# sunyzhi55/Diffusion_Models_Collection

Measured on AMD Instinct MI355X. Metric: CIFAR-10 UNet DDPM train imgs/sec (aggregate over GPUs), higher is better.
Workload: dtype bf16; 1 GPU; configs/cifar10_unet.py UNet DDPM train step at 32x32 (q_sample, fwd, MSE, bwd, clip, AdamW, EMA), dropout 0.1; model=UNet 37.06M (128ch, mult 1,2,2,2, attn 16/8), global_batch=128, per_gpu_batch=128, parallelism=dp1

## Files before the change

### diffusion_models_collection_amd/_lib.py

```python
import ctypes
import os
from pathlib import Path

import torch

_PKG = Path(__file__).resolve().parent
LIB_PATH = Path(os.environ.get("DMC_LIB", _PKG / "libdmc.so"))

DMC_F32, DMC_BF16 = 0, 1
MODE_NORMAL, MODE_UPSAMPLE, MODE_DILATE = 0, 1, 2
PRO_NONE, PRO_AFFINE_SILU, PRO_SILU, PRO_AFFINE, PRO_GN_SILU = 0, 1, 2, 3, 4
LOSS = {"l1": 0, "l2": 1, "huber": 2}
PRED = {"eps": 0, "v": 1}
OBJECTIVE_MAX_BLOCKS = 64
PACK_FWD, PACK_DGRAD, PACK_UPDGRAD = 0, 1, 2

_c_int, _c_p, _c_f, _c_u32, _c_long, _c_size = (ctypes.c_int, ctypes.c_void_p, ctypes.c_float, ctypes.c_uint32,
                                                ctypes.c_long, ctypes.c_size_t)


ACT_NONE, ACT_GELU, ACT_GELU_DROP, ACT_DGELU = 0, 1, 2, 3
FUSED_GN_STATS = 1


class ConvDesc(ctypes.Structure):
    _fields_ = [
        ("dtype", _c_int), ("N", _c_int), ("H", _c_int), ("W", _c_int),
        ("C1", _c_int), ("C2", _c_int), ("ld1", _c_int), ("ld2", _c_int), ("Kc", _c_int),
        ("OH", _c_int), ("OW", _c_int), ("Cout", _c_int), ("ntaps", _c_int), ("mode", _c_int), ("stride", _c_int),
        ("tap_dy", _c_int * 16), ("tap_dx", _c_int * 16),
        ("prologue", _c_int), ("pro_scale", _c_p), ("pro_shift", _c_p), ("ld_pro", _c_int),
        ("drop_seed", _c_u32), ("drop_thresh", _c_u32), ("drop_scale", _c_f), ("drop_ld", _c_int),
        ("drop_seed_base", _c_p),
        ("bias", _c_p), ("addvec", _c_p), ("ld_add", _c_int), ("resid", _c_p), ("ld_res", _c_int),
        ("silu_pre", _c_p), ("ld_silu", _c_int), ("Csplit", _c_int), ("ldy1", _c_int), ("ldy2", _c_int),
        ("out_f32", _c_int), ("out_nchw", _c_int), ("act", _c_int), ("y_pre", _c_p), ("ld_pre", _c_int),
        ("gn_part", _c_p), ("wg_bias", _c_p), ("pro_groups", _c_int), ("pro_eps", _c_f),
    ]


class ConvPlan(ctypes.Structure):
    _fields_ = [("family", _c_int), ("grid", ctypes.c_uint * 3), ("block", _c_int), ("splits", _c_int),
                ("gn_part", _c_int), ("fused_prologue", _c_int), ("ws_bytes", _c_size)]


CONV_FAMILIES = ("none", "nin_halo", "nout_halo", "narrow_in", "narrow_out", "img", "gemm1x1", "halo", "glds", "reg")
GN_PART_NONE, GN_PART_KERNEL, GN_PART_SPLITK, GN_PART_PASS = 0, 1, 2, 3


class WgradJob(ctypes.Structure):
    _fields_ = [("slab", ctypes.c_void_p), ("bslab", ctypes.c_void_p), ("dw", ctypes.c_void_p),
                ("dbias", ctypes.c_void_p), ("splits", ctypes.c_int), ("KK", ctypes.c_int), ("Cpad", ctypes.c_int),
                ("Cout", ctypes.c_int), ("Ctot", ctypes.c_int), ("ntaps", ctypes.c_int), ("Kc", ctypes.c_int),
                ("scale", ctypes.c_float), ("layout", ctypes.c_int)]


class WgradPlan(ctypes.Structure):
    _fields_ = [("kind", _c_int), ("grid", ctypes.c_uint * 3), ("block", _c_int), ("splits", _c_int),
                ("layout", _c_int), ("group_kind", _c_int), ("ws_bytes", _c_size)]


WGRAD_KINDS = ("", "img4", "pipe", "halo", "gemm1x1", "generic")


class WgradGroupItem(ctypes.Structure):
    _fields_ = [("d", ctypes.POINTER(ConvDesc)), ("dy", ctypes.c_void_p), ("ld_dy", ctypes.c_int),
                ("x1", ctypes.c_void_p), ("x2", ctypes.c_void_p), ("workspace", ctypes.c_void_p),
                ("dw", ctypes.c_void_p), ("scale", ctypes.c_float)]


WGRAD_GROUP_MAX = 8


class ColsumJob(ctypes.Structure):
    _fields_ = [("in_", ctypes.c_void_p), ("R", ctypes.c_int), ("C", ctypes.c_int), ("ld", ctypes.c_long),
                ("stride", ctypes.c_int), ("out0", ctypes.c_void_p), ("out1", ctypes.c_void_p),
                ("scale", ctypes.c_float)]


class PackJob(ctypes.Structure):
    _fields_ = [("w", _c_p), ("dst", _c_p), ("dtype", _c_int), ("mode", _c_int), ("Cout", _c_int), ("Cin", _c_int),
                ("kh", _c_int), ("kw", _c_int), ("Kc", _c_int), ("koff", _c_int)]


class TensorRef(ctypes.Structure):
    _fields_ = [("a", _c_p), ("b", _c_p), ("n", _c_long)]


def _load():
    if not LIB_PATH.exists():
        raise RuntimeError(
            f"libdmc.so not found at {LIB_PATH}. Build it with `python -m diffusion_models_collection_amd.build` "
            "(there is no fallback: the diffusion hot path runs only on the gfx950 HIP kernels).")
    lib = ctypes.CDLL(str(LIB_PATH))
    sig = {
        "dmc_version": (_c_int, []),
        "dmc_set_option": (_c_int, [ctypes.c_char_p, _c_long]),
        "dmc_get_option": (_c_long, [ctypes.c_char_p]),
        "dmc_reset_options": (None, [_c_int]),
        "dmc_last_error": (ctypes.c_char_p, []),
        "dmc_conv2d_workspace": (_c_size, [ctypes.POINTER(ConvDesc)]),
        "dmc_conv_halo_prologue": (_c_int, [ctypes.POINTER(ConvDesc)]),
        "dmc_conv2d_fused_epilogue": (_c_int, [ctypes.POINTER(ConvDesc), ctypes.c_size_t]),
        "dmc_conv2d_plan": (_c_int, [ctypes.POINTER(ConvDesc), ctypes.c_size_t, ctypes.POINTER(ConvPlan)]),
        "dmc_conv2d": (_c_int, [ctypes.POINTER(ConvDesc), _c_p, _c_p, _c_p, _c_p, _c_p, _c_p, _c_size, _c_p]),
        "dmc_conv2d_wgrad_workspace": (_c_size, [ctypes.POINTER(ConvDesc)]),
        "dmc_conv2d_wgrad": (_c_int, [ctypes.POINTER(ConvDesc), _c_p, _c_int, _c_p, _c_p, _c_p, _c_p, _c_f, _c_p]),
        "dmc_conv2d_wgrad_partial": (_c_int, [ctypes.POINTER(ConvDesc), _c_p, _c_int, _c_p, _c_p, _c_p, _c_p, _c_f,
                                              ctypes.POINTER(WgradJob), _c_p]),
        "dmc_wgrad_reduce_batch": (_c_int, [ctypes.POINTER(WgradJob), _c_int, _c_p]),
        "dmc_conv2d_wgrad_plan": (_c_int, [ctypes.POINTER(ConvDesc), _c_int, ctypes.POINTER(WgradPlan)]),
        "dmc_conv2d_wgrad_group_ok": (_c_int, [ctypes.POINTER(ConvDesc), _c_int]),
        "dmc_conv2d_wgrad_group_workspace": (_c_size, [ctypes.POINTER(WgradGroupItem), _c_int,
                                                       ctypes.POINTER(_c_size)]),
        "dmc_conv2d_wgrad_group": (_c_int, [ctypes.POINTER(WgradGroupItem), _c_int, ctypes.POINTER(WgradJob), _c_p]),
        "dmc_wgrad_slab_bytes": (_c_long, [_c_int]),
        "dmc_pack_weight": (_c_int, [_c_int, _c_int, _c_p, _c_int, _c_int, _c_int, _c_int, _c_int, _c_p, _c_p]),
        "dmc_pack_tiles": (_c_int, [ctypes.POINTER(PackJob), _c_int, _c_p, _c_int]),
        "dmc_pack_weights": (_c_int, [_c_p, _c_p, _c_int, _c_p]),
        "dmc_gn_workspace": (_c_size, [_c_int, _c_int, _c_int, _c_int]),
        "dmc_gn_stats": (_c_int, [_c_int, _c_p, _c_p, _c_int, _c_int, _c_int, _c_int, _c_int, _c_int, _c_int, _c_f,
                                  _c_p, _c_p, _c_p, _c_p, _c_p, _c_p, _c_p]),
        "dmc_gn_finalize": (_c_int, [_c_p, _c_int, _c_p, _c_int, _c_int, _c_int, _c_int, _c_f, _c_p, _c_p, _c_p, _c_p,
                                     _c_p, _c_p]),
        "dmc_gn_stats_apply_ok": (_c_int, [_c_int, _c_int, _c_int, _c_int, _c_int, _c_int]),
        "dmc_gn_stats_apply": (_c_int, [_c_int, _c_p, _c_p, _c_int, _c_int, _c_int, _c_int, _c_int, _c_int, _c_int,
                                        _c_f, _c_p, _c_p, _c_p, _c_p, _c_p, _c_int, _c_u32, _c_p, _c_u32, _c_f, _c_p,
                                        _c_int, _c_p]),
        "dmc_gn_apply": (_c_int, [_c_int, _c_p, _c_p, _c_int, _c_int, _c_int, _c_int, _c_int, _c_int, _c_p, _c_p,
                                  _c_int, _c_u32, _c_p, _c_u32, _c_f, _c_p, _c_int, _c_p]),
        "dmc_gn_silu_bwd": (_c_int, [_c_int, _c_p, _c_int, _c_p, _c_p, _c_int, _c_int, _c_int, _c_int, _c_int,
                                     _c_int, _c_int, _c_p, _c_p, _c_p, _c_int, _c_u32, _c_p, _c_u32, _c_f, _c_p, _c_p,
                                     _c_int, _c_int, _c_int, _c_int, _c_p, _c_p, _c_p, _c_int, _c_p, _c_p, _c_p,
                                     _c_p]),
        "dmc_gn_silu_bwd_deferred": (_c_int, [_c_int, _c_p, _c_int, _c_p, _c_p, _c_int, _c_int, _c_int, _c_int,
                                              _c_int, _c_int, _c_int, _c_p, _c_p, _c_p, _c_int, _c_u32, _c_p, _c_u32,
                                              _c_f, _c_p, _c_p, _c_int, _c_int, _c_int, _c_int, _c_p, _c_p, _c_p,
                                              _c_int, _c_p, _c_p, _c_p, _c_p, _c_p, ctypes.POINTER(ctypes.c_int),
                                              _c_p, _c_int, _c_p]),
        "dmc_colsum_batch": (_c_int, [ctypes.POINTER(ColsumJob), _c_int, _c_p]),
        "dmc_channel_sum_workspace": (_c_size, [_c_int, _c_int, _c_int]),
        "dmc_channel_sum": (_c_int, [_c_int, _c_p, _c_int, _c_int, _c_int, _c_int, _c_p, _c_int, _c_p, _c_f, _c_p,
                                     _c_p]),
        "dmc_attn_fwd": (_c_int, [_c_int, _c_p, _c_int, _c_int, _c_int, _c_int, _c_int, _c_p, _c_int, _c_p, _c_u32,
                                  _c_p, _c_u32, _c_f, _c_p]),
        "dmc_attn_workspace": (_c_size, [_c_int, _c_int, _c_int]),
        "dmc_attn_bwd": (_c_int, [_c_int, _c_p, _c_int, _c_p, _c_p, _c_int, _c_p, _c_int, _c_int, _c_int, _c_int,
                                  _c_p, _c_int, _c_p, _c_u32, _c_p, _c_u32, _c_f, _c_p]),
        "dmc_time_embed": (_c_int, [_c_p, _c_int, _c_int, _c_p, _c_p]),
        "dmc_embed_fwd": (_c_int, [_c_p, _c_int, _c_int, _c_p, _c_int, _c_p, _c_p]),
        "dmc_embed_bwd": (_c_int, [_c_p, _c_int, _c_int, _c_p, _c_int, _c_p, _c_p]),
        "dmc_pack_input": (_c_int, [_c_int, _c_p, _c_p, _c_p, _c_p, _c_p, _c_int, _c_int, _c_int, _c_int, _c_p,
                                    _c_int, _c_p]),
        "dmc_q_sample": (_c_int, [_c_p, _c_p, _c_p, _c_p, _c_p, _c_int, _c_int, _c_p, _c_p]),
        "dmc_loss_fwd": (_c_int, [_c_int, _c_p, _c_p, _c_long, _c_p, _c_p, _c_p]),
        "dmc_loss_bwd": (_c_int, [_c_int, _c_p, _c_p, _c_long, _c_p, _c_p, _c_p]),
        "dmc_objective": (_c_int, [_c_int, _c_int, _c_p, _c_p, _c_p, _c_p, _c_p, _c_p, _c_p, _c_int, _c_int, _c_int,
                                   _c_p, _c_p, _c_p, _c_p, _c_p]),
        "dmc_pred_convert": (_c_int, [_c_int, _c_p, _c_p, _c_p, _c_p, _c_int, _c_p, _c_int, _c_int, _c_int, _c_p,
                                      _c_p, _c_p]),
        "dmc_ddim_step": (_c_int, [_c_p, _c_p, _c_p, _c_p, _c_p, _c_p, _c_int, _c_int, _c_f, _c_int, _c_p, _c_p,
                                   _c_p]),
        "dmc_ddpm_step": (_c_int, [_c_p, _c_p, _c_p, _c_p, _c_p, _c_p, _c_p, _c_p, _c_p, _c_int, _c_int, _c_int,
                                   _c_p, _c_p, _c_p]),
        "dmc_dpm_step": (_c_int, [_c_p, _c_p, _c_p, _c_p, _c_p, _c_p, _c_int, _c_int, _c_int, _c_int, _c_p, _c_p,
                                  _c_p]),
        "dmc_known_blend": (_c_int, [_c_p, _c_p, _c_p, _c_int, _c_p, _c_p, _c_p, _c_p, _c_int, _c_int, _c_int, _c_p,
                                     _c_p]),
        "dmc_cfg_x0": (_c_int, [_c_p, _c_p, _c_p, _c_f, _c_p, _c_p, _c_p, _c_int, _c_int, _c_int, _c_f, _c_p, _c_p,
                                _c_p]),
        "dmc_ema_update": (_c_int, [_c_p, _c_int, _c_f, _c_p]),
        "dmc_clip_grad_norm": (_c_int, [_c_p, _c_int, _c_f, _c_p, _c_p, _c_p]),
        "dmc_grad_norm_flat": (_c_int, [_c_p, _c_long, _c_f, _c_p, _c_p, _c_p, _c_p]),
        "dmc_adamw_flat": (_c_int, [_c_p, _c_p, _c_p, _c_p, _c_p, _c_long, _c_p] + [_c_f] * 9 + [_c_p]),
        "dmc_adamw_flat_dev": (_c_int, [_c_p, _c_p, _c_p, _c_p, _c_p, _c_long, _c_p, _c_p, _c_p]),
        "dmc_silu_fwd": (_c_int, [_c_p, _c_p, _c_long, _c_p]),
        "dmc_upsample2x_nhwc": (_c_int, [_c_int, _c_p, _c_int, _c_int, _c_int, _c_int, _c_int, _c_p, _c_int, _c_p]),
        "dmc_unpack_output": (_c_int, [_c_int, _c_p, _c_int, _c_int, _c_int, _c_int, _c_int, _c_p, _c_p]),
        "dmc_add": (_c_int, [_c_int, _c_p, _c_p, _c_long, _c_p]),
        "dmc_ln_mod_fwd": (_c_int, [_c_int, _c_p, _c_p, _c_int, _c_p, _c_p, _c_p, _c_int, _c_int, _c_int, _c_int, _c_f,
                                    _c_u32, _c_p, _c_u32, _c_f, _c_p, _c_p, _c_int, _c_p, _c_p, _c_p]),
        "dmc_ln_mod_bwd": (_c_int, [_c_int, _c_p, _c_int, _c_p, _c_p, _c_p, _c_p, _c_int, _c_int, _c_int, _c_int, _c_p,
                                    _c_p, _c_p, _c_p, _c_p]),
        "dmc_dit_rowsum_workspace": (_c_size, [_c_int, _c_int, _c_int]),
        "dmc_gate_bwd": (_c_int, [_c_int, _c_p, _c_p, _c_int, _c_p, _c_int, _c_int, _c_int, _c_int, _c_u32, _c_p, _c_u32,
                                  _c_f, _c_p, _c_int, _c_p, _c_p, _c_p]),
# ... 87 lines not shown
```

### diffusion_models_collection_amd/csrc/dmc_conv.hip

```cpp
#include "dmc_conv_impl.h"

namespace {

template <typename T> DMC_DEV void load4(const char* p, size_t idx, float* v, bool f32);
template <typename T>
DMC_DEV void load4(const char* p, size_t idx, float* v, bool f32) {
  if (f32 || sizeof(T) == 4) {
    v4f x = *(const v4f*)(p + idx * 4);
    v[0] = x[0]; v[1] = x[1]; v[2] = x[2]; v[3] = x[3];
  } else {
    v2i x = *(const v2i*)(p + idx * 2);
    v[0] = bf2f((uint32_t)x[0] & 0xffffu); v[1] = bf2f((uint32_t)x[0] >> 16);
    v[2] = bf2f((uint32_t)x[1] & 0xffffu); v[3] = bf2f((uint32_t)x[1] >> 16);
  }
}
template <typename T>
DMC_DEV void store4(char* p, size_t idx, const float* v, bool f32) {
  if (f32 || sizeof(T) == 4) {
    v4f x = {v[0], v[1], v[2], v[3]};
    *(v4f*)(p + idx * 4) = x;
  } else {
    v2i x;
    x[0] = (int)f2bf2(v[0], v[1]);
    x[1] = (int)f2bf2(v[2], v[3]);
// ... 139 lines not shown
template <typename T>
DMC_DEV void apply_act(const ConvK& a, float* v, int pix, int co, bool of32) {
  if (a.act == DMC_ACT_DGELU) {
    float u[4];
    load4<T>(a.ypre, (size_t)pix * a.ldpre + co, u, of32);
    const uint32_t seed = a.dthresh ? a.dseed + (a.dseed_base ? *a.dseed_base : 0u) : 0u;
#pragma unroll
    for (int e = 0; e < 4; ++e) {
      const float g = (sizeof(T) == 2 && !of32) ? bf2f(f2bf(v[e])) : v[e];
      float m = 1.f;
      if (a.dthresh) m = drop_keep((uint64_t)pix * a.Cout + co + e, seed, a.dthresh) ? a.dscale : 0.f;
      v[e] = g * m * gelu_grad(u[e]);
    }
    return;
  }
  if (a.ypre) store4<T>(a.ypre, (size_t)pix * a.ldpre + co, v, of32);
#pragma unroll
  for (int e = 0; e < 4; ++e) {
    const float u = (sizeof(T) == 2 && !of32) ? bf2f(f2bf(v[e])) : v[e];
    v[e] = gelu_f(u);
  }
  if (a.act == DMC_ACT_GELU_DROP && a.dthresh) {
    const uint32_t seed = a.dseed + (a.dseed_base ? *a.dseed_base : 0u);
#pragma unroll
    for (int e = 0; e < 4; ++e)
      v[e] = drop_keep((uint64_t)pix * a.Cout + co + e, seed, a.dthresh) ? v[e] * a.dscale : 0.f;
  }
}

template <typename T>
DMC_DEV void conv_store_tile(const ConvK& a, const v4f accv, const int pix, const int co) {
  const bool of32 = a.out_f32 != 0;
  if (pix < a.M && co < a.Cout) {
    const int n = pix / a.OHW;
    {
      float v[4] = {accv[0], accv[1], accv[2], accv[3]};
      const bool full = (co + 3 < a.Cout) && ((a.Cout & 3) == 0);
      if (full && !a.out_nchw) {
        if (a.bias) { v4f b = *(const v4f*)(a.bias + co); v[0] += b[0]; v[1] += b[1]; v[2] += b[2]; v[3] += b[3]; }
        if (a.addvec) { v4f b = *(const v4f*)(a.addvec + (size_t)n * a.ld_add + co); v[0] += b[0]; v[1] += b[1]; v[2] += b[2]; v[3] += b[3]; }
        if (a.silu_pre) {
          v4f z = *(const v4f*)(a.silu_pre + (size_t)pix * a.ld_silu + co);
#pragma unroll
          for (int e = 0; e < 4; ++e) { float sg = sigmoid_f(z[e]); v[e] *= sg * (1.f + z[e] * (1.f - sg)); }
        }
        if (a.resid) { float r[4]; load4<T>(a.resid, (size_t)pix * a.ld_res + co, r, of32); v[0] += r[0]; v[1] += r[1]; v[2] += r[2]; v[3] += r[3]; }
        if (a.act) apply_act<T>(a, v, pix, co, of32);
        if (co < a.Csplit) store4<T>(a.y1, (size_t)pix * a.ldy1 + co, v, of32);
        else store4<T>(a.y2, (size_t)pix * a.ldy2 + (co - a.Csplit), v, of32);
      } else {
#pragma unroll
        for (int e = 0; e < 4; ++e) {
          const int c = co + e;
          if (c >= a.Cout) break;
          float x = v[e];
          if (a.bias) x += a.bias[c];
          if (a.addvec) x += a.addvec[(size_t)n * a.ld_add + c];
          if (a.silu_pre) { float z = a.silu_pre[(size_t)pix * a.ld_silu + c]; float sg = sigmoid_f(z); x *= sg * (1.f + z * (1.f - sg)); }
          if (a.out_nchw) {
            const int rem = pix - n * a.OHW;
            float* y = (float*)a.y1 + ((size_t)n * a.Cout + c) * a.OHW + rem;
            if (a.resid) x += ((const float*)a.resid)[((size_t)n * a.Cout + c) * a.OHW + rem];
            *y = x;
          } else {
            if (a.resid) x += (of32 ? ld_as_f<float>(a.resid, (size_t)pix * a.ld_res + c) : ld_as_f<T>(a.resid, (size_t)pix * a.ld_res + c));
            if (c < a.Csplit) {
              if (of32) ((float*)a.y1)[(size_t)pix * a.ldy1 + c] = x; else st_from_f<T>(a.y1, (size_t)pix * a.ldy1 + c, x);
            } else {
              if (of32) ((float*)a.y2)[(size_t)pix * a.ldy2 + c - a.Csplit] = x; else st_from_f<T>(a.y2, (size_t)pix * a.ldy2 + c - a.Csplit, x);
            }
          }
        }
      }
    }
  }
}

DMC_DEV void chan_eq(float& m, float& q, float mb, float qb, float n) {
  const float d = mb - m;
  q = q + qb + d * d * (0.5f * n);
  m = 0.5f * (m + mb);
}

template <int BM, int BN, int NT>
DMC_DEV void tile_epilogue8(const ConvK& a, const char* lds, int EP, int m0, int n0) {
  constexpr int CG = BN / 8, RS = NT / CG, IT = BM / RS;
  constexpr int SEG = 64, NSEG = BM / SEG, KPS = SEG / RS;
  static_assert((CG == 16 || CG == 8) && SEG % RS == 0 && BM % SEG == 0, "GroupNorm partial geometry");
  const int cg = threadIdx.x % CG, r0 = threadIdx.x / CG;
  const int co = n0 + cg * 8;
  if (co >= a.Cout) return;
  float gm[NSEG], gq[NSEG];
#pragma unroll
  for (int j = 0; j < NSEG; ++j) { gm[j] = 0.f; gq[j] = 0.f; }
  v4f b0 = {0.f, 0.f, 0.f, 0.f}, b1 = {0.f, 0.f, 0.f, 0.f};
  if (a.bias) { b0 = *(const v4f*)(a.bias + co); b1 = *(const v4f*)(a.bias + co + 4); }
  const bool first = co < a.Csplit;
  char* const y = first ? a.y1 : a.y2;
  const int ldy = first ? a.ldy1 : a.ldy2, cy = first ? co : co - a.Csplit;
  v4i rr[IT];
  if (a.resid) {
#pragma unroll
    for (int k = 0; k < IT; ++k) {
      const int pix = min(m0 + r0 + k * RS, a.M - 1);
      rr[k] = *(const v4i*)(a.resid + ((size_t)pix * a.ld_res + co) * 2);
    }
  }
  int n = (m0 + r0) / a.OHW, nend = (n + 1) * a.OHW;
  v4f e0 = {0.f, 0.f, 0.f, 0.f}, e1 = {0.f, 0.f, 0.f, 0.f};
  if (a.addvec) {
    e0 = *(const v4f*)(a.addvec + (size_t)n * a.ld_add + co);
    e1 = *(const v4f*)(a.addvec + (size_t)n * a.ld_add + co + 4);
  }
#pragma unroll
  for (int k = 0; k < IT; ++k) {
    const int pl = r0 + k * RS;
    const int pix = m0 + pl;
    if (pix < a.M) {
      if (a.addvec && pix >= nend) {
        n = pix / a.OHW;
        nend = (n + 1) * a.OHW;
        e0 = *(const v4f*)(a.addvec + (size_t)n * a.ld_add + co);
        e1 = *(const v4f*)(a.addvec + (size_t)n * a.ld_add + co + 4);
      }
      const v4f v0 = *(const v4f*)(lds + pl * EP + cg * 32) + b0 + e0;
      const v4f v1 = *(const v4f*)(lds + pl * EP + cg * 32 + 16) + b1 + e1;
      float f[8] = {v0[0], v0[1], v0[2], v0[3], v1[0], v1[1], v1[2], v1[3]};
      if (a.resid) {
        float r[8];
        Chunk<bf16_t>::unpack(rr[k], r);
#pragma unroll
        for (int e = 0; e < 8; ++e) f[e] += r[e];
      }
      if (a.act == DMC_ACT_DGELU) {
        Chunk<bf16_t>::unpack(Chunk<bf16_t>::pack(f), f);
        float u[8];
        Chunk<bf16_t>::unpack(*(const v4i*)(a.ypre + ((size_t)pix * a.ldpre + co) * 2), u);
        const uint32_t seed = a.dthresh ? a.dseed + (a.dseed_base ? *a.dseed_base : 0u) : 0u;
#pragma unroll
        for (int e = 0; e < 8; ++e) {
          float m = 1.f;
          if (a.dthresh) m = drop_keep((uint64_t)pix * a.Cout + co + e, seed, a.dthresh) ? a.dscale : 0.f;
          f[e] = f[e] * m * gelu_grad(u[e]);
        }
      } else if (a.act) {
        const v4i pre = Chunk<bf16_t>::pack(f);
        if (a.ypre) *(v4i*)(a.ypre + ((size_t)pix * a.ldpre + co) * 2) = pre;
        Chunk<bf16_t>::unpack(pre, f);
#pragma unroll
        for (int e = 0; e < 8; ++e) f[e] = gelu_f(f[e]);
        if (a.act == DMC_ACT_GELU_DROP && a.dthresh) {
          const uint32_t seed = a.dseed + (a.dseed_base ? *a.dseed_base : 0u);
#pragma unroll
          for (int e = 0; e < 8; ++e)
            f[e] = drop_keep((uint64_t)pix * a.Cout + co + e, seed, a.dthresh) ? f[e] * a.dscale : 0.f;
        }
      }
      const v4i out = Chunk<bf16_t>::pack(f);
      *(v4i*)(y + ((size_t)pix * ldy + cy) * 2) = out;
      if (a.gst) {
        float g[8];
        Chunk<bf16_t>::unpack(out, g);
        float mb = 0.f;
#pragma unroll
        for (int e = 0; e < 8; ++e) mb += g[e];
        mb *= 0.125f;
        float qb = 0.f;
#pragma unroll
        for (int e = 0; e < 8; ++e) qb = fmaf(g[e] - mb, g[e] - mb, qb);
        const int kk = k % KPS;
#pragma unroll
        for (int j = 0; j < NSEG; ++j) {
          if (j != k / KPS) continue;
          if (kk == 0) { gm[j] = mb; gq[j] = qb; }
          else {
            const float d = mb - gm[j], nn = 8.f * kk;
            gm[j] += d * (8.f / (nn + 8.f));
            gq[j] += qb + d * d * (nn * 8.f / (nn + 8.f));
          }
        }
      }
    }
  }
  if (a.gst) {
    const int lane = threadIdx.x & 63, wave = threadIdx.x >> 6;
    constexpr int NW = NT / 64;
    float cnt = 8.f * KPS;
#pragma unroll
    for (int sh = CG; sh < 64; sh <<= 1) {
#pragma unroll
      for (int j = 0; j < NSEG; ++j) {
        const float mb = __shfl_xor(gm[j], sh), qb = __shfl_xor(gq[j], sh);
        chan_eq(gm[j], gq[j], mb, qb, cnt);
      }
      cnt *= 2.f;
    }
    float* red = (float*)(lds + BM * EP);
    if (lane < CG) {
#pragma unroll
      for (int j = 0; j < NSEG; ++j) {
        red[((wave * NSEG + j) * CG + lane) * 2] = gm[j];
        red[((wave * NSEG + j) * CG + lane) * 2 + 1] = gq[j];
      }
    }
    __syncthreads();
    if (threadIdx.x < NSEG * CG) {
      const int j = threadIdx.x / CG, c = threadIdx.x % CG;
      float m = red[(j * CG + c) * 2], q = red[(j * CG + c) * 2 + 1];
      for (int w = 1; w < NW; ++w) {
        const float mb = red[((w * NSEG + j) * CG + c) * 2], qb = red[((w * NSEG + j) * CG + c) * 2 + 1];
        const float na = cnt * w, nb = cnt;
        const float d = mb - m;
        m += d * (nb / (na + nb));
        q += qb + d * d * (na * nb / (na + nb));
      }
      const size_t o = ((size_t)(m0 / SEG + j) * (a.Cout / 8) + (n0 / 8 + c)) * 2;
      a.gst[o] = m;
      a.gst[o + 1] = q;
    }
  }
}

template <typename T, int BM, int BN, int NT>
DMC_DEV void tile_epilogue(const ConvK& a, const char* lds, int EP, int m0, int n0) {
  constexpr int CG = BN / 4, RS = NT / CG;
  const int cg = threadIdx.x % CG, r0 = threadIdx.x / CG;
  const int co = n0 + cg * 4;
  if (a.out_nchw || a.silu_pre || (a.Cout & 3)) {
    for (int pl = r0; pl < BM; pl += RS) conv_store_tile<T>(a, *(const v4f*)(lds + pl * EP + cg * 16), m0 + pl, co);
    return;
  }
  if constexpr ((BN == 128 || BN == 64) && BM % 64 == 0) {
    if (sizeof(T) == 2 && !a.out_f32 && !((a.Cout | a.Csplit | a.ldy1 | a.ldy2 | a.ld_res) & 7)) {
      tile_epilogue8<BM, BN, NT>(a, lds, EP, m0, n0);
      return;
    }
  }
  if (co >= a.Cout) return;
  const bool of32 = a.out_f32 != 0;
  const v4f b = a.bias ? *(const v4f*)(a.bias + co) : v4f{0.f, 0.f, 0.f, 0.f};
  const bool first = co < a.Csplit;
  char* const y = first ? a.y1 : a.y2;
  const int ldy = first ? a.ldy1 : a.ldy2, cy = first ? co : co - a.Csplit;
  int n = (m0 + r0) / a.OHW, nend = (n + 1) * a.OHW;
  for (int pl = r0; pl < BM; pl += RS) {
    const int pix = m0 + pl;
    if (pix >= a.M) break;
    v4f v = *(const v4f*)(lds + pl * EP + cg * 16) + b;
    if (a.addvec) {
      while (pix >= nend) { ++n; nend += a.OHW; }
      v += *(const v4f*)(a.addvec + (size_t)n * a.ld_add + co);
    }
    float f[4] = {v[0], v[1], v[2], v[3]};
    if (a.resid) {
      float r[4];
      load4<T>(a.resid, (size_t)pix * a.ld_res + co, r, of32);
      f[0] += r[0]; f[1] += r[1]; f[2] += r[2]; f[3] += r[3];
    }
    if (a.act) apply_act<T>(a, f, pix, co, of32);
    store4<T>(y, (size_t)pix * ldy + cy, f, of32);
  }
}

__device__ v4i g_zero_page[64];


template <int AI, int BI, int BM>
DMC_DEV void glds_issue(const ConvK& a, char* base, int k0, int c0, int wave, int lrow, int lc, int n0,
                        const int* sp) {
  const int c = c0 + lc * 8;
  const int Ctot = a.C1 + a.C2;
#pragma unroll
  for (int j = 0; j < AI; ++j) {
    const void* src = g_zero_page;
    if (sp[j] >= 0 && c < Ctot)
      src = (c < a.C1) ? (const void*)(a.x1 + ((size_t)sp[j] * a.ld1 + c) * 2)
                       : (const void*)(a.x2 + ((size_t)sp[j] * a.ld2 + (c - a.C1)) * 2);
    __builtin_amdgcn_global_load_lds(src, (LDS_AS void*)(base + (wave * AI + j) * 8 * 128), 16, 0, 0);
  }
  const size_t wrow = (size_t)a.ntaps * a.Kc;
#pragma unroll
  for (int j = 0; j < BI; ++j) {
    const int co = n0 + (wave * BI + j) * 8 + lrow;
    const void* src = (co < a.Cout) ? (const void*)(a.w + ((size_t)co * wrow + k0 + lc * 8) * 2) : g_zero_page;
    __builtin_amdgcn_global_load_lds(src, (LDS_AS void*)(base + BM * 128 + (wave * BI + j) * 8 * 128), 16, 0, 0);
  }
}


template <int AI, int BI, int BM>
DMC_DEV void glds_issue_buf(const ConvK& a, char* base, int c0, unsigned k2, int wave, const unsigned* o1,
                            const unsigned* o2, const unsigned* ob) {
  if (c0 < a.C1) {
    const __amdgpu_buffer_rsrc_t r = __builtin_amdgcn_make_buffer_rsrc((void*)a.x1, (short)0, a.x1_bytes, 0x00020000);
    const unsigned c2 = (unsigned)c0 * 2u;
#pragma unroll
    for (int j = 0; j < AI; ++j)
      __builtin_amdgcn_raw_ptr_buffer_load_lds(r, (LDS_AS void*)(base + (wave * AI + j) * 1024), 16, o1[j] + c2, 0, 0, 0);
  } else {
    const __amdgpu_buffer_rsrc_t r = __builtin_amdgcn_make_buffer_rsrc((void*)a.x2, (short)0, a.x2_bytes, 0x00020000);
    const unsigned c2 = (unsigned)(c0 - a.C1) * 2u;
#pragma unroll
    for (int j = 0; j < AI; ++j)
      __builtin_amdgcn_raw_ptr_buffer_load_lds(r, (LDS_AS void*)(base + (wave * AI + j) * 1024), 16, o2[j] + c2, 0, 0, 0);
  }
  const __amdgpu_buffer_rsrc_t rw = __builtin_amdgcn_make_buffer_rsrc((void*)a.w, (short)0, a.w_bytes, 0x00020000);
#pragma unroll
  for (int j = 0; j < BI; ++j)
    __builtin_amdgcn_raw_ptr_buffer_load_lds(rw, (LDS_AS void*)(base + BM * 128 + (wave * BI + j) * 1024), 16, ob[j] + k2, 0, 0, 0);
}

DMC_DEV void xcd_tile(int NB, int& mb, int& nb) {
  const int total = gridDim.x, bid = blockIdx.x, per = total >> 3;
  const int t = bid < (per << 3) ? (bid & 7) * per + (bid >> 3) : bid;
  mb = t / NB;
  nb = t - mb * NB;
}

__host__ __device__ inline bool reg_epi_ok(const ConvK& a) {
  return a.reg_epi && (a.gst || a.reg_epi >= 2) && a.dtype_bytes == 2 && !a.out_f32 && !a.out_nchw && !a.silu_pre && a.Csplit == a.Cout &&
         a.act == DMC_ACT_NONE && (a.Cout & 127) == 0 && (a.ldy1 & 7) == 0 &&
         (!a.resid || (a.ld_res & 7) == 0) && (a.M & 127) == 0 && (!a.gst || a.OHW % 64 == 0);
}
DMC_DEV void reg_epilogue(const ConvK& a, v4f (&acc)[4][4], int m0, int n0, int wm, int wn) {
  const int lane = threadIdx.x & 63, fr = lane & 15, fh = lane >> 4;
  const bool odd = fh & 1;
  v4i rra[4][2];
  v4f ba[4], eva[4];
  const int img0 = (m0 + wm * 64) / a.OHW;
#pragma unroll
  for (int i = 0; i < 4; ++i) {
    const int co = n0 + wn * 64 + i * 16 + fh * 4;
    const int cc = co - (odd ? 4 : 0);
#pragma unroll
    for (int jp = 0; jp < 2; ++jp) {
      rra[i][jp] = v4i{0, 0, 0, 0};
      if (a.resid) {
        const int px = m0 + wm * 64 + (2 * jp + (odd ? 1 : 0)) * 16 + fr;
        rra[i][jp] = *(const v4i*)(a.resid + ((size_t)px * a.ld_res + cc) * 2);
      }
    }
    ba[i] = a.bias ? *(const v4f*)(a.bias + co) : v4f{0.f, 0.f, 0.f, 0.f};
    eva[i] = a.addvec ? *(const v4f*)(a.addvec + (size_t)img0 * a.ld_add + co) : v4f{0.f, 0.f, 0.f, 0.f};
  }
#pragma unroll
  for (int i = 0; i < 4; ++i) {
    const int co = n0 + wn * 64 + i * 16 + fh * 4;
    const int cc = co - (odd ? 4 : 0);
    const v4f b = ba[i];
    float gm = 0.f, gq = 0.f;
    int nimg = img0;
    v4f ev = eva[i];
#pragma unroll
    for (int jp = 0; jp < 2; ++jp) {
      v2i o[2];
      const v4i rr = rra[i][jp];
      v2i rs;
      rs[0] = __shfl_xor(odd ? rr[0] : rr[2], 16);
      rs[1] = __shfl_xor(odd ? rr[1] : rr[3], 16);
#pragma unroll
      for (int h = 0; h < 2; ++h) {
        const int j = 2 * jp + h;
        const int px = m0 + wm * 64 + j * 16 + fr;
        v4f v = acc[i][j] + b;
        if (a.addvec) {
          const int n = px / a.OHW;
          if (n != nimg) { nimg = n; ev = *(const v4f*)(a.addvec + (size_t)n * a.ld_add + co); }
          v = v + ev;
        }
        float f[4] = {v[0], v[1], v[2], v[3]};
        if (a.resid) {
          const bool own = (h == 1) == odd;
          const uint32_t r0 = own ? (uint32_t)(odd ? rr[2] : rr[0]) : (uint32_t)rs[0];
          const uint32_t r1 = own ? (uint32_t)(odd ? rr[3] : rr[1]) : (uint32_t)rs[1];
          f[0] += bf2f(r0 & 0xffffu); f[1] += bf2f(r0 >> 16);
          f[2] += bf2f(r1 & 0xffffu); f[3] += bf2f(r1 >> 16);
        }
        o[h][0] = (int)f2bf2(f[0], f[1]);
        o[h][1] = (int)f2bf2(f[2], f[3]);
        if (a.gst) {
          const float g0 = bf2f((uint32_t)o[h][0] & 0xffffu), g1 = bf2f((uint32_t)o[h][0] >> 16);
          const float g2 = bf2f((uint32_t)o[h][1] & 0xffffu), g3 = bf2f((uint32_t)o[h][1] >> 16);
          const float mb = ((g0 + g1) + (g2 + g3)) * 0.25f;
          const float qb =
              fmaf(g3 - mb, g3 - mb, fmaf(g2 - mb, g2 - mb, fmaf(g1 - mb, g1 - mb, (g0 - mb) * (g0 - mb))));
          if (j == 0) { gm = mb; gq = qb; }
          else {
            const float d = mb - gm, nn = 4.f * j;
            gm += d * (4.f / (nn + 4.f));
            gq += qb + d * d * (nn * 4.f / (nn + 4.f));
          }
        }
      }
      v2i send = odd ? o[0] : o[1], recv;
      recv[0] = __shfl_xor(send[0], 16);
      recv[1] = __shfl_xor(send[1], 16);
      v4i outv;
      if (!odd) { outv[0] = o[0][0]; outv[1] = o[0][1]; outv[2] = recv[0]; outv[3] = recv[1]; }
      else { outv[0] = recv[0]; outv[1] = recv[1]; outv[2] = o[1][0]; outv[3] = o[1][1]; }
      const int pxs = m0 + wm * 64 + (2 * jp + (odd ? 1 : 0)) * 16 + fr;
      *(v4i*)(a.y1 + ((size_t)pxs * a.ldy1 + cc) * 2) = outv;
    }
    if (a.gst) {
      float cnt = 16.f;
#pragma unroll
      for (int sh = 1; sh <= 16; sh <<= 1) {
        const float mb = __shfl_xor(gm, sh), qb = __shfl_xor(gq, sh);
        chan_eq(gm, gq, mb, qb, cnt);
        cnt *= 2.f;
      }
      if (fr == 0 && !odd) {
        const size_t o = ((size_t)((m0 + wm * 64) / 64) * (a.Cout / 8) + cc / 8) * 2;
        a.gst[o] = gm;
        a.gst[o + 1] = gq;
      }
    }
  }
}

template <int WM, int WN, bool BUF, int STAGES = 3>
__global__ __launch_bounds__(WM * WN * 64) void conv_fwd_glds_kernel(ConvK a) {
  using T = bf16_t;
  constexpr int NW = WM * WN;
  constexpr int BM = 64 * WM, BN = 64 * WN;
  constexpr int SB = (BM + BN) * 128;
  constexpr int AI = BM / 8 / NW;
  constexpr int BI = BN / 8 / NW;
  static_assert(AI >= 1 && BI >= 1, "tile too small for the wave count");
  constexpr int EPB = BM * (BN * 4 + 16) + NW * (BM / 64) * 16 * (NW <= 4 ? 64 : 8);
  constexpr int LDS_BYTES = STAGES * SB > EPB ? STAGES * SB : EPB;
  __shared__ __attribute__((aligned(16))) char lds[LDS_BYTES];

  const int lane = threadIdx.x & 63;
  const int wave = __builtin_amdgcn_readfirstlane(threadIdx.x >> 6);
  const int wm = wave % WM, wn = wave / WM;
  int mb = blockIdx.x, nb = blockIdx.y;
  if (!a.sk && gridDim.y == 1) xcd_tile((a.Cout + BN - 1) / BN, mb, nb);
  const int m0 = mb * BM;
  const int n0 = nb * BN;
  const int lrow = lane >> 3;
  const int lc = (lane & 7) ^ lrow;

  int pn[AI], poy[AI], pox[AI];
#pragma unroll
  for (int j = 0; j < AI; ++j) {
    const int pix = m0 + (wave * AI + j) * 8 + lrow;
    if (pix < a.M) {
      pn[j] = pix / a.OHW;
      const int rem = pix - pn[j] * a.OHW;
      poy[j] = rem / a.OW;
      pox[j] = rem - poy[j] * a.OW;
    } else {
      pn[j] = -1; poy[j] = 0; pox[j] = 0;
    }
  }
  const int nstages = a.ntaps * (a.Kc / 64);

  v4f acc[4][4];
#pragma unroll
  for (int i = 0; i < 4; ++i)
#pragma unroll
    for (int j = 0; j < 4; ++j) acc[i][j] = v4f{0.f, 0.f, 0.f, 0.f};

  const int s_begin = a.sk ? blockIdx.z * a.sk_per : 0;
  const int s_end = a.sk ? min(nstages, s_begin + a.sk_per) : nstages;
  const int ns = s_end - s_begin;
  const int kst = a.Kc / 64;
  int is_tap = s_begin / kst, is_c0 = (s_begin - is_tap * kst) * 64;
  int sp[AI];
  unsigned o1[AI], o2[AI], ob[BI];
  if constexpr (BUF) {
    const unsigned wrow = (unsigned)(a.ntaps * a.Kc);
#pragma unroll
    for (int j = 0; j < BI; ++j) {
      const int co = n0 + (wave * BI + j) * 8 + lrow;
      ob[j] = co < a.Cout ? ((unsigned)co * wrow + lc * 8) * 2u : kOOB;
    }
  }
  auto tap_rows = [&]() {
#pragma unroll
    for (int j = 0; j < AI; ++j) {
      const int p = pn[j] >= 0 ? src_pixel(a, pn[j], poy[j], pox[j], is_tap) : -1;
      if constexpr (BUF) {
        o1[j] = p >= 0 ? ((unsigned)p * a.ld1 + lc * 8) * 2u : kOOB;
        o2[j] = p >= 0 ? ((unsigned)p * a.ld2 + lc * 8) * 2u : kOOB;
      } else {
        sp[j] = p;
      }
    }
  };
  tap_rows();
  auto issue = [&](int S) {
    char* base = lds + (S % STAGES) * SB;
    if constexpr (BUF) {
      glds_issue_buf<AI, BI, BM>(a, base, is_c0, (unsigned)(s_begin + S) * 128u, wave, o1, o2, ob);
    } else {
      glds_issue<AI, BI, BM>(a, base, (s_begin + S) * 64, is_c0, wave, lrow, lc, n0, sp);
    }
    is_c0 += 64;
    if (is_c0 == a.Kc) { is_c0 = 0; ++is_tap; if (is_tap < a.ntaps) tap_rows(); }
  };
#define DMC_GLDS_ISSUE(S) issue(S)
  for (int q = 0; q < STAGES - 1 && q < ns; ++q) DMC_GLDS_ISSUE(q);
  const int fr = lane & 15, fh = lane >> 4;
  for (int s = 0; s < ns; ++s) {
    if (STAGES > 2 && s + STAGES - 2 < ns) __builtin_amdgcn_s_waitcnt(waitcnt_vm((STAGES - 2) * (AI + BI)));
    else __builtin_amdgcn_s_waitcnt(waitcnt_vm(0));
    asm volatile("" ::: "memory");
    __builtin_amdgcn_sched_barrier(0);
    __builtin_amdgcn_s_barrier();
    __builtin_amdgcn_sched_barrier(0);
    asm volatile("" ::: "memory");
    if (s + STAGES - 1 < ns) DMC_GLDS_ISSUE(s + STAGES - 1);
    const char* A = lds + (s % STAGES) * SB;
    const char* B = A + BM * 128;
    v4i fa[2][4], fb[2][4];
#pragma unroll
    for (int ks = 0; ks < 2; ++ks) {
      const int chunk = ks * 4 + fh;
#pragma unroll
      for (int i = 0; i < 4; ++i) {
        const int r = wn * 64 + i * 16 + fr;
        fa[ks][i] = *(const v4i*)(B + r * 128 + ((chunk ^ (r & 7)) << 4));
      }
#pragma unroll
      for (int j = 0; j < 4; ++j) {
        const int r = wm * 64 + j * 16 + fr;
        fb[ks][j] = *(const v4i*)(A + r * 128 + ((chunk ^ (r & 7)) << 4));
      }
    }
#pragma unroll
    for (int ks = 0; ks < 2; ++ks)
#pragma unroll
      for (int i = 0; i < 4; ++i)
#pragma unroll
        for (int j = 0; j < 4; ++j) acc[i][j] = mma16<T>(acc[i][j], fa[ks][i], fb[ks][j]);
    __builtin_amdgcn_sched_group_barrier(0x100, 8, 0);
#pragma unroll
    for (int g = 0; g < 8; ++g) {
      __builtin_amdgcn_sched_group_barrier(0x008, 2, 0);
      __builtin_amdgcn_sched_group_barrier(0x100, 1, 0);
    }
    __builtin_amdgcn_sched_group_barrier(0x008, 16, 0);
  }
#undef DMC_GLDS_ISSUE
  constexpr int EP = BN * 4 + 16;
  if constexpr (WM == 2 && WN == 2) {
    if (!a.sk && reg_epi_ok(a) && n0 + BN <= a.Cout && m0 + BM <= a.M) {
      reg_epilogue(a, acc, m0, n0, wm, wn);
      return;
    }
  }
  __syncthreads();
#pragma unroll
  for (int j = 0; j < 4; ++j)
#pragma unroll
    for (int i = 0; i < 4; ++i)
      *(v4f*)(lds + (wm * 64 + j * 16 + fr) * EP + (wn * 64 + i * 16 + fh * 4) * 4) = acc[i][j];
  __syncthreads();
  if (a.sk) {
    const int Cpad = gridDim.y * BN;
    float* slab = a.sk + (size_t)blockIdx.z * a.M * Cpad;
    for (int idx = threadIdx.x; idx < BM * BN / 4; idx += NW * 64) {
      const int pl = idx / (BN / 4), cg = idx - pl * (BN / 4);
      if (m0 + pl < a.M) *(v4f*)(slab + (size_t)(m0 + pl) * Cpad + n0 + cg * 4) = *(const v4f*)(lds + pl * EP + cg * 16);
    }
    return;
  }
  tile_epilogue<T, BM, BN, NW * 64>(a, lds, EP, m0, n0);
}

DMC_DEV void wait_vm_upto40(int n) {
  switch (n < 0 ? 0 : n) {
#define DMC_W(i) case i: __builtin_amdgcn_s_waitcnt(waitcnt_vm(i)); break;
    DMC_W(0) DMC_W(1) DMC_W(2) DMC_W(3) DMC_W(4) DMC_W(5) DMC_W(6) DMC_W(7) DMC_W(8) DMC_W(9) DMC_W(10)
    DMC_W(11) DMC_W(12) DMC_W(13) DMC_W(14) DMC_W(15) DMC_W(16) DMC_W(17) DMC_W(18) DMC_W(19) DMC_W(20)
    DMC_W(21) DMC_W(22) DMC_W(23) DMC_W(24) DMC_W(25) DMC_W(26) DMC_W(27) DMC_W(28) DMC_W(29) DMC_W(30)
    DMC_W(31) DMC_W(32) DMC_W(33) DMC_W(34) DMC_W(35) DMC_W(36) DMC_W(37) DMC_W(38) DMC_W(39)
#undef DMC_W
    default: __builtin_amdgcn_s_waitcnt(waitcnt_vm(40)); break;
  }
}

template <int NS>
__global__ __launch_bounds__(256, NS <= 2 ? 2 : 1) void gemm1x1_persist_kernel(ConvK a, int ntiles, int NB, int tpb) {
  using T = bf16_t;
  constexpr int BM = 128, BN = 128, AI = 4, BI = 4, SB = (BM + BN) * 128;
  __shared__ __attribute__((aligned(16))) char lds[NS * SB + 4096];
  float* const sbias = (float*)(lds + NS * SB);
  const int lane = threadIdx.x & 63;
  const int wave = __builtin_amdgcn_readfirstlane(threadIdx.x >> 6);
  const int wm = wave % 2, wn = wave / 2;
  const int lrow = lane >> 3, lc = (lane & 7) ^ lrow;
  const int fr = lane & 15, fh = lane >> 4;
  const int t_begin = blockIdx.x * tpb, t_end = min(ntiles, t_begin + tpb);
  if (t_begin >= t_end) return;
  const int kst = a.Kc / 64, total = (t_end - t_begin) * kst;
  for (int c = threadIdx.x; c < NB * BN; c += 256) sbias[c] = (a.bias && c < a.Cout) ? a.bias[c] : 0.f;
  __builtin_amdgcn_s_waitcnt(waitcnt_vm(0));

  unsigned o1[AI], o2[AI], ob[BI];
  int it_tile = -1;
  auto issue = [&](int S) {
    const int ti = t_begin + S / kst, k = S - (S / kst) * kst;
    if (ti != it_tile) {
      it_tile = ti;
      const int mb = ti / NB, nb = ti - mb * NB;
#pragma unroll
      for (int j = 0; j < AI; ++j) {
        const unsigned pix = (unsigned)(mb * BM + (wave * AI + j) * 8 + lrow);
        o1[j] = (pix * a.ld1 + lc * 8) * 2u;
        o2[j] = (pix * a.ld2 + lc * 8) * 2u;
      }
#pragma unroll
      for (int j = 0; j < BI; ++j) {
        const unsigned co = (unsigned)(nb * BN + (wave * BI + j) * 8 + lrow);
        ob[j] = (co * a.Kc + lc * 8) * 2u;
      }
    }
    glds_issue_buf<AI, BI, BM>(a, lds + (S % NS) * SB, k * 64, (unsigned)k * 128u, wave, o1, o2, ob);
  };
  int nvm = 0;
  int pos[NS];
#pragma unroll
  for (int q = 0; q < NS; ++q) pos[q] = 0;
  for (int q = 0; q < NS - 1 && q < total; ++q) {
    issue(q);
    nvm += AI + BI;
    pos[q] = nvm;
  }
  v4f acc[4][4];
#pragma unroll
  for (int i = 0; i < 4; ++i)
#pragma unroll
    for (int j = 0; j < 4; ++j) acc[i][j] = v4f{0.f, 0.f, 0.f, 0.f};
  for (int s = 0; s < total; ++s) {
    int mine = 0;
#pragma unroll
    for (int q = 0; q < NS; ++q)
      if (q == s % NS) mine = pos[q];
    wait_vm_upto40(nvm - mine);
    asm volatile("" ::: "memory");
    __builtin_amdgcn_sched_barrier(0);
    __builtin_amdgcn_s_barrier();
    __builtin_amdgcn_sched_barrier(0);
    asm volatile("" ::: "memory");
    v2i rres[4][4];
    const bool last = (s + 1) % kst == 0;
    if (a.resid && last) {
      const int t = t_begin + s / kst, mb = t / NB, nb = t - mb * NB;
#pragma unroll
      for (int i = 0; i < 4; ++i)
// ... 472 lines not shown
        const int cc = ks * 4 + fh;
#pragma unroll
        for (int i = 0; i < NI; ++i) {
          const int r = (i * 16 + fr) * 9 + t;
          ga[ks][i] = *(const v4i*)(Wt + r * 128 + ((cc ^ (r & 7)) << 4));
        }
#pragma unroll
        for (int j = 0; j < NJ; ++j)
          gb[ks][j] = *(const v4i*)(ok[j] ? A + src[j] * 128 + ((cc ^ (src[j] & 7)) << 4) : zrow);
      }
    };
    read_tap(0, fa[0], fb[0]);
    __builtin_amdgcn_sched_group_barrier(0x100, 2 * (NI + NJ), 0);
#pragma unroll
    for (int t = 0; t < 9; ++t) {
      const int cur = t & 1;
      if (t + 1 < 9) read_tap(t + 1, fa[cur ^ 1], fb[cur ^ 1]);
#pragma unroll
      for (int ks = 0; ks < 2; ++ks)
#pragma unroll
        for (int i = 0; i < NI; ++i)
#pragma unroll
          for (int j = 0; j < NJ; ++j) acc[i][j] = mma16<T>(acc[i][j], fa[cur][ks][i], fb[cur][ks][j]);
      if (t + 1 < 9) __builtin_amdgcn_sched_group_barrier(0x100, 2 * (NI + NJ), 0);
      __builtin_amdgcn_sched_group_barrier(0x008, 2 * NI * NJ, 0);
    }
  }
  if (fast) {
#pragma unroll
    for (int i = 0; i < NI; ++i) {
      float gm = 0.f, gq = 0.f;
#pragma unroll
      for (int j = 0; j < NJ; ++j) {
        const int co = n0 + i * 16 + fh * 4, pix = m0 + qrow[j];
        const v4f v = (acc[i][j] + eb[i]) + ea[i][NJE == 1 ? 0 : j];
        const float r0 = bf2f((uint32_t)er[i][j][0] & 0xffffu), r1 = bf2f((uint32_t)er[i][j][0] >> 16);
        const float r2 = bf2f((uint32_t)er[i][j][1] & 0xffffu), r3 = bf2f((uint32_t)er[i][j][1] >> 16);
        v2i o;
        o[0] = (int)f2bf2(v[0] + r0, v[1] + r1);
        o[1] = (int)f2bf2(v[2] + r2, v[3] + r3);
        *(v2i*)(a.y1 + ((size_t)pix * a.ldy1 + co) * 2) = o;
        if (MW == 64 && a.gst) {
          const float g0 = bf2f((uint32_t)o[0] & 0xffffu), g1 = bf2f((uint32_t)o[0] >> 16);
          const float g2 = bf2f((uint32_t)o[1] & 0xffffu), g3 = bf2f((uint32_t)o[1] >> 16);
          const float mb = ((g0 + g1) + (g2 + g3)) * 0.25f;
          const float qb =
              fmaf(g3 - mb, g3 - mb, fmaf(g2 - mb, g2 - mb, fmaf(g1 - mb, g1 - mb, (g0 - mb) * (g0 - mb))));
          if (j == 0) { gm = mb; gq = qb; }
          else {
            const float d = mb - gm, nn = 4.f * j;
            gm += d * (4.f / (nn + 4.f));
            gq += qb + d * d * (nn * 4.f / (nn + 4.f));
          }
        }
      }
      if (MW == 64 && a.gst) {
        float cnt = 16.f;
#pragma unroll
        for (int sh = 1; sh <= 16; sh <<= 1) {
          const float mb = __shfl_xor(gm, sh), qb = __shfl_xor(gq, sh);
          chan_eq(gm, gq, mb, qb, cnt);
          cnt *= 2.f;
        }
        if (fr == 0 && !(fh & 1)) {
          const size_t o = ((size_t)((m0 + wave * 64) / 64) * (a.Cout / 8) + (n0 + i * 16 + fh * 4) / 8) * 2;
          a.gst[o] = gm;
          a.gst[o + 1] = gq;
        }
      }
    }
    return;
  }
#pragma unroll
  for (int i = 0; i < NI; ++i)
#pragma unroll
    for (int j = 0; j < NJ; ++j) conv_store_tile<T>(a, acc[i][j], m0 + qrow[j], n0 + i * 16 + fh * 4);
}

bool dma_operands_ok(const ConvK& k) {
  return k.C1 % 64 == 0 && k.C2 % 64 == 0 && k.Kc == k.C1 + k.C2 && k.x1_bytes > 0 && (k.C2 == 0 || k.x2_bytes > 0) &&
         k.w_bytes > 0;
}

int img_plan(const ConvK& k, long mask) {
  if (!mask || k.dtype_bytes != 2 || (k.prologue != DMC_PRO_NONE && k.prologue != DMC_PRO_GN_SILU)) return 0;
  if (k.prologue == DMC_PRO_GN_SILU) {
    const int C = k.C1 + k.C2;
    if (k.tdy0 != -1 || C > 512 || k.gn_G <= 0 || C % k.gn_G || (C / k.gn_G) % 8 || 64 % (C / k.gn_G) || k.dthresh)
      return 0;
  }
  if (!same_size_3x3(k) || !((k.OH == 8 && k.OW == 8) || (k.OH == 4 && k.OW == 4)) || k.M % 128) return 0;
  if (!dma_operands_ok(k)) return 0;
  const int bit = (k.OH == 8 ? 2 : 0) + (k.tdy0 == 1 ? 1 : 0);
  if (!((mask >> bit) & 1)) return 0;
  const int bm = k.OH == 8 ? 256 : 128;
  if (k.M % bm) return 0;
  const int bn = (long)k.Cout * (k.M / bm) >= 512L * 16 ? 32 : 16;
  if (k.Cout % bn) return 0;
  if (k.OH == 8 && (long)(k.M / bm) * (k.Cout / bn) > 256) return 0;
  if (k.prologue == DMC_PRO_GN_SILU && !((k.OH == 4 && bn == 16) || (k.OH == 8 && bn == 32))) return 0;
  return bn;
}

int nin_plan(const ConvK& k, int* R, int* nimg) {
  if (k.dtype_bytes != 2 || k.prologue != DMC_PRO_NONE || k.C2 != 0 || k.C1 > 8 || k.ld1 != 8 || k.Cout % 128 ||
      k.silu_pre || k.act)
    return 0;
  return halo2_plan(k, R, nimg);
}
int nout_plan(const ConvK& k, int* R, int* nimg) {
  if (k.dtype_bytes != 2 || k.prologue != DMC_PRO_NONE || k.Cout > 16 || k.C1 + k.C2 > 128 || !dma_operands_ok(k) ||
      k.act)
    return 0;
  return halo2_plan(k, R, nimg);
}


template <typename T>
DMC_DEV v4i mask_chunk(v4i v, int n) {
#pragma unroll
  for (int d = 0; d < 4; ++d) {
    if (sizeof(T) == 4) {
      if (d >= n) v[d] = 0;
    } else {
      if (2 * d >= n) v[d] = 0;
      else if (2 * d + 1 >= n) v[d] &= 0xffff;
    }
  }
  return v;
}

DMC_DEV void pixel_coords(const ConvK& a, int pix, int& n, int& oy, int& ox) {
  n = pix < a.M ? pix / a.OHW : -1;
  const int rem = pix - (n < 0 ? 0 : n) * a.OHW;
  oy = rem / a.OW;
  ox = rem - oy * a.OW;
}

template <typename T>
__global__ __launch_bounds__(256) void conv_narrow_in_kernel(ConvK a) {
  const int lane = threadIdx.x & 63;
  const int fr = lane & 15, fh = lane >> 4;
  const int p0 = (blockIdx.x * 4 + (threadIdx.x >> 6)) * 64;
  const int n0 = blockIdx.y * 32;
  if (p0 >= a.M) return;
  int pn[4], poy[4], pox[4];
#pragma unroll
  for (int j = 0; j < 4; ++j) pixel_coords(a, p0 + 16 * j + fr, pn[j], poy[j], pox[j]);
  const size_t wrow = (size_t)a.ntaps * a.Kc;
  v4f acc[2][4];
#pragma unroll
  for (int i = 0; i < 2; ++i)
#pragma unroll
    for (int j = 0; j < 4; ++j) acc[i][j] = v4f{0.f, 0.f, 0.f, 0.f};
  for (int t0 = 0; t0 < a.ntaps; t0 += 4) {
    const int tap = t0 + fh;
    const bool tok = tap < a.ntaps;
    const int tp = tok ? tap : 0;
    v4i fa[2];
#pragma unroll
    for (int i = 0; i < 2; ++i) {
      const int co = n0 + 16 * i + fr;
      v4i w = *(const v4i*)(a.w + ((size_t)(co < a.Cout ? co : 0) * wrow + (size_t)tp * a.Kc) * sizeof(T));
      if (!(tok && co < a.Cout)) w = v4i{0, 0, 0, 0};
      fa[i] = w;
    }
// ... 236 lines not shown
  if constexpr (SP > 0) {
    v4f v[SP];
#pragma unroll
    for (int z = 0; z < SP; ++z) v[z] = *(const v4f*)(p + z * zs);
    v4f t = v[0];
#pragma unroll
    for (int z = 1; z < SP; ++z) t += v[z];
    return t;
  } else {
    v4f t = *(const v4f*)p;
    for (int z = 1; z < splits; ++z) t += *(const v4f*)(p + z * zs);
    return t;
  }
}

template <typename T, int SP>
__global__ __launch_bounds__(256) void conv_splitk_epilogue_kernel(ConvK a, int splits, int Cpad) {
  const int cg_per_row = Cpad / 4;
  const long total = (long)a.M * cg_per_row;
  const size_t zs = (size_t)a.M * Cpad;
  for (long idx = blockIdx.x * (long)blockDim.x + threadIdx.x; idx < total; idx += (long)gridDim.x * blockDim.x) {
    const int pix = idx / cg_per_row;
    const int co = (idx - (long)pix * cg_per_row) * 4;
    if (co >= a.Cout) continue;
    const v4f v = splitk_sum<SP>(a.sk + (size_t)pix * Cpad + co, zs, splits);
    conv_store_tile<T>(a, v, pix, co);
  }
}
template <typename T, int SP>
__global__ __launch_bounds__(256) void conv_splitk_epi_gn_kernel(ConvK a, int splits, int Cpad) {
  const int lane = threadIdx.x & 63;
  const int nch = a.Cout / 8;
  const long w = blockIdx.x * 4L + (threadIdx.x >> 6);
  if (w >= (long)(a.M / 64) * nch) return;
  const int seg = (int)(w / nch), ch = (int)(w - (long)seg * nch);
  const int pix = seg * 64 + lane, co = ch * 8;
  const size_t zs = (size_t)a.M * Cpad;
  const float* p = a.sk + (size_t)pix * Cpad + co;
  const v4f v0 = splitk_sum<SP>(p, zs, splits), v1 = splitk_sum<SP>(p + 4, zs, splits);
  conv_store_tile<T>(a, v0, pix, co);
  conv_store_tile<T>(a, v1, pix, co + 4);
  const size_t row = (size_t)pix * a.ldy1 + co;
  float f[8];
  load4<T>(a.y1, row, f, false);
  load4<T>(a.y1, row + 4, f + 4, false);
  float t = 0.f;
#pragma unroll
  for (int e = 0; e < 8; ++e) t += f[e];
  const float m = wave_sum(t) * (1.0f / 512.0f);
  float q = 0.f;
#pragma unroll
  for (int e = 0; e < 8; ++e) q = fmaf(f[e] - m, f[e] - m, q);
  q = wave_sum(q);
  if (lane == 0) { a.gsk[w * 2] = m; a.gsk[w * 2 + 1] = q; }
}

template <typename T>
void launch_splitk_epilogue(const ConvK& k, int splits, int Cpad, int blocks, hipStream_t s) {
  switch (splits) {
    case 2: conv_splitk_epilogue_kernel<T, 2><<<blocks, 256, 0, s>>>(k, splits, Cpad); break;
    case 3: conv_splitk_epilogue_kernel<T, 3><<<blocks, 256, 0, s>>>(k, splits, Cpad); break;
    case 4: conv_splitk_epilogue_kernel<T, 4><<<blocks, 256, 0, s>>>(k, splits, Cpad); break;
    case 5: conv_splitk_epilogue_kernel<T, 5><<<blocks, 256, 0, s>>>(k, splits, Cpad); break;
    case 6: conv_splitk_epilogue_kernel<T, 6><<<blocks, 256, 0, s>>>(k, splits, Cpad); break;
    case 7: conv_splitk_epilogue_kernel<T, 7><<<blocks, 256, 0, s>>>(k, splits, Cpad); break;
    case 8: conv_splitk_epilogue_kernel<T, 8><<<blocks, 256, 0, s>>>(k, splits, Cpad); break;
    default: conv_splitk_epilogue_kernel<T, 0><<<blocks, 256, 0, s>>>(k, splits, Cpad); break;
  }
}
void launch_splitk_epi_gn(const ConvK& k, int splits, int Cpad, hipStream_t s) {
  const int blocks = (int)(((long)(k.M / 64) * (k.Cout / 8) + 3) / 4);
  switch (splits) {
    case 2: conv_splitk_epi_gn_kernel<bf16_t, 2><<<blocks, 256, 0, s>>>(k, splits, Cpad); break;
    case 3: conv_splitk_epi_gn_kernel<bf16_t, 3><<<blocks, 256, 0, s>>>(k, splits, Cpad); break;
    case 4: conv_splitk_epi_gn_kernel<bf16_t, 4><<<blocks, 256, 0, s>>>(k, splits, Cpad); break;
    case 5: conv_splitk_epi_gn_kernel<bf16_t, 5><<<blocks, 256, 0, s>>>(k, splits, Cpad); break;
    case 6: conv_splitk_epi_gn_kernel<bf16_t, 6><<<blocks, 256, 0, s>>>(k, splits, Cpad); break;
    case 7: conv_splitk_epi_gn_kernel<bf16_t, 7><<<blocks, 256, 0, s>>>(k, splits, Cpad); break;
    case 8: conv_splitk_epi_gn_kernel<bf16_t, 8><<<blocks, 256, 0, s>>>(k, splits, Cpad); break;
    default: conv_splitk_epi_gn_kernel<bf16_t, 0><<<blocks, 256, 0, s>>>(k, splits, Cpad); break;
  }
}

DMC_DEV float pack_value(int mode, const float* w, int Cout, int Cin, int kh, int kw, int row, int t, int k) {
  if (mode == DMC_PACK_FWD) return k < Cin ? w[((size_t)row * Cin + k) * kh * kw + t] : 0.f;
  if (k >= Cout) return 0.f;
  if (mode == DMC_PACK_DGRAD) return w[((size_t)k * Cin + row) * kh * kw + t];
  const int u = t >> 2, vv = t & 3;
  const int khs[4][2] = {{2, -1}, {1, 2}, {0, 1}, {0, -1}};
  const float* base = w + ((size_t)k * Cin + row) * 9;
  float v = 0.f;
  for (int a1 = 0; a1 < 2; ++a1) {
    const int y = khs[u][a1];
    if (y < 0) continue;
    for (int b1 = 0; b1 < 2; ++b1) {
      const int x = khs[vv][b1];
      if (x < 0) continue;
      v += base[y * 3 + x];
    }
  }
  return v;
}

template <typename T>
__global__ void pack_weight_kernel(int mode, const float* w, int Cout, int Cin, int kh, int kw, int Kc, T* dst) {
  const int ntaps = (mode == DMC_PACK_UPDGRAD) ? 16 : kh * kw;
  const int rows = (mode == DMC_PACK_FWD) ? Cout : Cin;
  const long total = (long)rows * ntaps * Kc;
  for (long o = blockIdx.x * (long)blockDim.x + threadIdx.x; o < total; o += (long)gridDim.x * blockDim.x) {
    const int k = o % Kc;
    const long r = o / Kc;
    const float v = pack_value(mode, w, Cout, Cin, kh, kw, r / ntaps, r % ntaps, k);
    if (sizeof(T) == 4) ((float*)dst)[o] = v;
    else ((bf16_t*)dst)[o] = (bf16_t)f2bf(v);
  }
}

constexpr int kPackFwdK = 256, kPackFwdCo = 4, kPackDgC = 16, kPackDgCo = 64;
constexpr int kPackDgP = kPackDgC * 9 + 1;
constexpr int kPackLds = kPackDgCo * kPackDgP > kPackFwdCo * kPackFwdK * 9 ? kPackDgCo * kPackDgP
                                                                          : kPackFwdCo * kPackFwdK * 9;

__global__ __launch_bounds__(256) void pack_tiles_kernel(const dmc_pack_job* jobs, const int* tiles) {
  __shared__ float sw[kPackLds];
  const int* tl = tiles + 3 * blockIdx.x;
  const dmc_pack_job J = jobs[tl[0]];
  const int khkw = J.kh * J.kw;
  const int koff = J.koff >= 0 ? J.koff : 0;
  const bool f32 = J.dtype == DMC_F32;
  const int tid = threadIdx.x, wv = tid >> 6, ln = tid & 63;
  auto store = [&](long di, float v) {
    if (f32) ((float*)J.dst)[di] = v;
    else ((bf16_t*)J.dst)[di] = (bf16_t)f2bf(v);
  };
  if (J.mode == DMC_PACK_FWD) {
    const int co0 = tl[1], k0 = tl[2];
    const int nco = min(kPackFwdCo, J.Cout - co0);
    const int KW = J.koff >= 0 ? J.Cin : J.Kc;
    const int kn = min(kPackFwdK, KW - k0);
    const int kv = max(0, min(kn, J.Cin - k0));
    const int run = kv * khkw;
    {
      float v[kPackFwdCo][9];
#pragma unroll
      for (int r = 0; r < kPackFwdCo; ++r)
#pragma unroll
        for (int u = 0; u < 9; ++u) {
          const int j = tid + u * 256;
          v[r][u] = (r < nco && j < run) ? J.w[((size_t)(co0 + r) * J.Cin + k0) * khkw + j] : 0.f;
        }
#pragma unroll
      for (int r = 0; r < kPackFwdCo; ++r)
#pragma unroll
        for (int u = 0; u < 9; ++u)
          if (r < nco && tid + u * 256 < run) sw[r * kPackFwdK * 9 + tid + u * 256] = v[r][u];
    }
    __syncthreads();
    if (!f32 && ((J.Kc | koff | k0 | kn) & 1) == 0) {
      for (int r = 0; r < nco; ++r)
        for (int t = 0; t < khkw; ++t)
          for (int k = 2 * tid; k < kn; k += 512) {
            const float v0 = k < kv ? sw[r * kPackFwdK * 9 + k * khkw + t] : 0.f;
            const float v1 = k + 1 < kv ? sw[r * kPackFwdK * 9 + (k + 1) * khkw + t] : 0.f;
            *(uint32_t*)((bf16_t*)J.dst + ((long)(co0 + r) * khkw + t) * J.Kc + koff + k0 + k) = f2bf2(v0, v1);
          }
      return;
    }
    for (int r = 0; r < nco; ++r)
      for (int t = 0; t < khkw; ++t)
        for (int k = tid; k < kn; k += 256)
          store(((long)(co0 + r) * khkw + t) * J.Kc + koff + k0 + k, k < kv ? sw[r * kPackFwdK * 9 + k * khkw + t] : 0.f);
    return;
  }
  const int c0 = tl[1], co0 = tl[2];
  const int KW = J.koff >= 0 ? J.Cout : J.Kc;
  const int cn = min(kPackDgC, J.Cin - c0), con = min(kPackDgCo, KW - co0);
  const int cov = max(0, min(con, J.Cout - co0));
  const int run = cn * khkw;
  {
    float v[16][3];
#pragma unroll
    for (int a2 = 0; a2 < 16; ++a2)
#pragma unroll
      for (int u = 0; u < 3; ++u) {
        const int r = wv + 4 * a2, j = ln + 64 * u;
        v[a2][u] = (r < cov && j < run) ? J.w[((size_t)(co0 + r) * J.Cin + c0) * khkw + j] : 0.f;
      }
#pragma unroll
    for (int a2 = 0; a2 < 16; ++a2)
#pragma unroll
      for (int u = 0; u < 3; ++u) {
        const int r = wv + 4 * a2, j = ln + 64 * u;
        if (r < cov && j < run) sw[r * kPackDgP + j] = v[a2][u];
      }
  }
  __syncthreads();
  const int ntaps = J.mode == DMC_PACK_UPDGRAD ? 16 : khkw;
  auto value = [&](int co, int c, int t) {
    float v = 0.f;
    if (co < cov) {
      const float* wp = sw + co * kPackDgP + c * khkw;
      if (J.mode == DMC_PACK_DGRAD) {
        v = wp[t];
      } else {
        const int u = t >> 2, vv = t & 3;
        const int khs[4][2] = {{2, -1}, {1, 2}, {0, 1}, {0, -1}};
        for (int a1 = 0; a1 < 2; ++a1) {
          const int y = khs[u][a1];
          if (y < 0) continue;
          for (int b1 = 0; b1 < 2; ++b1) {
            const int x = khs[vv][b1];
            if (x >= 0) v += wp[y * 3 + x];
          }
        }
      }
    }
    return v;
  };
  if (!f32 && ((J.Kc | koff | co0 | con) & 1) == 0) {
    const int cp = 2 * (ln & 31);
    for (int q = 2 * wv + (ln >> 5); q < cn * ntaps; q += 8) {
      const int c = q / ntaps, t = q - c * ntaps;
      if (cp >= con) continue;
      *(uint32_t*)((bf16_t*)J.dst + ((long)(c0 + c) * ntaps + t) * J.Kc + koff + co0 + cp) =
          f2bf2(value(cp, c, t), value(cp + 1, c, t));
    }
    return;
  }
  const int co = ln;
  for (int q = wv; q < cn * ntaps; q += 4) {
    const int c = q / ntaps, t = q - c * ntaps;
    if (co >= con) continue;
    store(((long)(c0 + c) * ntaps + t) * J.Kc + koff + co0 + co, value(co, c, t));
  }
}


struct FwdPlan {
  int cfg;
  int splits;
  int per;
  size_t ws;
};

FwdPlan plan_glds(const ConvK& k) {
  FwdPlan p{0, 1, 0, 0};
  const int nst = k.ntaps * (k.Kc / 64);
  const long b42 = (long)dmc::cdiv(k.M, 256) * dmc::cdiv(k.Cout, 128);
  const long b22 = (long)dmc::cdiv(k.M, 128) * dmc::cdiv(k.Cout, 128);
  if (b42 >= 240) { p.cfg = 0; return p; }
  long blocks = b22;
  p.cfg = 1;
  const long target = dmc::opt(dmc::OPT_SK_TARGET);
  int sp = (int)((target + blocks - 1) / blocks);
  const int maxs = nst / 4;
  if (sp > maxs) sp = maxs;
  if (sp > dmc::opt(dmc::OPT_SK_MAX)) sp = (int)dmc::opt(dmc::OPT_SK_MAX);
  if (sp >= 2) {
    p.splits = sp;
    p.per = (nst + sp - 1) / sp;
    p.splits = (nst + p.per - 1) / p.per;
    p.ws = (size_t)p.splits * k.M * (size_t)dmc::cdiv(k.Cout, 128) * 128 * sizeof(float);
  } else if (b22 < 120) {
    p.cfg = 2;
  }
  return p;
}

struct RegPlan {
  bool big;
  int splits, per;
  size_t ws;
};

RegPlan plan_reg(const ConvK& k) {
  RegPlan p{false, 1, 0, 0};
  const long t128 = (long)dmc::cdiv(k.M, 128) * dmc::cdiv(k.Cout, 128);
  if (t128 >= 384 && k.Cout >= 128) { p.big = true; return p; }
  const int bk = k.dtype_bytes == 4 ? 32 : 64;
  const int nst = k.ntaps * (k.Kc / bk);
  const long t64 = (long)dmc::cdiv(k.M, 64) * dmc::cdiv(k.Cout, 64);
  if (t64 >= 256 || nst < 16) return p;
  int sp = (int)((256 + t64 - 1) / t64);
  if (sp > nst / 4) sp = nst / 4;
  if (sp > 16) sp = 16;
  if (sp < 2) return p;
  p.per = (nst + sp - 1) / sp;
  p.splits = (nst + p.per - 1) / p.per;
  p.ws = (size_t)p.splits * k.M * (size_t)dmc::cdiv(k.Cout, 64) * 64 * sizeof(float);
  return p;
}

template <typename T>
__global__ __launch_bounds__(256) void gn_part_kernel(const char* y, int ldy, int nseg, int nch, float* out) {
  const int lane = threadIdx.x & 63;
  const long w = blockIdx.x * 4L + (threadIdx.x >> 6);
  if (w >= (long)nseg * nch) return;
  const int seg = (int)(w / nch), ch = (int)(w - (long)seg * nch);
  const size_t row = ((size_t)seg * 64 + lane) * ldy + ch * 8;
  float f[8];
  load4<T>(y, row, f, false);
  load4<T>(y, row + 4, f + 4, false);
  float t = 0.f;
#pragma unroll
  for (int e = 0; e < 8; ++e) t += f[e];
  const float m = wave_sum(t) * (1.0f / 512.0f);
  float q = 0.f;
#pragma unroll
  for (int e = 0; e < 8; ++e) q = fmaf(f[e] - m, f[e] - m, q);
  q = wave_sum(q);
  if (lane == 0) { out[w * 2] = m; out[w * 2 + 1] = q; }
}

int gemm1x1_plan(const ConvK& k) {
  if (k.dtype_bytes != 2 || k.ntaps != 1 || k.stride != 1 || k.mode != DMC_MODE_NORMAL || k.tdy0 || k.tdx0 ||
      k.H != k.OH || k.W != k.OW || k.prologue != DMC_PRO_NONE || !dma_operands_ok(k))
    return 0;
  if (k.addvec || (k.resid && (k.ld_res & 3)) || k.silu_pre || k.act != DMC_ACT_NONE || k.out_f32 || k.out_nchw ||
      (k.ldy1 & 3) || k.M % 128 || k.Cout % 128 || k.Cout > 1024)
    return 0;
  if (k.Csplit != k.Cout && (k.Csplit % 128 || (k.ldy2 & 3) || !k.y2 || k.resid)) return 0;
  const long ntiles = (long)(k.M / 128) * (k.Cout / 128);
  if (ntiles < 128) return 0;
  const long blocks = 512;
  return (int)((ntiles + blocks - 1) / blocks);
}

struct ConvPlan {
  int family = DMC_CONV_NONE;
  dim3 grid{0, 0, 0};
  int block = 256;
  int hp = 0, R = 0, nimg = 0;
  int npl = 0;
  int bn = 0;
  int tpb = 0;
  int wm = 2, stages = 3;
  bool buf = false;
  int tile = 64;
  int splits = 1, per = 0;
  bool fused_pro = false;
  int gn = DMC_GN_PART_NONE;
  size_t ws_report = 0;
};

ConvPlan plan_conv(const ConvK& k, bool want_gn_part, size_t ws_avail) {
  ConvPlan p;
  if (k.M == 0 || k.Cout == 0) return p;
  const bool bf16 = k.dtype_bytes == 2;
  const int epc = bf16 ? 8 : 4;
  const bool no_splitk = dmc::opt(dmc::OPT_NO_SPLITK), no_glds = dmc::opt(dmc::OPT_NO_GLDS);
  const bool no_halo = dmc::opt(dmc::OPT_NO_HALO), no_xcd = dmc::opt(dmc::OPT_NO_XCD);
  const bool dma = dma_operands_ok(k), buf = dma && !dmc::opt(dmc::OPT_NO_BUFLDS);
  const int nb128 = dmc::cdiv(k.Cout, 128);
  auto tiles = [&](int bm) {
    return no_xcd ? dim3(dmc::cdiv(k.M, bm), nb128) : dim3(dmc::cdiv(k.M, bm) * nb128);
  };

  const bool glds_path = bf16 && k.prologue == DMC_PRO_NONE && !no_glds;
  const bool pro_cand = bf16 && k.prologue == DMC_PRO_AFFINE_SILU && k.dthresh == 0 && k.ldp >= k.C1 + k.C2 &&
                        dmc::opt(dmc::OPT_HALO_PRO) && !no_halo && !no_glds && buf;
  const FwdPlan gp = (glds_path || pro_cand) ? plan_glds(k) : FwdPlan{0, 1, 0, 0};
  const RegPlan rp = glds_path ? RegPlan{false, 1, 0, 0} : plan_reg(k);
  p.ws_report = glds_path ? gp.ws : rp.ws;

  const bool narrow = !dmc::opt(dmc::OPT_NO_NARROW), nhalo = narrow && bf16 && !dmc::opt(dmc::OPT_NO_NHALO);
  const bool narrow_in = narrow && k.C2 == 0 && k.C1 <= epc && k.Cout >= 16;
  int R = 0, nimg = 0;
  const int nin_hp = nhalo && narrow_in ? nin_plan(k, &R, &nimg) : 0;
  const int img_bn = img_plan(k, dmc::opt(dmc::OPT_IMG_MASK));
  int pro_R = 0, pro_nimg = 0;
  int pro_hp = pro_cand && (gp.splits == 1 || no_splitk) ? halo2_plan(k, &pro_R, &pro_nimg) : 0;
  if (pro_nimg != 1) pro_hp = 0;
  p.fused_pro = pro_hp != 0 || (k.prologue == DMC_PRO_GN_SILU && img_bn != 0);

  bool epi = false;
  if (want_gn_part && bf16 && !k.out_f32 && !k.out_nchw && !k.silu_pre && k.Csplit == k.Cout && k.Cout % 128 == 0 &&
      k.M % 256 == 0 && k.OHW % 64 == 0 && !((k.Cout | k.ldy1 | k.ld_res) & 7)) {
    if (narrow_in) epi = nin_hp != 0;
    else if (no_glds || dmc::opt(dmc::OPT_NO_EPI_STATS)) epi = false;
    else if (img_bn) epi = k.OH == 8 && k.act == DMC_ACT_NONE;
    else if (k.prologue == DMC_PRO_AFFINE_SILU) epi = pro_hp != 0;
    else if (k.prologue == DMC_PRO_NONE) epi = gp.splits == 1 || ws_avail < gp.ws || no_splitk;
  }
  const bool skgn = want_gn_part && !epi && !dmc::opt(dmc::OPT_NO_SKGN);
  p.gn = !want_gn_part ? DMC_GN_PART_NONE : epi ? DMC_GN_PART_KERNEL : DMC_GN_PART_PASS;

  if (nin_hp) {
    p.family = DMC_CONV_NIN_HALO; p.hp = nin_hp; p.R = R; p.nimg = nimg;
    p.grid = dim3(k.M / 128, k.Cout / 128);
    return p;
  }
  if (nhalo && k.Cout <= 8 && (p.hp = nout_plan(k, &p.R, &p.nimg)) != 0) {
    p.family = DMC_CONV_NOUT_HALO; p.npl = (k.C1 + k.C2) / 64;
    p.grid = dim3(k.M / 128);
    return p;
  }
  if (narrow_in) {
    p.family = DMC_CONV_NARROW_IN;
    p.grid = dim3(dmc::cdiv(k.M, 256), dmc::cdiv(k.Cout, 32));
    return p;
  }
  if (narrow && k.Cout <= 8 && (k.C2 == 0 || k.C1 % epc == 0)) {
    p.family = DMC_CONV_NARROW_OUT;
    p.grid = dim3(dmc::cdiv(k.M, 256));
    return p;
  }
  if (img_bn) {
    p.family = DMC_CONV_IMG; p.bn = img_bn;
    p.grid = dim3(k.M / (k.OH == 8 ? 256 : 128) * (k.Cout / img_bn));
    return p;
  }
  if (dmc::opt(dmc::OPT_GEMM1X1) && !epi && !skgn && (p.tpb = gemm1x1_plan(k)) != 0) {
    p.family = DMC_CONV_GEMM1X1;
    p.grid = dim3(dmc::cdiv((k.M / 128) * (k.Cout / 128), p.tpb));
    return p;
  }
  if (pro_hp) {
    p.family = DMC_CONV_HALO; p.hp = pro_hp; p.R = pro_R; p.nimg = pro_nimg;
    p.grid = tiles(128);
    return p;
  }
  if (glds_path) {
    const bool split = gp.splits > 1 && ws_avail >= gp.ws && !no_splitk;
    p.buf = buf;
    if (buf && !split && !no_halo && (p.hp = halo2_plan(k, &p.R, &p.nimg)) != 0) {
      p.family = DMC_CONV_HALO;
      p.grid = tiles(128);
      return p;
    }
    p.family = DMC_CONV_GLDS;
    if (split) {
      p.splits = gp.splits; p.per = gp.per;
      p.grid = dim3(dmc::cdiv(k.M, 128), nb128, gp.splits);
      if (skgn && k.M % 64 == 0 && k.Cout % 8 == 0 && !k.out_f32 && !k.out_nchw && k.Csplit == k.Cout)
        p.gn = DMC_GN_PART_SPLITK;
    } else if (gp.splits > 1 || gp.cfg == 2) {
      p.wm = 1; p.block = 128;
      p.grid = tiles(64);
    } else {
      if (gp.cfg == 0 || (long)dmc::cdiv(k.M, 128) * nb128 > 256) p.stages = 2;
      p.grid = tiles(128);
    }
    return p;
  }
  p.family = DMC_CONV_REG;
  if (rp.big) {
    p.tile = 128;
    p.grid = dim3(dmc::cdiv(k.M, 128), nb128);
  } else if (rp.splits > 1 && ws_avail >= rp.ws && !no_splitk) {
    p.splits = rp.splits; p.per = rp.per;
    p.grid = dim3(dmc::cdiv(k.M, 64), dmc::cdiv(k.Cout, 64), rp.splits);
  } else {
    p.grid = dim3(dmc::cdiv(k.M, 64), dmc::cdiv(k.Cout, 64));
  }
  return p;
}

int launch_conv(const ConvK& k, const ConvPlan& p, float* part, hipStream_t s) {
  const dim3 g = p.grid;
  switch (p.family) {
    case DMC_CONV_NIN_HALO:
      if (reg_epi_ok(k)) conv3x3_nin_kernel<true><<<g, 256, 0, s>>>(k, p.R, p.nimg);
      else conv3x3_nin_kernel<false><<<g, 256, 0, s>>>(k, p.R, p.nimg);
      break;
    case DMC_CONV_NOUT_HALO:
      if (p.hp == 6) { if (p.npl == 1) conv3x3_nout_kernel<6, 1><<<g, 256, 0, s>>>(k, p.R, p.nimg); else conv3x3_nout_kernel<6, 2><<<g, 256, 0, s>>>(k, p.R, p.nimg); }
      else if (p.hp == 7) { if (p.npl == 1) conv3x3_nout_kernel<7, 1><<<g, 256, 0, s>>>(k, p.R, p.nimg); else conv3x3_nout_kernel<7, 2><<<g, 256, 0, s>>>(k, p.R, p.nimg); }
      else { if (p.npl == 1) conv3x3_nout_kernel<9, 1><<<g, 256, 0, s>>>(k, p.R, p.nimg); else conv3x3_nout_kernel<9, 2><<<g, 256, 0, s>>>(k, p.R, p.nimg); }
      break;
    case DMC_CONV_NARROW_IN:
      if (k.dtype_bytes == 4) conv_narrow_in_kernel<float><<<g, 256, 0, s>>>(k);
      else conv_narrow_in_kernel<bf16_t><<<g, 256, 0, s>>>(k);
      break;
    case DMC_CONV_NARROW_OUT:
      if (k.dtype_bytes == 4) conv_narrow_out_kernel<float><<<g, 256, 0, s>>>(k);
      else conv_narrow_out_kernel<bf16_t><<<g, 256, 0, s>>>(k);
      break;
    case DMC_CONV_IMG:
      if (k.prologue == DMC_PRO_GN_SILU) {
        if (k.OH == 8) conv3x3_img_kernel<32, 64, 2, true><<<g, 256, 0, s>>>(k);
        else conv3x3_img_kernel<16, 32, 4, true><<<g, 256, 0, s>>>(k);
      } else if (k.OH == 8) {
        if (p.bn == 16) conv3x3_img_kernel<16, 64, 3><<<g, 256, 0, s>>>(k);
        else conv3x3_img_kernel<32, 64, 2><<<g, 256, 0, s>>>(k);
      } else {
        if (p.bn == 16) conv3x3_img_kernel<16, 32, 4><<<g, 256, 0, s>>>(k);
        else conv3x3_img_kernel<32, 32, 3><<<g, 256, 0, s>>>(k);
      }
      break;
    case DMC_CONV_GEMM1X1: {
      const int NB = k.Cout / 128, ntiles = (k.M / 128) * NB;
      gemm1x1_persist_kernel<2><<<g, 256, 0, s>>>(k, ntiles, NB, p.tpb);
      break;
    }
    case DMC_CONV_HALO:
      if (p.fused_pro) {
        if (p.hp == 6) conv3x3_halo2_kernel<6, 3, true><<<g, 256, 0, s>>>(k, p.R, p.nimg);
        else if (p.hp == 7) conv3x3_halo2_kernel<7, 3, true><<<g, 256, 0, s>>>(k, p.R, p.nimg);
        else conv3x3_halo2_kernel<9, 2, true><<<g, 256, 0, s>>>(k, p.R, p.nimg);
      } else {
        if (p.hp == 6) conv3x3_halo2_kernel<6, 3, false><<<g, 256, 0, s>>>(k, p.R, p.nimg);
        else if (p.hp == 7) conv3x3_halo2_kernel<7, 3, false><<<g, 256, 0, s>>>(k, p.R, p.nimg);
        else conv3x3_halo2_kernel<9, 2, false><<<g, 256, 0, s>>>(k, p.R, p.nimg);
      }
      break;
    case DMC_CONV_GLDS:
      if (p.wm == 1) {
        if (p.buf) conv_fwd_glds_kernel<1, 2, true><<<g, 128, 0, s>>>(k);
        else conv_fwd_glds_kernel<1, 2, false><<<g, 128, 0, s>>>(k);
      } else if (p.stages == 2) {
        if (p.buf) conv_fwd_glds_kernel<2, 2, true, 2><<<g, 256, 0, s>>>(k);
        else conv_fwd_glds_kernel<2, 2, false, 2><<<g, 256, 0, s>>>(k);
      } else {
        if (p.buf) conv_fwd_glds_kernel<2, 2, true><<<g, 256, 0, s>>>(k);
        else conv_fwd_glds_kernel<2, 2, false><<<g, 256, 0, s>>>(k);
      }
      break;
    case DMC_CONV_REG:
      if (k.dtype_bytes == 4) {
        if (p.tile == 128) conv_fwd_kernel<float, 128, 128><<<g, 256, 0, s>>>(k);
        else conv_fwd_kernel<float, 64, 64><<<g, 256, 0, s>>>(k);
      } else {
        if (p.tile == 128) conv_fwd_kernel<bf16_t, 128, 128><<<g, 256, 0, s>>>(k);
        else conv_fwd_kernel<bf16_t, 64, 64><<<g, 256, 0, s>>>(k);
      }
      break;
    default: return 0;
  }
  if (p.splits > 1) {
    const int bn = p.family == DMC_CONV_GLDS ? 128 : 64, Cpad = dmc::cdiv(k.Cout, bn) * bn;
    const long total = (long)k.M * Cpad / 4;
    const int blocks = (int)((total + 255) / 256 < 8192 ? (total + 255) / 256 : 8192);
    if (p.gn == DMC_GN_PART_SPLITK) launch_splitk_epi_gn(k, p.splits, Cpad, s);
    else if (k.dtype_bytes == 4) launch_splitk_epilogue<float>(k, p.splits, Cpad, blocks, s);
    else launch_splitk_epilogue<bf16_t>(k, p.splits, Cpad, blocks, s);
  }
  const int rc = dmc::check_launch("dmc_conv2d");
  if (rc || p.gn != DMC_GN_PART_PASS) return rc;
  const int nseg = k.M / 64, nch = k.Cout / 8;
  const int blocks = (int)(((long)nseg * nch + 3) / 4);
  if (k.out_f32 || k.dtype_bytes == 4) gn_part_kernel<float><<<blocks, 256, 0, s>>>(k.y1, k.ldy1, nseg, nch, part);
  else gn_part_kernel<bf16_t><<<blocks, 256, 0, s>>>(k.y1, k.ldy1, nseg, nch, part);
  return dmc::check_launch("dmc_conv2d (GroupNorm partials)");
}

int plan_desc(const dmc_conv_desc* d, size_t ws_avail, ConvK& k, ConvPlan& p) {
  if (k.M != 0 && k.Cout != 0 && d->gn_part)
    DMC_REQUIRE(k.OHW % 64 == 0 && k.Cout % 8 == 0 && k.Csplit == k.Cout && !k.out_nchw && k.ldy1 % 4 == 0,
                "conv: GroupNorm partials need OH*OW %% 64 == 0, Cout %% 8 == 0 and one NHWC output");
  p = plan_conv(k, d->gn_part != nullptr, ws_avail);
  DMC_REQUIRE(p.family == DMC_CONV_NONE || k.prologue != DMC_PRO_GN_SILU || p.fused_pro,
              "conv: DMC_PRO_GN_SILU is taken only by the small-map conv (dmc_conv_halo_prologue says when)");
  return 0;
}

}

extern "C" size_t dmc_conv2d_workspace(const dmc_conv_desc* d) {
  ConvK k;
  if (fill_convk(d, nullptr, nullptr, nullptr, nullptr, nullptr, k)) return 0;
  return plan_conv(k, false, 0).ws_report;
}

extern "C" int dmc_conv2d_fused_epilogue(const dmc_conv_desc* d, size_t ws_bytes) {
  ConvK k;
  if (fill_convk(d, nullptr, nullptr, nullptr, nullptr, nullptr, k)) return 0;
  return plan_conv(k, true, ws_bytes).gn == DMC_GN_PART_KERNEL ? DMC_FUSED_GN_STATS : 0;
}

extern "C" int dmc_conv_halo_prologue(const dmc_conv_desc* d) {
  ConvK k;
  if (d == nullptr || fill_convk(d, nullptr, nullptr, nullptr, nullptr, nullptr, k)) return 0;
  return plan_conv(k, false, 0).fused_pro ? 1 : 0;
}

extern "C" int dmc_conv2d_plan(const dmc_conv_desc* d, size_t ws_bytes, dmc_conv_plan* out) {
  ConvK k;
  ConvPlan p;
  static char y2_present;
  if (fill_convk(d, nullptr, nullptr, nullptr, nullptr, &y2_present, k) || plan_desc(d, ws_bytes, k, p)) return 1;
  out->family = p.family;
  out->grid[0] = p.grid.x; out->grid[1] = p.grid.y; out->grid[2] = p.grid.z;
  out->block = p.block;
  out->splits = p.splits;
  out->gn_part = p.gn;
  out->fused_prologue = p.fused_pro;
  out->ws_bytes = p.ws_report;
  return 0;
}

extern "C" int dmc_conv2d(const dmc_conv_desc* d, const void* x1, const void* x2, const void* w, void* y1,
                          void* y2, void* workspace, size_t ws_bytes, void* stream) {
  ConvK k;
  ConvPlan p;
  if (fill_convk(d, x1, x2, w, y1, y2, k) || plan_desc(d, workspace ? ws_bytes : 0, k, p)) return 1;
  if (p.gn == DMC_GN_PART_KERNEL) k.gst = d->gn_part;
  if (p.gn == DMC_GN_PART_SPLITK) k.gsk = d->gn_part;
  if (p.splits > 1) { k.sk = (float*)workspace; k.sk_per = p.per; }
  return launch_conv(k, p, d->gn_part, dmc::as_stream(stream));
}


extern "C" int dmc_pack_weight(int pack_mode, int dtype, const float* w, int Cout, int Cin, int kh, int kw, int Kc,
                               void* dst, void* stream) {
  DMC_REQUIRE(pack_mode >= 0 && pack_mode <= 2, "pack: mode");
  DMC_REQUIRE(pack_mode != DMC_PACK_UPDGRAD || (kh == 3 && kw == 3), "pack: UPDGRAD needs 3x3");
  const int ntaps = pack_mode == DMC_PACK_UPDGRAD ? 16 : kh * kw;
  const long rows = pack_mode == DMC_PACK_FWD ? Cout : Cin;
  const long total = rows * ntaps * Kc;
  const int blocks = (int)((total + 255) / 256 < 8192 ? (total + 255) / 256 : 8192);
  hipStream_t s = dmc::as_stream(stream);
  if (dtype == DMC_F32)
    pack_weight_kernel<float><<<blocks, 256, 0, s>>>(pack_mode, w, Cout, Cin, kh, kw, Kc, (float*)dst);
  else
    pack_weight_kernel<bf16_t><<<blocks, 256, 0, s>>>(pack_mode, w, Cout, Cin, kh, kw, Kc, (bf16_t*)dst);
  return dmc::check_launch("dmc_pack_weight");
}

extern "C" int dmc_pack_tiles(const dmc_pack_job* j, int job_index, int* tiles, int cap) {
  int n = 0;
  auto put = [&](int a, int b) {
    if (tiles && n < cap) { tiles[3 * n] = job_index; tiles[3 * n + 1] = a; tiles[3 * n + 2] = b; }
    ++n;
  };
  if (j->mode == DMC_PACK_FWD) {
    const int KW = j->koff >= 0 ? j->Cin : j->Kc;
    for (int co = 0; co < j->Cout; co += kPackFwdCo)
      for (int k0 = 0; k0 < KW; k0 += kPackFwdK) put(co, k0);
  } else {
    const int KW = j->koff >= 0 ? j->Cout : j->Kc;
    for (int c0 = 0; c0 < j->Cin; c0 += kPackDgC)
      for (int co0 = 0; co0 < KW; co0 += kPackDgCo) put(c0, co0);
  }
  return n;
}

extern "C" int dmc_pack_weights(const dmc_pack_job* jobs, const int* tiles, int ntiles, void* stream) {
  DMC_REQUIRE(ntiles > 0, "pack_weights: empty tile list");
  pack_tiles_kernel<<<ntiles, 256, 0, dmc::as_stream(stream)>>>(jobs, tiles);
  return dmc::check_launch("dmc_pack_weights");
}
```

### diffusion_models_collection_amd/csrc/dmc_conv_impl.h

```cpp
#pragma once
#include "dmc_common.h"
#include "dmc_internal.h"

namespace {

struct ConvK {
  const char* x1; const char* x2; const char* w; char* y1; char* y2;
  int N, H, W, C1, C2, ld1, ld2, Kc, OH, OW, Cout, ntaps, mode, stride;
  int tkw, tdy0, tdx0, tsy, tsx;
  int prologue; const float* psc; const float* psh; int ldp;
  uint32_t dseed, dthresh; float dscale; int dld; const uint32_t* dseed_base;
  const float* bias; const float* addvec; int ld_add;
  const char* resid; int ld_res; const float* silu_pre; int ld_silu;
  int Csplit, ldy1, ldy2, out_f32, out_nchw;
  int act; char* ypre; int ldpre;
  float* gst;
  float* wgb;
  float* gsk;
  int M;
  int OHW;
  float* sk;
  int sk_per;
  int x1_bytes, x2_bytes, w_bytes;
  int dtype_bytes;
  int reg_epi;
  int gn_G; float gn_eps;
};

DMC_DEV int src_pixel(const ConvK& a, int n, int oy, int ox, int tap) {
  const int tr = tap / a.tkw;
  int iy = oy * a.stride + a.tdy0 + a.tsy * tr;
  int ix = ox * a.stride + a.tdx0 + a.tsx * (tap - tr * a.tkw);
  if (a.mode == DMC_MODE_UPSAMPLE) {
    if (iy < 0 || iy >= 2 * a.H || ix < 0 || ix >= 2 * a.W) return -1;
    iy >>= 1; ix >>= 1;
  } else if (a.mode == DMC_MODE_DILATE) {
    if (iy < 0 || ix < 0 || (iy & 1) || (ix & 1)) return -1;
    iy >>= 1; ix >>= 1;
    if (iy >= a.H || ix >= a.W) return -1;
  } else {
    if (iy < 0 || iy >= a.H || ix < 0 || ix >= a.W) return -1;
  }
  return (n * a.H + iy) * a.W + ix;
}

template <typename T>
DMC_DEV v4i load_act_chunk(const ConvK& a, int n, int sp, int c) {
  constexpr int EPC = TT<T>::KPL;
  v4i v = {0, 0, 0, 0};
  if (sp < 0) return v;
  const char* src;
  if (c < a.C1) src = a.x1 + ((size_t)sp * a.ld1 + c) * sizeof(T);
  else if (c < a.C1 + a.C2) src = a.x2 + ((size_t)sp * a.ld2 + (c - a.C1)) * sizeof(T);
  else return v;
  v = *(const v4i*)src;
  if (a.prologue != DMC_PRO_NONE) {
    float f[EPC];
    Chunk<T>::unpack(v, f);
    if (a.prologue == DMC_PRO_AFFINE_SILU) {
      const float* sc = a.psc + (size_t)n * a.ldp + c;
      const float* sh = a.psh + (size_t)n * a.ldp + c;
#pragma unroll
      for (int e = 0; e < EPC; ++e) f[e] = silu_f(fmaf(f[e], sc[e], sh[e]));
    } else if (a.prologue == DMC_PRO_AFFINE) {
      const float* sc = a.psc + (size_t)n * a.ldp + c;
      const float* sh = a.psh + (size_t)n * a.ldp + c;
#pragma unroll
      for (int e = 0; e < EPC; ++e) f[e] = fmaf(f[e], sc[e], sh[e]);
    } else {
#pragma unroll
      for (int e = 0; e < EPC; ++e) f[e] = silu_f(f[e]);
    }
    if (a.dthresh) {
      const uint64_t base = (uint64_t)sp * a.dld + c;
      const uint32_t seed = a.dseed + (a.dseed_base ? *a.dseed_base : 0u);
#pragma unroll
      for (int e = 0; e < EPC; ++e) f[e] = drop_keep(base + e, seed, a.dthresh) ? f[e] * a.dscale : 0.f;
    }
    v = Chunk<T>::pack(f);
  }
  return v;
}


DMC_DEV constexpr int waitcnt_vm(int n) { return (n & 15) | ((n >> 4) << 14) | (7 << 4) | (15 << 8); }
DMC_DEV constexpr int waitcnt_lgkm0() { return 15 | (3 << 14) | (7 << 4); }

constexpr unsigned kOOB = 0x80000000u;

DMC_DEV void wait_vm_dyn(int n) {
  switch (n) {
    case 0: __builtin_amdgcn_s_waitcnt(waitcnt_vm(0)); break;
    case 1: __builtin_amdgcn_s_waitcnt(waitcnt_vm(1)); break;
    case 2: __builtin_amdgcn_s_waitcnt(waitcnt_vm(2)); break;
    case 3: __builtin_amdgcn_s_waitcnt(waitcnt_vm(3)); break;
    case 4: __builtin_amdgcn_s_waitcnt(waitcnt_vm(4)); break;
    case 5: __builtin_amdgcn_s_waitcnt(waitcnt_vm(5)); break;
    case 6: __builtin_amdgcn_s_waitcnt(waitcnt_vm(6)); break;
    case 7: __builtin_amdgcn_s_waitcnt(waitcnt_vm(7)); break;
    case 8: __builtin_amdgcn_s_waitcnt(waitcnt_vm(8)); break;
    case 9: __builtin_amdgcn_s_waitcnt(waitcnt_vm(9)); break;
    default: __builtin_amdgcn_s_waitcnt(waitcnt_vm(10)); break;
  }
}

template <int N>
DMC_DEV void dma_pieces(const void* base, int nbytes, char* dst, const unsigned* off, unsigned add, int pb, int pe) {
  const __amdgpu_buffer_rsrc_t r = __builtin_amdgcn_make_buffer_rsrc((void*)base, (short)0, nbytes, 0x00020000);
#pragma unroll
  for (int p = 0; p < N; ++p)
// ... 1 lines not shown
      __builtin_amdgcn_raw_ptr_buffer_load_lds(r, (LDS_AS void*)(dst + p * 1024), 16, off[p] + add, 0, 0, 0);
}

bool same_size_3x3(const ConvK& k) {
  if (k.mode != DMC_MODE_NORMAL || k.stride != 1 || k.ntaps != 9 || k.tkw != 3) return false;
  if (!((k.tdy0 == -1 && k.tsy == 1) || (k.tdy0 == 1 && k.tsy == -1))) return false;
  if (!((k.tdx0 == -1 && k.tsx == 1) || (k.tdx0 == 1 && k.tsx == -1))) return false;
  return k.OH == k.H && k.OW == k.W;
}

int halo_plan(const ConvK& k, int* R, int* nimg, int maxhp = 7) {
  if (!same_size_3x3(k)) return 0;
  const int ohw = k.OH * k.OW;
  if (ohw % 256 == 0 && 256 % k.OW == 0) { *nimg = 1; *R = 256 / k.OW; }
  else if (256 % ohw == 0 && k.N % (256 / ohw) == 0) { *nimg = 256 / ohw; *R = k.OH; }
  else return 0;
  const int npix = *nimg * (*R + 2) * (k.OW + 2);
  return npix <= 6 * 64 ? 6 : npix <= 7 * 64 ? 7 : (maxhp >= 9 && npix <= 9 * 64) ? 9 : 0;
}

int halo2_plan(const ConvK& k, int* R, int* nimg) {
  if (!same_size_3x3(k)) return 0;
  const int ohw = k.OH * k.OW;
  if (ohw % 128 == 0 && 128 % k.OW == 0) { *nimg = 1; *R = 128 / k.OW; }
  else if (128 % ohw == 0 && k.N % (128 / ohw) == 0) { *nimg = 128 / ohw; *R = k.OH; }
  else return 0;
  const int npix = *nimg * (*R + 2) * (k.OW + 2);
  return npix <= 6 * 32 ? 6 : npix <= 7 * 32 ? 7 : npix <= 9 * 32 ? 9 : 0;
}


int fill_convk(const dmc_conv_desc* d, const void* x1, const void* x2, const void* w, void* y1, void* y2,
               ConvK& k) {
  DMC_REQUIRE(d->dtype == DMC_F32 || d->dtype == DMC_BF16, "conv: bad dtype %d", d->dtype);
  const int epc = d->dtype == DMC_F32 ? 4 : 8;
  const int bk = d->dtype == DMC_F32 ? 32 : 64;
  DMC_REQUIRE((d->C1 % epc == 0 || (d->C2 == 0 && d->prologue == DMC_PRO_NONE && d->ld1 >= (d->C1 + epc - 1) / epc * epc)) &&
                  d->C2 % epc == 0,
              "conv: C1/C2 (%d,%d) must be multiples of %d", d->C1, d->C2, epc);
  DMC_REQUIRE(d->Kc % bk == 0 && d->Kc >= d->C1 + d->C2, "conv: Kc %d must be a multiple of %d and >= C1+C2", d->Kc, bk);
  DMC_REQUIRE(d->ntaps >= 1 && d->ntaps <= 16, "conv: ntaps %d", d->ntaps);
  DMC_REQUIRE(d->ld1 % epc == 0 && (d->C2 == 0 || d->ld2 % epc == 0), "conv: source pitch alignment");
  DMC_REQUIRE(d->Csplit >= 0 && d->Csplit <= d->Cout && (d->Csplit == d->Cout || d->Csplit % 4 == 0),
              "conv: Csplit %d", d->Csplit);
  k.x1 = (const char*)x1; k.x2 = (const char*)x2; k.w = (const char*)w; k.y1 = (char*)y1; k.y2 = (char*)y2;
  k.dtype_bytes = d->dtype == DMC_F32 ? 4 : 2;
  k.N = d->N; k.H = d->H; k.W = d->W; k.C1 = d->C1; k.C2 = d->C2; k.ld1 = d->ld1; k.ld2 = d->ld2; k.Kc = d->Kc;
  k.OH = d->OH; k.OW = d->OW; k.Cout = d->Cout; k.ntaps = d->ntaps; k.mode = d->mode; k.stride = d->stride;
  {
    int kw = 1;
    while (kw < d->ntaps && d->tap_dy[kw] == d->tap_dy[0]) ++kw;
    k.tkw = kw;
    k.tdy0 = d->tap_dy[0]; k.tdx0 = d->tap_dx[0];
    k.tsx = kw > 1 ? d->tap_dx[1] - d->tap_dx[0] : 1;
    k.tsy = d->ntaps > kw ? d->tap_dy[kw] - d->tap_dy[0] : 1;
    bool ok = d->ntaps % kw == 0;
    for (int t = 0; ok && t < d->ntaps; ++t)
      ok = d->tap_dy[t] == k.tdy0 + k.tsy * (t / kw) && d->tap_dx[t] == k.tdx0 + k.tsx * (t % kw);
    DMC_REQUIRE(ok, "conv: taps must form a regular grid");
  }
  k.prologue = d->prologue; k.psc = d->pro_scale; k.psh = d->pro_shift; k.ldp = d->ld_pro;
  k.gn_G = d->pro_groups; k.gn_eps = d->pro_eps;
  DMC_REQUIRE(d->prologue != DMC_PRO_GN_SILU || (d->pro_groups > 0 && d->drop_thresh == 0 && d->pro_scale && d->pro_shift),
              "conv: DMC_PRO_GN_SILU needs pro_groups, gamma / beta and no dropout");
  k.dseed = d->drop_seed; k.dthresh = d->drop_thresh; k.dscale = d->drop_scale; k.dld = d->drop_ld;
  k.dseed_base = d->drop_seed_base;
  k.bias = d->bias; k.addvec = d->addvec; k.ld_add = d->ld_add; k.resid = (const char*)d->resid; k.ld_res = d->ld_res;
  k.silu_pre = d->silu_pre; k.ld_silu = d->ld_silu;
  k.Csplit = d->Csplit; k.ldy1 = d->ldy1; k.ldy2 = d->ldy2; k.out_f32 = d->out_f32; k.out_nchw = d->out_nchw;
  DMC_REQUIRE(d->act == DMC_ACT_NONE ||
                  ((d->act >= DMC_ACT_GELU && d->act <= DMC_ACT_DGELU) && d->Csplit == d->Cout && !d->out_nchw &&
                   !d->silu_pre && d->Cout % 4 == 0 && (!d->y_pre || d->ld_pre % 4 == 0)),
              "conv: act %d needs a single NHWC output, Cout %% 4 == 0, no silu'", d->act);
  DMC_REQUIRE((d->act != DMC_ACT_GELU_DROP && d->act != DMC_ACT_DGELU) || d->prologue == DMC_PRO_NONE,
              "conv: the GELU-dropout epilogues use the drop_* fields, so no prologue");
  DMC_REQUIRE(d->act != DMC_ACT_DGELU || d->y_pre, "conv: DGELU reads the pre-activation y_pre");
  k.act = d->act; k.ypre = (char*)d->y_pre; k.ldpre = d->ld_pre;
  k.gst = nullptr;
  k.wgb = nullptr;
  k.gsk = nullptr;
  k.reg_epi = (int)dmc::opt(dmc::OPT_REG_EPI);
  k.M = d->N * d->OH * d->OW; k.OHW = d->OH * d->OW;
  k.sk = nullptr; k.sk_per = 0;
  {
    const size_t esz = d->dtype == DMC_F32 ? 4 : 2;
    const size_t b1 = (size_t)d->N * d->H * d->W * d->ld1 * esz;
    const size_t b2 = d->C2 ? (size_t)d->N * d->H * d->W * d->ld2 * esz : 0;
    const size_t bw = (size_t)d->Cout * d->ntaps * d->Kc * esz;
    const size_t lim = 0x7fff0000u;
    k.x1_bytes = b1 < lim ? (int)b1 : 0;
    k.x2_bytes = b2 < lim ? (int)b2 : 0;
    k.w_bytes = bw < lim ? (int)bw : 0;
  }
  return 0;
}

}
```

### diffusion_models_collection_amd/csrc/dmc_elem.hip

```cpp
#include <stdlib.h>
#include <string.h>
#include "dmc_common.h"
#include "dmc_internal.h"

namespace dmc {
static thread_local char g_err[512] = "";
void set_error(const char* fmt, ...) {
  va_list ap;
  va_start(ap, fmt);
  vsnprintf(g_err, sizeof(g_err), fmt, ap);
  va_end(ap);
}
}

namespace dmc {
namespace {
struct OptDef {
  const char* name;
  long def;
};
constexpr OptDef kOpts[OPT_COUNT] = {
    {"DMC_NO_NARROW", 0}, {"DMC_NO_GLDS", 0}, {"DMC_NO_SPLITK", 0}, {"DMC_NO_BUFLDS", 0}, {"DMC_NO_HALO", 0},
    {"DMC_HALO_PRO", 1}, {"DMC_GN_STATS_SPLIT", 0}, {"DMC_GN_BWD_SPLIT", 0}, {"DMC_ATTN_STAGED", 0},
    {"DMC_ATTN_HG", 0}, {"DMC_WG_BLOCKS", 512}, {"DMC_GN_STATS_ONE_MAX", 1l << 20}, {"DMC_GN_BWD_ONE_MAX", 65536},
    {"DMC_NO_XCD", 0}, {"DMC_NO_EPI_STATS", 0}, {"DMC_WG_MINPIX", 0}, {"DMC_GN_BWD_SLICES", 2}, {"DMC_NO_SKGN", 0},
    {"DMC_WG_HALO_TARGET", 256}, {"DMC_SK_TARGET", 240}, {"DMC_SK_MAX", 8}, {"DMC_NO_NHALO", 0},
    {"DMC_GN_BWD_FUSED", 4}, {"DMC_GN_BWD_FUSED_MAXHW", 1l << 30}, {"DMC_GN_BWD_NT", 1024},
    {"DMC_REG_EPI", 3}, {"DMC_GEMM1X1", 1}, {"DMC_WG_PIPE", 1}, {"DMC_IMG_MASK", 15}, {"DMC_IMG_GN", 1}, {"DMC_WG_IMG4", 1},
};
struct OptTable {
  long v[OPT_COUNT];
  OptTable() { reset(true); }
  void reset(bool env) {
    for (int i = 0; i < OPT_COUNT; ++i) {
      v[i] = kOpts[i].def;
      const char* e = env ? getenv(kOpts[i].name) : nullptr;
      if (e && e[0]) v[i] = atol(e);
    }
  }
};
OptTable& table() {
  static OptTable t;
  return t;
}
}
long opt(Opt o) { return table().v[o]; }
}

extern "C" int dmc_set_option(const char* name, long value) {
  for (int i = 0; i < dmc::OPT_COUNT; ++i)
    if (strcmp(name, dmc::kOpts[i].name) == 0) {
      dmc::table().v[i] = value;
      return 0;
    }
  dmc::set_error("set_option: unknown option %s", name);
  return 1;
}
extern "C" long dmc_get_option(const char* name) {
  for (int i = 0; i < dmc::OPT_COUNT; ++i)
    if (strcmp(name, dmc::kOpts[i].name) == 0) return dmc::table().v[i];
  return -1;
}
extern "C" void dmc_reset_options(int from_env) { dmc::table().reset(from_env != 0); }

extern "C" int dmc_version(void) { return 1; }
extern "C" const char* dmc_last_error(void) { return dmc::g_err; }

namespace {

inline int grid_for(long n, int block = 256, int cap = 8192) {
  long b = (n + block - 1) / block;
  if (b < 1) b = 1;
  return (int)(b < cap ? b : cap);
}

__global__ void time_embed_kernel(const int64_t* t, int B, int dim, float* out) {
  const int half = dim / 2;
  const float e = (float)(9.210340371976184 / (double)(half - 1));
  const int total = B * half;
  for (int i = blockIdx.x * blockDim.x + threadIdx.x; i < total; i += gridDim.x * blockDim.x) {
    const int b = i / half, k = i % half;
    const float f = expf((float)k * -e);
    const float a = (float)t[b] * f;
    out[(size_t)b * dim + k] = sinf(a);
    out[(size_t)b * dim + half + k] = cosf(a);
  }
}

__global__ void embed_fwd_kernel(const int64_t* y, int B, int rows, const float* table, int dim, float* out) {
  const int total = B * dim;
  for (int i = blockIdx.x * blockDim.x + threadIdx.x; i < total; i += gridDim.x * blockDim.x) {
    const int b = i / dim, d = i % dim;
    long yy = y[b];
    yy = yy < 0 ? 0 : (yy > rows - 1 ? rows - 1 : yy);
    out[i] = table[(size_t)yy * dim + d];
  }
}

__global__ void embed_bwd_kernel(const int64_t* y, int B, int rows, const float* dout, int dim, float* dtable) {
  const int total = rows * dim;
  for (int i = blockIdx.x * blockDim.x + threadIdx.x; i < total; i += gridDim.x * blockDim.x) {
    const int r = i / dim, d = i % dim;
    float s = 0.f;
    if (r != 0) {
      for (int b = 0; b < B; ++b) {
        long yy = y[b];
        yy = yy < 0 ? 0 : (yy > rows - 1 ? rows - 1 : yy);
        if (yy == r) s += dout[(size_t)b * dim + d];
      }
    }
    dtable[i] = s;
// ... 909 lines not shown
```

### diffusion_models_collection_amd/csrc/dmc_internal.h

```cpp
#pragma once
#include <hip/hip_runtime.h>
#include <stdarg.h>
#include <stdio.h>
#include "dmc.h"

namespace dmc {
void set_error(const char* fmt, ...);
inline hipStream_t as_stream(void* s) { return (hipStream_t)s; }
inline int check_launch(const char* what) {
  hipError_t e = hipGetLastError();
  if (e != hipSuccess) {
    set_error("%s: launch failed: %s", what, hipGetErrorString(e));
    return 2;
  }
  return 0;
}
inline int cdiv(long a, long b) { return (int)((a + b - 1) / b); }
}

namespace dmc {
enum Opt {
  OPT_NO_NARROW, OPT_NO_GLDS, OPT_NO_SPLITK, OPT_NO_BUFLDS, OPT_NO_HALO, OPT_HALO_PRO, OPT_GN_STATS_SPLIT,
  OPT_GN_BWD_SPLIT, OPT_ATTN_STAGED, OPT_ATTN_HG, OPT_WG_BLOCKS, OPT_GN_STATS_ONE_MAX, OPT_GN_BWD_ONE_MAX,
  OPT_NO_XCD, OPT_NO_EPI_STATS, OPT_WG_MINPIX, OPT_GN_BWD_SLICES, OPT_NO_SKGN, OPT_WG_HALO_TARGET, OPT_SK_TARGET,
  OPT_SK_MAX, OPT_NO_NHALO, OPT_GN_BWD_FUSED, OPT_GN_BWD_FUSED_MAXHW, OPT_GN_BWD_NT,
  OPT_REG_EPI, OPT_GEMM1X1, OPT_WG_PIPE, OPT_IMG_MASK, OPT_IMG_GN, OPT_WG_IMG4, OPT_COUNT
};
long opt(Opt o);
}

#define DMC_REQUIRE(cond, ...)       \
  do {                               \
    if (!(cond)) {                   \
      dmc::set_error(__VA_ARGS__);   \
      return 1;                      \
    }                                \
  } while (0)
```

### diffusion_models_collection_amd/kernels.py

```python
import ctypes

import torch

from . import _lib as L
from ._lib import LIB, check, ptr

TAPS3 = [(kh - 1, kw - 1) for kh in range(3) for kw in range(3)]
TAPS3_DGRAD = [(1 - kh, 1 - kw) for kh in range(3) for kw in range(3)]
TAPS1 = [(0, 0)]
TAPS_UPDGRAD = [(u - 1, v - 1) for u in range(4) for v in range(4)]


class Scratch:

    def __init__(self):
        self.bufs = {}

    def get(self, nbytes: int, device) -> torch.Tensor:
        nbytes = max(int(nbytes), 256)
        key = L.stream()
        buf = self.bufs.get(key)
        if buf is None or buf.numel() < nbytes:
            buf = torch.empty(int(nbytes * 1.25) + 4096, dtype=torch.uint8, device=device)
            self.bufs[key] = buf
# ... 32 lines not shown
    d.ld_pro = ld
    d.drop_seed, d.drop_seed_base, d.drop_thresh, d.drop_scale = drop_args(drop)
    d.drop_ld = drop_ld if drop is not None else 0


def set_epilogue(d, bias=None, addvec=None, ld_add=0, resid=None, ld_res=0, silu_pre=None, ld_silu=0,
                 ldy1=0, ldy2=0, Csplit=None, out_f32=False, out_nchw=False, act=L.ACT_NONE, y_pre=None, ld_pre=0,
                 gn_part=None):
    d._keep_epi = (bias, addvec, resid, silu_pre, y_pre, gn_part)
    d.gn_part = ptr(gn_part)
    d.act = act
    d.y_pre = ptr(y_pre)
    d.ld_pre = ld_pre
    d.bias = ptr(bias)
    d.addvec = ptr(addvec)
    d.ld_add = ld_add
    d.resid = ptr(resid)
    d.ld_res = ld_res
    d.silu_pre = ptr(silu_pre)
    d.ld_silu = ld_silu
    d.ldy1, d.ldy2 = ldy1, ldy2
    d.Csplit = d.Cout if Csplit is None else Csplit
    d.out_f32 = int(out_f32)
    d.out_nchw = int(out_nchw)


class LayerProfile:

    def __init__(self):
        import os
        self.on = os.environ.get("DMC_LAYER_PROF", "0") not in ("", "0")
        self.pending = []

    def wrap(self, kind, d, fn):
        if not self.on:
            return fn()
        e0, e1 = torch.cuda.Event(enable_timing=True), torch.cuda.Event(enable_timing=True)
        e0.record()
        fn()
        e1.record()
        M = d.N * d.OH * d.OW
        key = (kind, d.dtype, d.N, d.H, d.W, d.C1 + d.C2, d.OH, d.OW, d.Cout, d.ntaps, d.mode)
        self.pending.append((key, 2.0 * M * d.Cout * d.ntaps * (d.C1 + d.C2), e0, e1))

    def report(self, steps=1):
        torch.cuda.synchronize()
        agg = {}
        for key, fl, e0, e1 in self.pending:
            a = agg.setdefault(key, [0, 0.0, 0.0])
            a[0] += 1
            a[1] += e0.elapsed_time(e1)
            a[2] += fl
        self.pending = []
        rows = sorted(agg.items(), key=lambda kv: -kv[1][1])
        tot = sum(v[1] for v in agg.values())
        lines = [f"conv launches: {tot / steps:.3f} ms/step"]
        for (kind, dt, N, H, W, Cin, OH, OW, Cout, nt, mode), (n, ms, fl) in rows:
            lines.append(f"{ms / steps * 1e3:8.1f} us/step  n/step {n / steps:4.1f}  avg {ms / n * 1e3:7.1f} us  "
                         f"{fl / (ms * 1e-3) / 1e12:7.1f} TF/s  {kind:5s} N{N} {H}x{W}x{Cin} -> {OH}x{OW}x{Cout} "
                         f"taps {nt} mode {mode}")
        return "\n".join(lines)


PROF = LayerProfile()


def conv(d, x1, x2, w, y1, y2=None):
    nbytes = LIB.dmc_conv2d_workspace(ctypes.byref(d))
    ws = SCRATCH.get(nbytes, y1.device) if nbytes else None
    PROF.wrap("conv", d, lambda: check(LIB.dmc_conv2d(ctypes.byref(d), ptr(x1), ptr(x2), ptr(w), ptr(y1), ptr(y2),
                                                      ptr(ws), nbytes, L.stream()), "dmc_conv2d"))


def conv_fused(d):
    return LIB.dmc_conv2d_fused_epilogue(ctypes.byref(d), LIB.dmc_conv2d_workspace(ctypes.byref(d)))


def conv_plan(d, ws_bytes=None):
    if ws_bytes is None:
        ws_bytes = LIB.dmc_conv2d_workspace(ctypes.byref(d))
    p = L.ConvPlan()
    check(LIB.dmc_conv2d_plan(ctypes.byref(d), ws_bytes, ctypes.byref(p)), "dmc_conv2d_plan")
    return p


def upsample2x(dtype, x, C):
    N, H, W, ld = x.shape
    y = torch.empty(N, 2 * H, 2 * W, C, dtype=x.dtype, device=x.device)
    check(LIB.dmc_upsample2x_nhwc(L.dtype_code(dtype), ptr(x), N, H, W, C, ld, ptr(y), C, L.stream()),
          "dmc_upsample2x_nhwc")
    return y


def conv_halo_prologue(d):
    return bool(LIB.dmc_conv_halo_prologue(ctypes.byref(d)))


def _byte_span(t):
    n = 1 + sum((sz - 1) * st for sz, st in zip(t.shape, t.stride())) if t.numel() else 0
    return t.data_ptr(), t.data_ptr() + n * t.element_size()


class WgradDefer:

    def __init__(self):
        import os
        self.every = int(os.environ.get("DMC_WG_FLUSH_EVERY", "3"))
        self.group = max(1, min(int(os.environ.get("DMC_WG_DEFER", "4") or 1), L.WGRAD_GROUP_MAX))
        self.arenas = []
        self.buf = None
        self.off = 0
        self.jobs = []
        self.pending = []
        self.pending_ow = 0
        self.pending1 = []

    def alloc(self, nbytes, device):
        nbytes = (max(int(nbytes), 256) + 255) // 256 * 256
        if self.buf is None or self.buf.device != device or self.off + nbytes > self.buf.numel():
            need = nbytes if self.buf is None or self.buf.device != device else self.off + nbytes
            self.flush()
            if self.buf is None or self.buf.device != device or need > self.buf.numel():
                self.buf = torch.empty(int(need * 1.25), dtype=torch.uint8, device=device)
                self.arenas.append(self.buf)
        ws = self.buf[self.off:self.off + nbytes]
        self.off += nbytes
        return ws

    def add(self, job):
        if job.splits == 0:
            return
        self.jobs.append(job)
        if self.every and len(self.jobs) >= self.every:
            self.flush()

    def flush(self):
        for k in range(0, len(self.jobs), 32):
            chunk = self.jobs[k:k + 32]
            arr = (L.WgradJob * len(chunk))(*chunk)
            check(LIB.dmc_wgrad_reduce_batch(arr, len(chunk), L.stream()), "dmc_wgrad_reduce_batch")
        self.jobs = []
        self.off = 0

    def group_add(self, item):
        if self.group <= 1:
            return False
        ow = LIB.dmc_conv2d_wgrad_group_ok(ctypes.byref(item[0]), item[2])
        if not ow:
            return False
        if ow == 1:
            self.pending1.append(item)
            if len(self.pending1) >= self.group:
                items, self.pending1 = self.pending1, []
                wgrad_group(items, defer=self)
            return True
        if self.pending and ow != self.pending_ow:
            self.launch_pending()
        self.pending.append(item)
        self.pending_ow = ow
        if len(self.pending) >= self.group:
            self.launch_pending()
        return True

    def holds(self, t):
        lo, hi = _byte_span(t)
        for it in self.pending + self.pending1:
# ... 8 lines not shown
        for items in (self.pending, self.pending1):
            if items:
                batch = items[:]
                del items[:]
                wgrad_group(batch, defer=self)

    def end_segment(self):
        self.launch_pending()
        self.flush()

    def reset(self):
        self.jobs = []
        self.pending = []
        self.pending1 = []
        self.off = 0


def wgrad_slab_bytes(reset=False):
    return LIB.dmc_wgrad_slab_bytes(int(reset))


def wgrad_plan(d, ld_dy):
    p = L.WgradPlan()
    check(LIB.dmc_conv2d_wgrad_plan(ctypes.byref(d), ld_dy, ctypes.byref(p)), "dmc_conv2d_wgrad_plan")
    return p


def wgrad_group(items, defer=None):
    n = len(items)
    arr = (L.WgradGroupItem * n)()
    for i, (d, dy, ld_dy, x1, x2, dw, scale, dbias) in enumerate(items):
        d.wg_bias = ptr(dbias)
        d._keep_wgb = dbias
        arr[i].d = ctypes.pointer(d)
        arr[i].dy, arr[i].ld_dy, arr[i].x1, arr[i].x2 = ptr(dy), ld_dy, ptr(x1), ptr(x2)
        arr[i].dw, arr[i].scale = ptr(dw), scale
    sizes = (ctypes.c_size_t * n)()
    if not LIB.dmc_conv2d_wgrad_group_workspace(arr, n, sizes):
        raise L.DMCError("wgrad_group: the jobs are no valid group (bf16 stride-1 convs: 3x3 of one map width, or 1x1)")
    offs, total = [], 0
    for i in range(n):
        offs.append(total)
        total += (sizes[i] + 255) // 256 * 256
    dev = items[0][1].device
    ws = defer.alloc(total, dev) if defer is not None else SCRATCH.get(total, dev)
    for i in range(n):
        arr[i].workspace = ws.data_ptr() + offs[i]
    jobs = (L.WgradJob * n)()
    PROF.wrap("wgrad", items[0][0], lambda: check(LIB.dmc_conv2d_wgrad_group(arr, n, jobs, L.stream()),
                                                  "dmc_conv2d_wgrad_group"))
    if defer is not None:
        defer.jobs.extend(L.WgradJob.from_buffer_copy(jobs[i]) for i in range(n))
        if defer.every and len(defer.jobs) >= defer.every:
            defer.flush()
        return
    check(LIB.dmc_wgrad_reduce_batch(jobs, n, L.stream()), "dmc_wgrad_reduce_batch")


def wgrad(d, dy, ld_dy, x1, x2, dw, scale=1.0, dbias=None, defer=None):
    d.wg_bias = ptr(dbias)
    d._keep_wgb = dbias
    if defer is not None and defer.group_add((d, dy, ld_dy, x1, x2, dw, scale, dbias)):
        return
    nbytes = LIB.dmc_conv2d_wgrad_workspace(ctypes.byref(d))
    if defer is not None:
        ws = defer.alloc(nbytes, dy.device)
        job = L.WgradJob()
        PROF.wrap("wgrad", d, lambda: check(LIB.dmc_conv2d_wgrad_partial(
            ctypes.byref(d), ptr(dy), ld_dy, ptr(x1), ptr(x2), ptr(ws), ptr(dw), scale, ctypes.byref(job), L.stream()),
            "dmc_conv2d_wgrad_partial"))
        defer.add(job)
        return
    ws = SCRATCH.get(nbytes, dy.device)
    PROF.wrap("wgrad", d, lambda: check(LIB.dmc_conv2d_wgrad(ctypes.byref(d), ptr(dy), ld_dy, ptr(x1), ptr(x2), ptr(ws),
                                                             ptr(dw), scale, L.stream()), "dmc_conv2d_wgrad"))


def pack_weight(mode, dtype, w, Kc, out=None):
    w = w.detach()
    if w.dim() == 2:
        Cout, Cin, kh, kw = w.shape[0], w.shape[1], 1, 1
    else:
        Cout, Cin, kh, kw = w.shape
    ntaps = 16 if mode == L.PACK_UPDGRAD else kh * kw
    rows = Cout if mode == L.PACK_FWD else Cin
    if out is None:
        out = torch.empty(rows * ntaps * Kc, dtype=dtype, device=w.device)
    check(LIB.dmc_pack_weight(mode, L.dtype_code(dtype), ptr(w.contiguous()), Cout, Cin, kh, kw, Kc, ptr(out),
                              L.stream()), "dmc_pack_weight")
    return out


class PackBatch:

    def __init__(self, jobs, device):
        arr = (L.PackJob * len(jobs))()
        self.keep = []
        tiles = []
        for i, (w, dst, off, mode, Cout, Cin, kh, kw, Kc, koff) in enumerate(jobs):
            w = w.detach()
            if not w.is_contiguous():
                raise L.DMCError("pack job: master weight must be contiguous")
            self.keep.append(w)
            j = arr[i]
            j.w = w.data_ptr()
            j.dst = dst.data_ptr() + off * dst.element_size()
            j.dtype = L.dtype_code(dst.dtype)
            j.mode, j.Cout, j.Cin, j.kh, j.kw, j.Kc, j.koff = mode, Cout, Cin, kh, kw, Kc, koff
            n = LIB.dmc_pack_tiles(ctypes.byref(j), i, None, 0)
            buf = (ctypes.c_int * (3 * n))()
            LIB.dmc_pack_tiles(ctypes.byref(j), i, buf, n)
            tiles.append(torch.frombuffer(bytearray(buf), dtype=torch.int32))
        self.count = len(jobs)
        t = torch.cat(tiles)
        self.ntiles = t.numel() // 3
        self.jobs = torch.frombuffer(bytearray(arr), dtype=torch.uint8).to(device)
        self.tiles = t.to(device)

    def launch(self):
        check(LIB.dmc_pack_weights(ptr(self.jobs), ptr(self.tiles), self.ntiles, L.stream()), "dmc_pack_weights")


def gn_stats(dtype, x1, x2, N, HW, C1, C2, ld1, ld2, G, eps, gamma, beta):
    C = C1 + C2
    dev = x1.device
    mr = torch.empty(N * G * 2, dtype=torch.float32, device=dev)
    sc = torch.empty(N * C, dtype=torch.float32, device=dev)
    sh = torch.empty(N * C, dtype=torch.float32, device=dev)
    ws = SCRATCH.get(LIB.dmc_gn_workspace(N, C, G, HW), dev)
    check(LIB.dmc_gn_stats(L.dtype_code(dtype), ptr(x1), ptr(x2), N, HW, C1, C2, ld1, ld2, G, eps, ptr(gamma),
                           ptr(beta), ptr(ws), ptr(mr), ptr(sc), ptr(sh), L.stream()), "dmc_gn_stats")
    return sc, sh, mr


def gn_finalize(p1, C1, p2, C2, N, HW, G, eps, gamma, beta, out=None):
    dev = p1.device
    C = C1 + C2
    if out is None:
        out = (torch.empty(N * C, dtype=torch.float32, device=dev),
               torch.empty(N * C, dtype=torch.float32, device=dev),
               torch.empty(N * G * 2, dtype=torch.float32, device=dev))
    sc, sh, mr = out
    check(LIB.dmc_gn_finalize(ptr(p1), C1, ptr(p2), C2, N, HW, G, eps, ptr(gamma), ptr(beta), ptr(mr), ptr(sc),
                              ptr(sh), L.stream()), "dmc_gn_finalize")
    return sc, sh, mr


def gn_stats_apply_ok(dtype, N, HW, C1, C2, G):
    return bool(LIB.dmc_gn_stats_apply_ok(L.dtype_code(dtype), N, HW, C1, C2, G))


def gn_stats_apply(dtype, x1, x2, N, HW, C1, C2, ld1, ld2, G, eps, gamma, beta, silu=True, drop=None):
    C = C1 + C2
    dev = x1.device
    mr = torch.empty(N * G * 2, dtype=torch.float32, device=dev)
    sc = torch.empty(N * C, dtype=torch.float32, device=dev)
    sh = torch.empty(N * C, dtype=torch.float32, device=dev)
    out = torch.empty(N * HW * C, dtype=dtype, device=dev)
    seed, base, thresh, dscale = drop_args(drop)
    check(LIB.dmc_gn_stats_apply(L.dtype_code(dtype), ptr(x1), ptr(x2), N, HW, C1, C2, ld1, ld2, G, eps, ptr(gamma),
                                 ptr(beta), ptr(mr), ptr(sc), ptr(sh), int(silu), seed, base, thresh, dscale, ptr(out),
                                 C, L.stream()), "dmc_gn_stats_apply")
    return (sc, sh, mr), out


def gn_apply(dtype, x1, x2, N, HW, C1, C2, ld1, ld2, scale, shift, silu=True, drop=None, out=None):
    C = C1 + C2
    if out is None:
# ... 516 lines not shown
```

### diffusion_models_collection_amd/models/_unet_exec.py

```python
import contextlib
import ctypes
import math
import os
import weakref
from typing import List, Optional

import torch

from .. import _lib as L
from .. import kernels as K


class Act:

    __slots__ = ("t", "H", "W", "C", "grad", "part")

    def __init__(self, t, H, W, C):
        self.t, self.H, self.W, self.C = t, H, W, C
        self.grad = None
        self.part = None


_GN_PARTIALS = os.environ.get("DMC_GN_PARTIALS", "1") not in ("", "0")
_GN_DEFER = os.environ.get("DMC_GN_DEFER", "1") not in ("", "0")
# ... 22 lines not shown
            buf = e[1] if e is not None and e[2] == tuple(id(s) for s in srcs) else make_buf()
            jobs = make_jobs(buf)
            K.PackBatch(jobs, buf.device).launch()
            e = (v, buf, tuple(id(s) for s in srcs), srcs, jobs)
            self.entries[key] = e
        return e[1]

    def refresh(self):
        stale = []
        for k, e in self.entries.items():
            v = self._ver(e[3])
            if e[0] != v:
                stale.append((k, e, v))
        if not stale:
            return
        key = tuple((k, e[1].data_ptr(), v[1:]) for k, e, v in stale)
        if self._batch is None or self._batch[0] != tuple((k, b, tuple(p for _, p in vv)) for k, b, vv in key):
            jobs = [j for _, e, _ in stale for j in e[4]]
            self._batch = (tuple((k, b, tuple(p for _, p in vv)) for k, b, vv in key),
                           K.PackBatch(jobs, stale[0][1][1].device))
        self._batch[1].launch()
        for k, e, v in stale:
            self.entries[k] = (v,) + e[1:]


class ExecCore:

    def _setup(self, model):
        self._mref = weakref.ref(model)
        self.dt = model.compute_dtype
        self.cdt = L.dtype_code(self.dt)
        self.chunk = L.chunk_for(self.dt)
        self.wgen = 0
        self.packs = _PackCache(self)
        self.params = list(model.parameters())
        self.pindex = {id(p): i for i, p in enumerate(self.params)}
        self.training_grad_scale = 1.0
        self.grad_hook = None
        self.seed_ptr = None

    def _set_grad_order(self, order):
        assert len(order) == len(self.params) and {id(p) for p in order} == set(self.pindex), "gradient layout"
        self.goff = [0] * len(self.params)
        off = 0
        for p in order:
            self.goff[self.pindex[id(p)]] = off
            off += p.numel()
        self.gtotal = off

    def _grad_buffer(self, device):
        flat = getattr(self, "_flat", None)
        if flat is None or flat.device != device or any(p.grad is not None for p in self.params):
            flat = torch.empty(self.gtotal, dtype=torch.float32, device=device)
        self._flat = flat
        self.flat = flat
        return flat

    def run(self, x, t, y=None):
        need_grad = torch.is_grad_enabled() and (x.requires_grad or any(p.requires_grad for p in self.params))
        if need_grad:
            return _ExecFunction.apply(self, x, t, y, *self.params)
        out, _ = self.forward(x, t, y, keep=False)
        return out

    @property
    def m(self):
        m = self._mref()
        if m is None:
            raise RuntimeError("the model this executor ran has been freed")
        return m

    def _gview(self, flat, p):
        i = self.pindex[id(p)]
        o = self.goff[i]
        return flat[o:o + p.numel()].view(p.shape)

    def _wpack(self, conv, mode, Kc, dtype=None):
        dtype = dtype or self.dt
        w = conv.weight
        if w.dim() == 2:
            Cout, Cin, kh, kw = w.shape[0], w.shape[1], 1, 1
        else:
            Cout, Cin, kh, kw = w.shape
        ntaps = 16 if mode == L.PACK_UPDGRAD else kh * kw
        rows = Cout if mode == L.PACK_FWD else Cin

        def make_buf():
            return torch.empty(rows * ntaps * Kc, dtype=dtype, device=w.device)

        return self.packs.get((id(conv), mode, Kc, dtype), (w,), make_buf,
                              lambda buf: [(w, buf, 0, mode, Cout, Cin, kh, kw, Kc, -1)])

    def _conv(self, srcs, conv, taps, OH, OW, Cout, mode=L.MODE_NORMAL, stride=1, pro=None, drop=None,
              bias=None, addvec=None, ld_add=0, resid=None, out=None, out_f32=False, out_nchw=False,
              dtype=None, packmode=L.PACK_FWD, w=None, Kc=None, silu_pre=None, ld_silu=0, split=None,
              act=L.ACT_NONE, y_pre=None, stats=None):
        dtype = dtype or self.dt
        gn_part = None
        if (stats is not None and _GN_PARTIALS and dtype == torch.bfloat16 and (OH * OW) % 64 == 0 and Cout % 8 == 0
                and split is None and not out_nchw and not out_f32):
            gn_part = torch.empty(srcs[0].t.shape[0] * OH * OW // 64 * (Cout // 8) * 2, dtype=torch.float32,
                                  device=srcs[0].t.device)
            stats.part = gn_part
        a = srcs[0]
        C1 = a.C
        C2 = srcs[1].C if len(srcs) > 1 else 0
        ld1 = a.t.shape[-1]
        ld2 = srcs[1].t.shape[-1] if len(srcs) > 1 else 0
        N = a.t.shape[0]
        if Kc is None:
            Kc = L.kc_for(C1 + C2, dtype)
        if w is None:
            w = self._wpack(conv, packmode, Kc, dtype)
        d = K.make_desc(dtype, N, a.H, a.W, C1, C2, ld1, ld2, Kc, OH, OW, Cout, taps, mode, stride)
        if pro is not None:
            K.set_prologue(d, pro[0], pro[1], pro[2], C1 + C2, drop, C1 + C2)
            if pro[0] == L.PRO_GN_SILU:
                d.pro_groups, d.pro_eps = pro[3], pro[4]
        elif drop is not None:
            if act not in (L.ACT_GELU_DROP, L.ACT_DGELU):
                raise ValueError("dropout needs a prologue (or the GELU-dropout epilogue)")
            K.set_prologue(d, L.PRO_NONE, drop=drop)
        ldy2 = 0
        y2 = None
        if split is not None:
            (y1, ldy1), (y2, ldy2), csplit = split
        else:
            y1 = out
            ldy1 = 0 if out_nchw else out.shape[-1]
            csplit = None
        K.set_epilogue(d, bias=bias, addvec=addvec, ld_add=ld_add, resid=resid,
                       ld_res=(0 if resid is None or out_nchw else resid.shape[-1]), silu_pre=silu_pre,
                       ld_silu=ld_silu, ldy1=ldy1, ldy2=ldy2, Csplit=csplit, out_f32=out_f32, out_nchw=out_nchw,
                       act=act, y_pre=y_pre, ld_pre=0 if y_pre is None else y_pre.shape[-1], gn_part=gn_part)
        K.conv(d, a.t, srcs[1].t if len(srcs) > 1 else None, w, y1, y2)
        return d

    def _wgrad(self, srcs, dy, ld_dy, taps, OH, OW, Cout, dw, mode=L.MODE_NORMAL, stride=1, pro=None, drop=None,
               dtype=None, dbias=None):
        dtype = dtype or self.dt
        a = srcs[0]
        C1 = a.C
        C2 = srcs[1].C if len(srcs) > 1 else 0
        N = a.t.shape[0]
        Kc = L.kc_for(C1 + C2, dtype)
        d = K.make_desc(dtype, N, a.H, a.W, C1, C2, a.t.shape[-1], srcs[1].t.shape[-1] if len(srcs) > 1 else 0, Kc,
                        OH, OW, Cout, taps, mode, stride)
        if pro is not None:
            K.set_prologue(d, pro[0], pro[1], pro[2], C1 + C2, drop, C1 + C2)
        K.wgrad(d, dy, ld_dy, a.t, srcs[1].t if len(srcs) > 1 else None, dw, self.training_grad_scale, dbias=dbias,
                defer=getattr(self, "_wg_defer", None))

    def _new(self, N, H, W, C, dtype=None):
        return Act(torch.empty(N, H, W, C, dtype=dtype or self.dt, device=self.device), H, W, C)



class UNetExecutor(ExecCore):
    def __init__(self, model):
        self._setup(model)
        self._halo_pro_cache = {}
        self._gsa_cache = {}
        self.res_blocks = [mod for mod in model.modules() if type(mod).__name__ == "ResidualBlock"]
        self.temb_off = {}
        off = 0
        for rb in self.res_blocks:
            self.temb_off[id(rb)] = off
            off += rb.out_channels
        self.temb_total = off
        self._layout_grads()
        self.daddvec = None
        self.plan = []
        for block in model.down_blocks:
            for j, layer in enumerate(block):
                self.plan.append((layer, False, j == len(block) - 1))
        for layer in model.middle_block:
            if type(layer).__name__ != "Identity":
                self.plan.append((layer, False, False))
        for block in model.up_blocks:
            for j, layer in enumerate(block):
                self.plan.append((layer, j == 0, False))

    def _layout_grads(self):
        m = self.m
        rbs = [mod for mod in m.modules() if type(mod).__name__ == "ResidualBlock"]
        tail = [rb.time_mlp[1].weight for rb in rbs] + [rb.time_mlp[1].bias for rb in rbs]
        if m.num_classes is not None:
            tail += [rb.label_proj[1].weight for rb in rbs]
        last = list(m.input_conv.parameters())
        tail_ids = {id(p) for p in tail + last}
        head = [p for p in reversed(self.params) if id(p) not in tail_ids]
        self._set_grad_order(head + tail + last)
        self.temb_w_off = self.goff[self.pindex[id(tail[0])]]
        self.temb_b_off = self.goff[self.pindex[id(tail[len(rbs)])]]
        self.temb_l_off = self.goff[self.pindex[id(tail[2 * len(rbs)])]] if m.num_classes is not None else None

    def _temb_lins(self, which):
        return [(rb.time_mlp[1] if which == 0 else rb.label_proj[1]) for rb in self.res_blocks]

    def _temb_pack(self, which, dtype):
        lins = self._temb_lins(which)
        dim = lins[0].weight.shape[1]
        Kc = L.kc_for(dim, torch.float32)

        def jobs(buf):
            out, off = [], 0
            for lin in lins:
                co = lin.weight.shape[0]
                out.append((lin.weight, buf, off * Kc, L.PACK_FWD, co, dim, 1, 1, Kc, -1))
                off += co
            return out

        return self.packs.get(("temb", which), tuple(lin.weight for lin in lins),
                              lambda: torch.zeros(self.temb_total * Kc, dtype=torch.float32,
                                                  device=lins[0].weight.device), jobs)

    def _temb_pack_dgrad(self, which):
# ... 123 lines not shown
        if drop_on:
            p = float(m.dropout)
            self._drop = (min(int(round(p * 4294967296.0)), 4294967295), 1.0 / (1.0 - p) if p < 1 else 0.0)
            if self.seed_ptr is not None:
                self._seed_base = 0
            else:
                self._seed_base = _seed_from_torch()
        else:
            self._drop = None
        self._blk_idx = 0

        f32 = torch.float32
        te = m.time_embed
        mc = te[0].dim
        tdim = te[1].out_features
        Nt = t.shape[0]
        if Nt != N and not (Nt == 1 and not keep and (m.num_classes is None or y is None)):
            raise ValueError(f"UNet: t has {Nt} entries for a batch of {N}")
        e0 = torch.empty(Nt, mc, dtype=f32, device=x.device)
        K.time_embed(t, mc, e0)
        A0 = Act(e0.view(Nt, 1, 1, mc), 1, 1, mc)
        A1 = self._new(Nt, 1, 1, tdim, f32)
        self._conv([A0], te[1], K.TAPS1, 1, 1, tdim, bias=te[1].bias, out=A1.t, dtype=f32)
        A2 = self._new(Nt, 1, 1, tdim, f32)
        self._conv([A1], te[3], K.TAPS1, 1, 1, tdim, pro=(L.PRO_SILU, None, None), bias=te[3].bias, out=A2.t,
                   dtype=f32)
        Ay = None
        if m.num_classes is not None and y is not None:
            y = y.to(device=x.device, dtype=torch.long).contiguous()
            ye = torch.empty(N, tdim, dtype=f32, device=x.device)
            K.embed_fwd(y, m.label_embed.weight, ye)
            Ay = Act(ye.view(N, 1, 1, tdim), 1, 1, tdim)
        addvec = torch.empty(Nt, 1, 1, self.temb_total, dtype=f32, device=x.device)
        Kt = L.kc_for(tdim, f32)
        self._conv([A2], None, K.TAPS1, 1, 1, self.temb_total, pro=(L.PRO_SILU, None, None), bias=self._temb_bias(),
                   out=addvec, dtype=f32, w=self._temb_pack(0, f32), Kc=Kt)
        if Ay is not None:
            self._conv([Ay], None, K.TAPS1, 1, 1, self.temb_total, pro=(L.PRO_SILU, None, None), resid=addvec,
                       out=addvec, dtype=f32, w=self._temb_pack(1, f32), Kc=Kt)
        self.addvec = addvec
        self._ld_add = self.temb_total if Nt == N else 0
        if keep:
            tape.append(("temb", t, y, A0, A1, A2, Ay, addvec))

        ldx = (Cin + self.chunk - 1) // self.chunk * self.chunk
        xin = Act(K.pack_input(dt, x, ldx), H, W, Cin)
        h = self._new(N, H, W, m.model_channels)
        self._conv([xin], m.input_conv, K.TAPS3, H, W, m.model_channels, bias=m.input_conv.bias, out=h.t, stats=h)
        if keep:
            tape.append(("conv_in", xin, h, x.requires_grad))
        hs = [h]
        for i, (layer, cat, push) in enumerate(self.plan):
            srcs = [h, hs.pop()] if cat else [h]
            h = self._layer(srcs, layer, tape)
            if push:
                hs.append(h)
        gno, convo = m.output[0], m.output[2]
        sto = self._gn([h], gno)
        ao = self._apply([h], sto, silu=True)
        out = torch.empty(N, m.out_channels, H, W, dtype=f32, device=x.device)
        self._conv([ao], convo, K.TAPS3, H, W, m.out_channels, bias=convo.bias, out=out, out_f32=True, out_nchw=True)
        if keep:
            tape.append(("out", h, sto, ao))
        return out, tape

    def _layer(self, srcs, layer, tape):
        name = type(layer).__name__
        if name == "ResidualBlock":
            return self._res_fwd(srcs, layer, tape)
        if name == "AttentionBlock":
            return self._attn_fwd(srcs[0], layer, tape)
        if name == "Downsample":
            a = srcs[0]
            OH, OW = (a.H + 2 - 3) // 2 + 1, (a.W + 2 - 3) // 2 + 1
            out = self._new(a.t.shape[0], OH, OW, a.C)
            self._conv([a], layer.conv, K.TAPS3, OH, OW, a.C, stride=2, bias=layer.conv.bias, out=out.t, stats=out)
            if tape is not None:
                tape.append(("down", layer, a, out))
            return out
        if name == "Upsample":
            a = srcs[0]
            out = self._new(a.t.shape[0], 2 * a.H, 2 * a.W, a.C)
            self._conv([a], layer.conv, K.TAPS3, 2 * a.H, 2 * a.W, a.C, mode=L.MODE_UPSAMPLE, bias=layer.conv.bias,
                       out=out.t, stats=out)
            if tape is not None:
                tape.append(("up", layer, a, out))
            return out
        raise TypeError(f"unexpected layer {name}")

    def _res_fwd(self, srcs, rb, tape):
        a = srcs[0]
        N, H, W = a.t.shape[0], a.H, a.W
        Cout = rb.out_channels
        gn1, conv1, gn2, conv2 = rb.conv1[0], rb.conv1[2], rb.conv2[0], rb.conv2[3]
        h1 = self._new(N, H, W, Cout)
        off = self.temb_off[id(rb)]
        gn_in1 = tape is None and self._img_gn_ok(srcs, Cout, gn1)
        fused = None if gn_in1 else self._gn_apply_small(srcs, gn1, True)
        st1 = None if gn_in1 else fused[0] if fused else self._gn(srcs, gn1)
        if gn_in1:
            a1 = None
            self._conv(srcs, conv1, K.TAPS3, H, W, Cout, pro=(L.PRO_GN_SILU, gn1.weight, gn1.bias, gn1.num_groups,
                                                              gn1.eps), bias=conv1.bias,
                       addvec=self.addvec.view(self.addvec.shape[0], -1)[:, off:], ld_add=self._ld_add, out=h1.t, stats=h1)
        elif fused:
            a1 = fused[1]
            self._conv([a1], conv1, K.TAPS3, H, W, Cout, bias=conv1.bias,
                       addvec=self.addvec.view(self.addvec.shape[0], -1)[:, off:], ld_add=self._ld_add, out=h1.t, stats=h1)
        elif tape is None and self._halo_pro_ok(srcs, Cout, st1):
            a1 = None
            self._conv(srcs, conv1, K.TAPS3, H, W, Cout, pro=(L.PRO_AFFINE_SILU, st1[0], st1[1]), bias=conv1.bias,
                       addvec=self.addvec.view(self.addvec.shape[0], -1)[:, off:], ld_add=self._ld_add, out=h1.t, stats=h1)
        else:
            a1 = self._apply(srcs, st1, silu=True)
            self._conv([a1], conv1, K.TAPS3, H, W, Cout, bias=conv1.bias,
                       addvec=self.addvec.view(self.addvec.shape[0], -1)[:, off:], ld_add=self._ld_add, out=h1.t, stats=h1)
        if isinstance(rb.shortcut, torch.nn.Conv2d):
            s = torch.empty(N, H, W, Cout, dtype=self.dt, device=self.device)
            self._conv(srcs, rb.shortcut, K.TAPS1, H, W, Cout, bias=rb.shortcut.bias, out=s)
            resid = s
        else:
            resid = a.t
        drop = None
        if self._drop is not None:
            drop = ((self._seed_base + 7919 * self._blk_idx) & 0xFFFFFFFF, self._drop[0], self._drop[1])
            if self.seed_ptr is not None:
                drop = drop + (self.seed_ptr,)
        self._blk_idx += 1
        out = self._new(N, H, W, Cout)
        gn_in2 = tape is None and drop is None and self._img_gn_ok([h1], Cout, gn2)
        fused = None if gn_in2 else self._gn_apply_small([h1], gn2, True, drop)
        st2 = None if gn_in2 else fused[0] if fused else self._gn([h1], gn2)
        if gn_in2:
            a2 = None
            self._conv([h1], conv2, K.TAPS3, H, W, Cout, pro=(L.PRO_GN_SILU, gn2.weight, gn2.bias, gn2.num_groups,
                                                              gn2.eps), bias=conv2.bias, resid=resid, out=out.t, stats=out)
        elif fused:
            a2 = fused[1]
            self._conv([a2], conv2, K.TAPS3, H, W, Cout, bias=conv2.bias, resid=resid, out=out.t, stats=out)
        elif tape is None and drop is None and self._halo_pro_ok([h1], Cout, st2):
            a2 = None
            self._conv([h1], conv2, K.TAPS3, H, W, Cout, pro=(L.PRO_AFFINE_SILU, st2[0], st2[1]), bias=conv2.bias,
                       resid=resid, out=out.t, stats=out)
        else:
            a2 = self._apply([h1], st2, silu=True, drop=drop)
            self._conv([a2], conv2, K.TAPS3, H, W, Cout, bias=conv2.bias, resid=resid, out=out.t, stats=out)
        st1 = (st1, a1)
        st2 = (st2, a2)
        if tape is not None:
            tape.append(("res", rb, srcs, h1, st1, st2, drop, out))
        return out

    def _attn_fwd(self, a, ab, tape):
        N, H, W, C = a.t.shape[0], a.H, a.W, a.C
        Lq = H * W
        heads = ab.num_heads
        hd = C // heads
        qkv = self._new(N, H, W, 3 * C)
        fused = self._gn_apply_small([a], ab.norm, False)
        if fused:
            st, an = fused
        else:
            st = self._gn([a], ab.norm)
            an = self._apply([a], st, silu=False)
        self._conv([an], ab.qkv, K.TAPS1, H, W, 3 * C, bias=ab.qkv.bias, out=qkv.t)
        st = (st, an)
        o = self._new(N, H, W, C)
# ... 33 lines not shown
                last = ri == len(recs) - 1
                self._backward_record(rec, dout, gv)
                if kind == "conv_in" and rec[3]:
                    dx = self._dx
                if hook is not None:
                    for p in self._record_params(rec):
                        final[self.pindex[id(p)]] = True
                    while cursor < len(order) and final[order[cursor]]:
                        cursor += 1
                    hi = self.goff[order[cursor]] if cursor < len(order) else self.gtotal
                    if getattr(hook, "wants", None) is None or hook.wants(hi, last):
                        self._flush_gn()
                    hook(flat, hi, last)
            self._flush_gn()
        except BaseException:
            if self._wg_defer is not None:
                self._wg_defer.reset()
            raise
        finally:
            self._gn_defer = None
            self._wg_defer = None
        self.daddvec = None
        grads = [self._gview(flat, p) for p in self.params]
        return dx, grads

    def _record_params(self, rec):
        kind = rec[0]
        m = self.m
        if kind == "out":
            return list(m.output.parameters())
        if kind == "res":
            rb = rec[1]
            skip = {id(p) for p in rb.time_mlp.parameters()}
            if rb.label_proj is not None:
                skip |= {id(p) for p in rb.label_proj.parameters()}
            return [p for p in rb.parameters() if id(p) not in skip]
        if kind in ("attn", "down", "up"):
            return list(rec[1].parameters())
        if kind == "conv_in":
            return list(m.input_conv.parameters())
        ps = list(m.time_embed.parameters())
        if m.label_embed is not None:
            ps += list(m.label_embed.parameters())
        for rb in self.res_blocks:
            ps += list(rb.time_mlp.parameters())
            if rb.label_proj is not None:
                ps += list(rb.label_proj.parameters())
        return ps

    def _backward_record(self, rec, dout, gv):
        m = self.m
        dt = self.dt
        f32 = torch.float32
        kind = rec[0]
        if True:
            if kind == "out":
                _, h, (sc, sh, mr), ao = rec
                gno, convo = m.output[0], m.output[2]
                N, H, W = h.t.shape[0], h.H, h.W
                Co = m.out_channels
                ldo = (Co + self.chunk - 1) // self.chunk * self.chunk
                dy = K.pack_input(dt, dout.contiguous(), ldo)
                self._wgrad([ao], dy, ldo, K.TAPS3, H, W, Co, gv(convo.weight), dbias=gv(convo.bias))
                g = torch.empty(N, H, W, h.C, dtype=dt, device=dout.device)
                dya = Act(dy, H, W, Co)
                self._conv([dya], convo, K.TAPS3_DGRAD, H, W, h.C, out=g, packmode=L.PACK_DGRAD,
                           Kc=L.kc_for(Co, dt))
                buf, acc = self._grad_target(h)
                self._gn_bwd(dt, g, h.C, h.t, None, N, H * W, h.C, 0, h.t.shape[-1], 0, gno.num_groups, mr, gno.weight,
                         gno.bias, True, None, buf, None, h.C, 0, acc, 0, gv(gno.weight), gv(gno.bias))
            elif kind == "res":
                self._res_bwd(rec, gv)
            elif kind == "attn":
                self._attn_bwd(rec, gv)
            elif kind == "down":
                _, layer, a, out = rec
                N = a.t.shape[0]
                dy = out.grad
                self._wgrad([a], dy, out.C, K.TAPS3, out.H, out.W, out.C, gv(layer.conv.weight), stride=2,
                            dbias=gv(layer.conv.bias))
                buf, acc = self._grad_target(a)
                dya = Act(dy, out.H, out.W, out.C)
                self._conv([dya], layer.conv, K.TAPS3_DGRAD, a.H, a.W, a.C, mode=L.MODE_DILATE,
                           out=buf, resid=buf if acc else None, packmode=L.PACK_DGRAD)
            elif kind == "up":
                _, layer, a, out = rec
                N = a.t.shape[0]
                dy = out.grad
                if dt == torch.bfloat16:
                    up = K.upsample2x(dt, a.t, a.t.shape[-1])
                    self._wgrad([Act(up, 2 * a.H, 2 * a.W, a.C)], dy, out.C, K.TAPS3, out.H, out.W, out.C,
                                gv(layer.conv.weight), dbias=gv(layer.conv.bias))
                else:
                    self._wgrad([a], dy, out.C, K.TAPS3, out.H, out.W, out.C, gv(layer.conv.weight),
                                mode=L.MODE_UPSAMPLE, dbias=gv(layer.conv.bias))
                buf, acc = self._grad_target(a)
                dya = Act(dy, out.H, out.W, out.C)
                self._conv([dya], layer.conv, K.TAPS_UPDGRAD, a.H, a.W, a.C, stride=2, out=buf,
                           resid=buf if acc else None, packmode=L.PACK_UPDGRAD)
            elif kind == "conv_in":
                _, xin, h, xg = rec
                N = h.t.shape[0]
                dy = h.grad
                conv = m.input_conv
                self._wgrad([xin], dy, h.C, K.TAPS3, h.H, h.W, h.C, gv(conv.weight), dbias=gv(conv.bias))
                if xg:
                    ldx = xin.t.shape[-1]
                    g = torch.empty(N, h.H, h.W, ldx, dtype=dt, device=dout.device)
                    self._conv([Act(dy, h.H, h.W, h.C)], conv, K.TAPS3_DGRAD, h.H, h.W, xin.C, out=g,
                               packmode=L.PACK_DGRAD)
                    self._dx = K.unpack_output(dt, g, ldx, N, xin.C, h.H, h.W)
            elif kind == "temb":
                self._temb_bwd(rec, self.daddvec, gv)

    def _res_bwd(self, rec, gv):
        _, rb, srcs, h1, (st1, a1), (st2, a2), drop, out = rec
        dt = self.dt
        a = srcs[0]
        N, H, W = a.t.shape[0], a.H, a.W
        Cout = rb.out_channels
        C1 = a.C
        C2 = srcs[1].C if len(srcs) > 1 else 0
        gn1, conv1, gn2, conv2 = rb.conv1[0], rb.conv1[2], rb.conv2[0], rb.conv2[3]
        dout = out.grad
        HW = H * W
        short_add = None
        self._wgrad([a2], dout, Cout, K.TAPS3, H, W, Cout, gv(conv2.weight), dbias=gv(conv2.bias))
        g2 = torch.empty(N, H, W, Cout, dtype=dt, device=dout.device)
        self._conv([Act(dout, H, W, Cout)], conv2, K.TAPS3_DGRAD, H, W, Cout, out=g2, packmode=L.PACK_DGRAD)
        if isinstance(rb.shortcut, torch.nn.Conv2d):
            sc = rb.shortcut
            self._wgrad(srcs, dout, Cout, K.TAPS1, H, W, Cout, gv(sc.weight), dbias=gv(sc.bias))
            if len(srcs) == 1:
                buf, acc = self._grad_target(a)
                self._conv([Act(dout, H, W, Cout)], sc, K.TAPS1, H, W, C1, out=buf, resid=buf if acc else None,
                           packmode=L.PACK_DGRAD)
            else:
                b = srcs[1]
                b1, acc1 = self._grad_target(a)
                b2, acc2 = self._grad_target(b)
                if acc1 or acc2:
                    tmp = torch.empty(N, H, W, C1 + C2, dtype=dt, device=dout.device)
                    self._conv([Act(dout, H, W, Cout)], sc, K.TAPS1, H, W, C1 + C2, out=tmp, packmode=L.PACK_DGRAD)
                    self._scatter_add_concat(tmp, b1, acc1, b2, acc2, C1, C2)
                else:
                    self._conv([Act(dout, H, W, Cout)], sc, K.TAPS1, H, W, C1 + C2, packmode=L.PACK_DGRAD,
                               split=((b1, C1), (b2, C2), C1))
        else:
            if a.grad is None:
                a.grad = dout
            elif len(srcs) == 1:
                short_add = dout
            else:
                self._wg_before_write(a.grad)
                K.add_(dt, a.grad, dout)
        off = self.temb_off[id(rb)]
        if self.daddvec is None:
            self.daddvec = torch.empty(N, self.temb_total, dtype=torch.float32, device=dout.device)
        dh1 = torch.empty(N, H, W, Cout, dtype=dt, device=dout.device)
        self._gn_bwd(dt, g2, Cout, h1.t, None, N, HW, Cout, 0, Cout, 0, gn2.num_groups, st2[2], gn2.weight, gn2.bias, True,
                 drop, dh1, None, Cout, 0, 0, 0, gv(gn2.weight), gv(gn2.bias), dx_sum_nc=self.daddvec[:, off:],
                 ld_sum_nc=self.temb_total, dx_sum_c=gv(conv1.bias))
        self._wgrad([a1], dh1, Cout, K.TAPS3, H, W, Cout, gv(conv1.weight))
        g1 = torch.empty(N, H, W, C1 + C2, dtype=dt, device=dout.device)
        x2 = srcs[1].t if len(srcs) > 1 else None
        self._conv([Act(dh1, H, W, Cout)], conv1, K.TAPS3_DGRAD, H, W, C1 + C2, out=g1, packmode=L.PACK_DGRAD)
        b1, acc1 = self._grad_target(a)
# ... 168 lines not shown
```

### include/dmc.h

```cpp
#ifndef DMC_H
#define DMC_H
#include <stddef.h>
#include <stdint.h>
#ifdef __cplusplus
extern "C" {
#endif

enum { DMC_F32 = 0, DMC_BF16 = 1 };
enum { DMC_MODE_NORMAL = 0, DMC_MODE_UPSAMPLE = 1, DMC_MODE_DILATE = 2 };
enum { DMC_PRO_NONE = 0, DMC_PRO_AFFINE_SILU = 1, DMC_PRO_SILU = 2, DMC_PRO_AFFINE = 3, DMC_PRO_GN_SILU = 4 };
enum { DMC_LOSS_L1 = 0, DMC_LOSS_L2 = 1, DMC_LOSS_HUBER = 2 };
enum { DMC_PRED_EPS = 0, DMC_PRED_V = 1 };
#define DMC_OBJECTIVE_MAX_BLOCKS 64
enum { DMC_PACK_FWD = 0, DMC_PACK_DGRAD = 1, DMC_PACK_UPDGRAD = 2 };

int dmc_version(void);
const char* dmc_last_error(void);

int dmc_set_option(const char* name, long value);
long dmc_get_option(const char* name);
void dmc_reset_options(int from_env);

typedef struct dmc_conv_desc {
  int dtype;
  int N, H, W;
  int C1, C2, ld1, ld2;
  int Kc;
  int OH, OW, Cout;
  int ntaps, mode, stride;
  int tap_dy[16], tap_dx[16];
  int prologue;
  const float* pro_scale;
  const float* pro_shift;
  int ld_pro;
  uint32_t drop_seed;
  uint32_t drop_thresh;
  float drop_scale;
  int drop_ld;
  const uint32_t* drop_seed_base;
  const float* bias;
  const float* addvec;
  int ld_add;
  const void* resid;
  int ld_res;
  const float* silu_pre;
  int ld_silu;
  int Csplit;
  int ldy1, ldy2;
  int out_f32;
  int out_nchw;
  int act;
  void* y_pre;
  int ld_pre;
  float* gn_part;
  float* wg_bias;
  int pro_groups;
  float pro_eps;
} dmc_conv_desc;
enum { DMC_ACT_NONE = 0, DMC_ACT_GELU = 1, DMC_ACT_GELU_DROP = 2, DMC_ACT_DGELU = 3 };

size_t dmc_conv2d_workspace(const dmc_conv_desc* d);
int dmc_conv_halo_prologue(const dmc_conv_desc* d);
int dmc_conv2d_fused_epilogue(const dmc_conv_desc* d, size_t ws_bytes);
enum { DMC_FUSED_GN_STATS = 1 };
enum { DMC_CONV_NONE = 0,
       DMC_CONV_NIN_HALO = 1,
       DMC_CONV_NOUT_HALO = 2,
       DMC_CONV_NARROW_IN = 3,
       DMC_CONV_NARROW_OUT = 4,
       DMC_CONV_IMG = 5,
       DMC_CONV_GEMM1X1 = 6,
       DMC_CONV_HALO = 7,
       DMC_CONV_GLDS = 8,
       DMC_CONV_REG = 9 };
enum { DMC_GN_PART_NONE = 0,
       DMC_GN_PART_KERNEL = 1,
       DMC_GN_PART_SPLITK = 2,
       DMC_GN_PART_PASS = 3 };
typedef struct dmc_conv_plan {
  int family;
  unsigned grid[3];
  int block;
  int splits;
  int gn_part;
  int fused_prologue;
  size_t ws_bytes;
} dmc_conv_plan;
int dmc_conv2d_plan(const dmc_conv_desc* d, size_t ws_bytes, dmc_conv_plan* out);
int dmc_conv2d(const dmc_conv_desc* d, const void* x1, const void* x2, const void* w,
               void* y1, void* y2, void* workspace, size_t ws_bytes, void* stream);

size_t dmc_conv2d_wgrad_workspace(const dmc_conv_desc* d);
int dmc_conv2d_wgrad(const dmc_conv_desc* d, const void* dy, int ld_dy, const void* x1,
                     const void* x2, void* workspace, float* dw, float scale, void* stream);
typedef struct dmc_wgrad_job {
  const float* slab;
  const float* bslab;
  float* dw;
  float* dbias;
  int splits, KK, Cpad, Cout, Ctot, ntaps, Kc;
  float scale;
  int layout;
} dmc_wgrad_job;
int dmc_conv2d_wgrad_partial(const dmc_conv_desc* d, const void* dy, int ld_dy, const void* x1, const void* x2,
                             void* workspace, float* dw, float scale, dmc_wgrad_job* job, void* stream);
int dmc_wgrad_reduce_batch(const dmc_wgrad_job* jobs, int njobs, void* stream);
enum { DMC_WGRAD_IMG4 = 1,
       DMC_WGRAD_PIPE = 2,
       DMC_WGRAD_HALO = 3,
       DMC_WGRAD_GEMM1X1 = 4,
       DMC_WGRAD_GENERIC = 5 };
typedef struct dmc_wgrad_plan {
  int kind;
  unsigned grid[3];
  int block;
  int splits;
  int layout;
  int group_kind;
  size_t ws_bytes;
} dmc_wgrad_plan;
int dmc_conv2d_wgrad_plan(const dmc_conv_desc* d, int ld_dy, dmc_wgrad_plan* out);

#define DMC_WGRAD_GROUP_MAX 8
typedef struct dmc_wgrad_group_item {
  const dmc_conv_desc* d;
  const void* dy;
  int ld_dy;
  const void* x1;
  const void* x2;
  void* workspace;
  float* dw;
  float scale;
} dmc_wgrad_group_item;
int dmc_conv2d_wgrad_group_ok(const dmc_conv_desc* d, int ld_dy);
size_t dmc_conv2d_wgrad_group_workspace(const dmc_wgrad_group_item* items, int njobs, size_t* bytes);
int dmc_conv2d_wgrad_group(const dmc_wgrad_group_item* items, int njobs, dmc_wgrad_job* jobs, void* stream);
long dmc_wgrad_slab_bytes(int reset);

int dmc_pack_weight(int pack_mode, int dtype, const float* w, int Cout, int Cin, int kh, int kw,
                    int Kc, void* dst, void* stream);
typedef struct dmc_pack_job {
  const float* w;
  void* dst;
  int dtype, mode, Cout, Cin, kh, kw, Kc, koff;
} dmc_pack_job;
int dmc_pack_tiles(const dmc_pack_job* job, int job_index, int* tiles, int cap);
int dmc_pack_weights(const dmc_pack_job* jobs, const int* tiles, int ntiles, void* stream);

size_t dmc_gn_workspace(int N, int C, int G, int HW);
int dmc_gn_stats(int dtype, const void* x1, const void* x2, int N, int HW, int C1, int C2, int ld1,
                 int ld2, int G, float eps, const float* gamma, const float* beta, void* workspace,
                 float* mean_rstd, float* scale, float* shift, void* stream);

int dmc_gn_finalize(const float* part1, int C1, const float* part2, int C2, int N, int HW, int G, float eps,
                    const float* gamma, const float* beta, float* mean_rstd, float* scale, float* shift,
                    void* stream);

int dmc_gn_apply(int dtype, const void* x1, const void* x2, int N, int HW, int C1, int C2, int ld1,
                 int ld2, const float* scale, const float* shift, int silu, uint32_t drop_seed,
                 const uint32_t* drop_seed_base, uint32_t drop_thresh, float drop_scale, void* out, int ld_out,
                 void* stream);

int dmc_gn_stats_apply_ok(int dtype, int N, int HW, int C1, int C2, int G);
int dmc_gn_stats_apply(int dtype, const void* x1, const void* x2, int N, int HW, int C1, int C2, int ld1, int ld2,
                       int G, float eps, const float* gamma, const float* beta, float* mean_rstd, float* scale,
                       float* shift, int silu, uint32_t drop_seed, const uint32_t* drop_seed_base,
                       uint32_t drop_thresh, float drop_scale, void* out, int ld_out, void* stream);

int dmc_gn_silu_bwd(int dtype, const void* g, int ld_g, const void* x1, const void* x2, int N,
                    int HW, int C1, int C2, int ld1, int ld2, int G, const float* mean_rstd,
                    const float* gamma, const float* beta, int silu, uint32_t drop_seed,
// ... 161 lines not shown
```

Before: 11950 img/s.

## Fold upsample conv and downsample dgrad into per-parity sub-pixel convolutions

Replaces the nearest-upsample followed by a 3x3 conv with four parity classes of 2x2 convolutions on the low-resolution input, using pre-summed folded weights. The strided-downsample dgrad (dilated conv) is likewise split into four parity classes with 1, 2, 2 and 4 taps. Both cut MAC count and skip reads of zero or duplicated pixels. In exchange it adds new weight-pack modes, scattered output and GroupNorm-segment indexing, and a new glds kernel variant with a per-class z grid. It also removes the SK_MAX option.

```diff
diff --git a/diffusion_models_collection_amd/_lib.py b/diffusion_models_collection_amd/_lib.py
--- a/diffusion_models_collection_amd/_lib.py
+++ b/diffusion_models_collection_amd/_lib.py
@@ -13,7 +13,9 @@
 LOSS = {"l1": 0, "l2": 1, "huber": 2}
 PRED = {"eps": 0, "v": 1}
 OBJECTIVE_MAX_BLOCKS = 64
-PACK_FWD, PACK_DGRAD, PACK_UPDGRAD = 0, 1, 2
+PACK_FWD, PACK_DGRAD, PACK_UPDGRAD, PACK_UPFOLD, PACK_DOWNDGRAD = 0, 1, 2, 3, 4
+FOLD_NONE, FOLD_UP, FOLD_DOWN_DGRAD = 0, 1, 2
+FOLD_PACK = {FOLD_UP: PACK_UPFOLD, FOLD_DOWN_DGRAD: PACK_DOWNDGRAD}
 
 _c_int, _c_p, _c_f, _c_u32, _c_long, _c_size = (ctypes.c_int, ctypes.c_void_p, ctypes.c_float, ctypes.c_uint32,
                                                 ctypes.c_long, ctypes.c_size_t)
@@ -36,6 +38,7 @@
         ("silu_pre", _c_p), ("ld_silu", _c_int), ("Csplit", _c_int), ("ldy1", _c_int), ("ldy2", _c_int),
         ("out_f32", _c_int), ("out_nchw", _c_int), ("act", _c_int), ("y_pre", _c_p), ("ld_pre", _c_int),
         ("gn_part", _c_p), ("wg_bias", _c_p), ("pro_groups", _c_int), ("pro_eps", _c_f),
+        ("fold", _c_int),
     ]
 
 
@@ -102,6 +105,7 @@
         "dmc_conv2d_workspace": (_c_size, [ctypes.POINTER(ConvDesc)]),
         "dmc_conv_halo_prologue": (_c_int, [ctypes.POINTER(ConvDesc)]),
         "dmc_conv2d_fused_epilogue": (_c_int, [ctypes.POINTER(ConvDesc), ctypes.c_size_t]),
+        "dmc_conv_resample_fold": (_c_int, [ctypes.POINTER(ConvDesc), ctypes.c_size_t]),
         "dmc_conv2d_plan": (_c_int, [ctypes.POINTER(ConvDesc), ctypes.c_size_t, ctypes.POINTER(ConvPlan)]),
         "dmc_conv2d": (_c_int, [ctypes.POINTER(ConvDesc), _c_p, _c_p, _c_p, _c_p, _c_p, _c_p, _c_size, _c_p]),
         "dmc_conv2d_wgrad_workspace": (_c_size, [ctypes.POINTER(ConvDesc)]),
diff --git a/diffusion_models_collection_amd/csrc/dmc_conv.hip b/diffusion_models_collection_amd/csrc/dmc_conv.hip
--- a/diffusion_models_collection_amd/csrc/dmc_conv.hip
+++ b/diffusion_models_collection_amd/csrc/dmc_conv.hip
@@ -245,8 +245,8 @@
   m = 0.5f * (m + mb);
 }
 
-template <int BM, int BN, int NT>
-DMC_DEV void tile_epilogue8(const ConvK& a, const char* lds, int EP, int m0, int n0) {
+template <int BM, int BN, int NT, bool CLS = false>
+DMC_DEV void tile_epilogue8(const ConvK& a, const char* lds, int EP, int m0, int n0, int par = 0) {
   constexpr int CG = BN / 8, RS = NT / CG, IT = BM / RS;
   constexpr int SEG = 64, NSEG = BM / SEG, KPS = SEG / RS;
   static_assert((CG == 16 || CG == 8) && SEG % RS == 0 && BM % SEG == 0, "GroupNorm partial geometry");
@@ -266,7 +266,8 @@
 #pragma unroll
     for (int k = 0; k < IT; ++k) {
       const int pix = min(m0 + r0 + k * RS, a.M - 1);
-      rr[k] = *(const v4i*)(a.resid + ((size_t)pix * a.ld_res + co) * 2);
+      const int po = CLS ? cls_out_pixel(a, par, pix) : pix;
+      rr[k] = *(const v4i*)(a.resid + ((size_t)po * a.ld_res + co) * 2);
     }
   }
   int n = (m0 + r0) / a.OHW, nend = (n + 1) * a.OHW;
@@ -320,7 +321,8 @@
         }
       }
       const v4i out = Chunk<bf16_t>::pack(f);
-      *(v4i*)(y + ((size_t)pix * ldy + cy) * 2) = out;
+      const int po = CLS ? cls_out_pixel(a, par, pix) : pix;
+      *(v4i*)(y + ((size_t)po * ldy + cy) * 2) = out;
       if (a.gst) {
         float g[8];
         Chunk<bf16_t>::unpack(out, g);
@@ -377,15 +379,20 @@
         m += d * (nb / (na + nb));
         q += qb + d * d * (na * nb / (na + nb));
       }
-      const size_t o = ((size_t)(m0 / SEG + j) * (a.Cout / 8) + (n0 / 8 + c)) * 2;
+      const int seg = CLS ? cls_out_seg(a, par, m0 / SEG + j) : m0 / SEG + j;
+      const size_t o = ((size_t)seg * (a.Cout / 8) + (n0 / 8 + c)) * 2;
       a.gst[o] = m;
       a.gst[o + 1] = q;
     }
   }
 }
 
-template <typename T, int BM, int BN, int NT>
-DMC_DEV void tile_epilogue(const ConvK& a, const char* lds, int EP, int m0, int n0) {
+template <typename T, int BM, int BN, int NT, bool CLS = false>
+DMC_DEV void tile_epilogue(const ConvK& a, const char* lds, int EP, int m0, int n0, int par = 0) {
+  if constexpr (CLS) {
+    tile_epilogue8<BM, BN, NT, true>(a, lds, EP, m0, n0, par);
+    return;
+  }
   constexpr int CG = BN / 4, RS = NT / CG;
   const int cg = threadIdx.x % CG, r0 = threadIdx.x / CG;
   const int co = n0 + cg * 4;
@@ -485,7 +492,8 @@
          a.act == DMC_ACT_NONE && (a.Cout & 127) == 0 && (a.ldy1 & 7) == 0 &&
          (!a.resid || (a.ld_res & 7) == 0) && (a.M & 127) == 0 && (!a.gst || a.OHW % 64 == 0);
 }
-DMC_DEV void reg_epilogue(const ConvK& a, v4f (&acc)[4][4], int m0, int n0, int wm, int wn) {
+template <bool CLS = false>
+DMC_DEV void reg_epilogue(const ConvK& a, v4f (&acc)[4][4], int m0, int n0, int wm, int wn, int par = 0) {
   const int lane = threadIdx.x & 63, fr = lane & 15, fh = lane >> 4;
   const bool odd = fh & 1;
   v4i rra[4][2];
@@ -499,7 +507,8 @@
     for (int jp = 0; jp < 2; ++jp) {
       rra[i][jp] = v4i{0, 0, 0, 0};
       if (a.resid) {
-        const int px = m0 + wm * 64 + (2 * jp + (odd ? 1 : 0)) * 16 + fr;
+        const int pc = m0 + wm * 64 + (2 * jp + (odd ? 1 : 0)) * 16 + fr;
+        const int px = CLS ? cls_out_pixel(a, par, pc) : pc;
         rra[i][jp] = *(const v4i*)(a.resid + ((size_t)px * a.ld_res + cc) * 2);
       }
     }
@@ -561,7 +570,8 @@
       v4i outv;
       if (!odd) { outv[0] = o[0][0]; outv[1] = o[0][1]; outv[2] = recv[0]; outv[3] = recv[1]; }
       else { outv[0] = recv[0]; outv[1] = recv[1]; outv[2] = o[1][0]; outv[3] = o[1][1]; }
-      const int pxs = m0 + wm * 64 + (2 * jp + (odd ? 1 : 0)) * 16 + fr;
+      const int pcs = m0 + wm * 64 + (2 * jp + (odd ? 1 : 0)) * 16 + fr;
+      const int pxs = CLS ? cls_out_pixel(a, par, pcs) : pcs;
       *(v4i*)(a.y1 + ((size_t)pxs * a.ldy1 + cc) * 2) = outv;
     }
     if (a.gst) {
@@ -573,7 +583,8 @@
         cnt *= 2.f;
       }
       if (fr == 0 && !odd) {
-        const size_t o = ((size_t)((m0 + wm * 64) / 64) * (a.Cout / 8) + cc / 8) * 2;
+        const int seg = CLS ? cls_out_seg(a, par, (m0 + wm * 64) / 64) : (m0 + wm * 64) / 64;
+        const size_t o = ((size_t)seg * (a.Cout / 8) + cc / 8) * 2;
         a.gst[o] = gm;
         a.gst[o + 1] = gq;
       }
@@ -581,9 +592,11 @@
   }
 }
 
-template <int WM, int WN, bool BUF, int STAGES = 3>
+template <int WM, int WN, bool BUF, int STAGES = 3, bool CLS = false>
 __global__ __launch_bounds__(WM * WN * 64) void conv_fwd_glds_kernel(ConvK a) {
   using T = bf16_t;
+  const int par = CLS ? 3 - (int)blockIdx.z : 0;
+  const ConvCls cq = CLS ? cls_select(a, par) : ConvCls{a.ntaps, a.tkw, a.tdy0, a.tdx0, a.tsy, a.tsx, 0};
   constexpr int NW = WM * WN;
   constexpr int BM = 64 * WM, BN = 64 * WN;
   constexpr int SB = (BM + BN) * 128;
@@ -598,7 +611,7 @@
   const int wave = __builtin_amdgcn_readfirstlane(threadIdx.x >> 6);
   const int wm = wave % WM, wn = wave / WM;
   int mb = blockIdx.x, nb = blockIdx.y;
-  if (!a.sk && gridDim.y == 1) xcd_tile((a.Cout + BN - 1) / BN, mb, nb);
+  if ((CLS || !a.sk) && gridDim.y == 1) xcd_tile((a.Cout + BN - 1) / BN, mb, nb);
   const int m0 = mb * BM;
   const int n0 = nb * BN;
   const int lrow = lane >> 3;
@@ -617,7 +630,7 @@
       pn[j] = -1; poy[j] = 0; pox[j] = 0;
     }
   }
-  const int nstages = a.ntaps * (a.Kc / 64);
+  const int nstages = cq.ntaps * (a.Kc / 64);
 
   v4f acc[4][4];
 #pragma unroll
@@ -625,25 +638,26 @@
 #pragma unroll
     for (int j = 0; j < 4; ++j) acc[i][j] = v4f{0.f, 0.f, 0.f, 0.f};
 
-  const int s_begin = a.sk ? blockIdx.z * a.sk_per : 0;
-  const int s_end = a.sk ? min(nstages, s_begin + a.sk_per) : nstages;
+  const int s_begin = (!CLS && a.sk) ? blockIdx.z * a.sk_per : 0;
+  const int s_end = (!CLS && a.sk) ? min(nstages, s_begin + a.sk_per) : nstages;
   const int ns = s_end - s_begin;
   const int kst = a.Kc / 64;
   int is_tap = s_begin / kst, is_c0 = (s_begin - is_tap * kst) * 64;
   int sp[AI];
   unsigned o1[AI], o2[AI], ob[BI];
   if constexpr (BUF) {
-    const unsigned wrow = (unsigned)(a.ntaps * a.Kc);
+    const unsigned wrow = (unsigned)(cq.ntaps * a.Kc);
 #pragma unroll
     for (int j = 0; j < BI; ++j) {
       const int co = n0 + (wave * BI + j) * 8 + lrow;
-      ob[j] = co < a.Cout ? ((unsigned)co * wrow + lc * 8) * 2u : kOOB;
+      ob[j] = co < a.Cout ? (unsigned)cq.woff + ((unsigned)co * wrow + lc * 8) * 2u : kOOB;
     }
   }
   auto tap_rows = [&]() {
 #pragma unroll
     for (int j = 0; j < AI; ++j) {
-      const int p = pn[j] >= 0 ? src_pixel(a, pn[j], poy[j], pox[j], is_tap) : -1;
+      const int p = pn[j] < 0 ? -1 : CLS ? cls_src_pixel(a, cq, pn[j], poy[j], pox[j], is_tap)
+                                        : src_pixel(a, pn[j], poy[j], pox[j], is_tap);
       if constexpr (BUF) {
         o1[j] = p >= 0 ? ((unsigned)p * a.ld1 + lc * 8) * 2u : kOOB;
         o2[j] = p >= 0 ? ((unsigned)p * a.ld2 + lc * 8) * 2u : kOOB;
@@ -661,7 +675,7 @@
       glds_issue<AI, BI, BM>(a, base, (s_begin + S) * 64, is_c0, wave, lrow, lc, n0, sp);
     }
     is_c0 += 64;
-    if (is_c0 == a.Kc) { is_c0 = 0; ++is_tap; if (is_tap < a.ntaps) tap_rows(); }
+    if (is_c0 == a.Kc) { is_c0 = 0; ++is_tap; if (is_tap < cq.ntaps) tap_rows(); }
   };
 #define DMC_GLDS_ISSUE(S) issue(S)
   for (int q = 0; q < STAGES - 1 && q < ns; ++q) DMC_GLDS_ISSUE(q);
@@ -709,8 +723,8 @@
 #undef DMC_GLDS_ISSUE
   constexpr int EP = BN * 4 + 16;
   if constexpr (WM == 2 && WN == 2) {
-    if (!a.sk && reg_epi_ok(a) && n0 + BN <= a.Cout && m0 + BM <= a.M) {
-      reg_epilogue(a, acc, m0, n0, wm, wn);
+    if ((CLS || !a.sk) && reg_epi_ok(a) && n0 + BN <= a.Cout && m0 + BM <= a.M) {
+      reg_epilogue<CLS>(a, acc, m0, n0, wm, wn, par);
       return;
     }
   }
@@ -721,7 +735,7 @@
     for (int i = 0; i < 4; ++i)
       *(v4f*)(lds + (wm * 64 + j * 16 + fr) * EP + (wn * 64 + i * 16 + fh * 4) * 4) = acc[i][j];
   __syncthreads();
-  if (a.sk) {
+  if (!CLS && a.sk) {
     const int Cpad = gridDim.y * BN;
     float* slab = a.sk + (size_t)blockIdx.z * a.M * Cpad;
     for (int idx = threadIdx.x; idx < BM * BN / 4; idx += NW * 64) {
@@ -730,7 +744,7 @@
     }
     return;
   }
-  tile_epilogue<T, BM, BN, NW * 64>(a, lds, EP, m0, n0);
+  tile_epilogue<T, BM, BN, NW * 64, CLS>(a, lds, EP, m0, n0, par);
 }
 
 DMC_DEV void wait_vm_upto40(int n) {
@@ -1369,6 +1383,38 @@
          k.w_bytes > 0;
 }
 
+int fold_kind(const ConvK& k) {
+  if (k.dtype_bytes != 2 || k.prologue != DMC_PRO_NONE || !dma_operands_ok(k)) return DMC_FOLD_NONE;
+  if (k.ntaps != 9 || k.tkw != 3 || k.stride != 1 || k.OH != 2 * k.H || k.OW != 2 * k.W) return DMC_FOLD_NONE;
+  if (k.out_f32 || k.out_nchw || k.silu_pre || k.addvec || k.act != DMC_ACT_NONE || k.Csplit != k.Cout ||
+      ((k.Cout | k.ldy1 | k.ld_res) & 7) || (long)k.N * k.OH * k.OW >= (1l << 31))
+    return DMC_FOLD_NONE;
+  if (k.mode == DMC_MODE_UPSAMPLE && k.tdy0 == -1 && k.tsy == 1 && k.tdx0 == -1 && k.tsx == 1)
+    return ((long)k.Cout * 16 * k.Kc * 2 < 0x7fff0000l && (k.H * k.W) % 64 == 0) ? DMC_FOLD_UP : DMC_FOLD_NONE;
+  if (k.mode == DMC_MODE_DILATE && k.tdy0 == 1 && k.tsy == -1 && k.tdx0 == 1 && k.tsx == -1) return DMC_FOLD_DOWN_DGRAD;
+  return DMC_FOLD_NONE;
+}
+
+void set_fold(ConvK& k, int kind) {
+  int base = 0;
+  for (int c = 0; c < 4; ++c) {
+    ConvCls q{};
+    const int a = c >> 1, b = c & 1;
+    if (kind == DMC_FOLD_UP) {
+      q.ntaps = 4; q.tkw = 2; q.tdy0 = a - 1; q.tdx0 = b - 1; q.tsy = 1; q.tsx = 1;
+    } else {
+      q.tkw = b ? 2 : 1; q.ntaps = (a ? 2 : 1) * q.tkw; q.tdy0 = a; q.tdx0 = b; q.tsy = -1; q.tsx = -1;
+    }
+    k.cls[c] = cls_pack(q, base);
+    base += q.ntaps;
+  }
+  k.w_bytes = base * k.Cout * k.Kc * 2;
+  k.ncls = 4;
+  k.mode = DMC_MODE_NORMAL;
+  k.OH = k.H; k.OW = k.W; k.OHW = k.H * k.W; k.M = k.N * k.OHW;
+  k.ntaps = 4;
+}
+
 int img_plan(const ConvK& k, long mask) {
   if (!mask || k.dtype_bytes != 2 || (k.prologue != DMC_PRO_NONE && k.prologue != DMC_PRO_GN_SILU)) return 0;
   if (k.prologue == DMC_PRO_GN_SILU) {
@@ -1771,10 +1817,28 @@
   }
 }
 
+DMC_DEV int fold_lo(int par, int r) { return r == 0 ? 0 : par ? 2 : 1; }
+DMC_DEV int fold_hi(int par, int r) { return r == 0 ? (par ? 1 : 0) : 2; }
+DMC_DEV float fold_sum(const float* w9, int a, int b, int r, int c) {
+  float v = 0.f;
+  for (int ky = fold_lo(a, r); ky <= fold_hi(a, r); ++ky)
+    for (int kx = fold_lo(b, c); kx <= fold_hi(b, c); ++kx) v += w9[ky * 3 + kx];
+  return v;
+}
+DMC_DEV int down_ntaps(int cls) { return cls == 0 ? 1 : cls == 3 ? 4 : 2; }
+DMC_DEV int down_base(int cls) { return cls == 0 ? 0 : cls == 1 ? 1 : cls == 2 ? 3 : 5; }
+
 DMC_DEV float pack_value(int mode, const float* w, int Cout, int Cin, int kh, int kw, int row, int t, int k) {
   if (mode == DMC_PACK_FWD) return k < Cin ? w[((size_t)row * Cin + k) * kh * kw + t] : 0.f;
+  if (mode == DMC_PACK_UPFOLD)
+    return k < Cin ? fold_sum(w + ((size_t)row * Cin + k) * 9, t >> 3, (t >> 2) & 1, (t >> 1) & 1, t & 1) : 0.f;
   if (k >= Cout) return 0.f;
   if (mode == DMC_PACK_DGRAD) return w[((size_t)k * Cin + row) * kh * kw + t];
+  if (mode == DMC_PACK_DOWNDGRAD) {
+    const int a = t >> 3, b = (t >> 2) & 1, tt = t & 3, ntx = b ? 2 : 1;
+    const int ky = a ? 2 * (tt / ntx) : 1, kx = b ? 2 * (tt % ntx) : 1;
+    return w[((size_t)k * Cin + row) * 9 + ky * 3 + kx];
+  }
   const int u = t >> 2, vv = t & 3;
   const int khs[4][2] = {{2, -1}, {1, 2}, {0, 1}, {0, -1}};
   const float* base = w + ((size_t)k * Cin + row) * 9;
@@ -1793,13 +1857,23 @@
 
 template <typename T>
 __global__ void pack_weight_kernel(int mode, const float* w, int Cout, int Cin, int kh, int kw, int Kc, T* dst) {
-  const int ntaps = (mode == DMC_PACK_UPDGRAD) ? 16 : kh * kw;
-  const int rows = (mode == DMC_PACK_FWD) ? Cout : Cin;
+  const int ntaps = (mode == DMC_PACK_UPDGRAD || mode == DMC_PACK_UPFOLD) ? 16 : kh * kw;
+  const int rows = (mode == DMC_PACK_FWD || mode == DMC_PACK_UPFOLD) ? Cout : Cin;
   const long total = (long)rows * ntaps * Kc;
   for (long o = blockIdx.x * (long)blockDim.x + threadIdx.x; o < total; o += (long)gridDim.x * blockDim.x) {
     const int k = o % Kc;
     const long r = o / Kc;
-    const float v = pack_value(mode, w, Cout, Cin, kh, kw, r / ntaps, r % ntaps, k);
+    float v;
+    if (mode == DMC_PACK_UPFOLD) {
+      const int cls = (int)(r / (4l * rows));
+      v = pack_value(mode, w, Cout, Cin, kh, kw, (int)(r / 4 % rows), cls * 4 + (int)(r % 4), k);
+    } else if (mode == DMC_PACK_DOWNDGRAD) {
+      const int cls = r < rows ? 0 : r < 3l * rows ? 1 : r < 5l * rows ? 2 : 3;
+      const int nt = down_ntaps(cls), r2 = (int)(r - (long)down_base(cls) * rows);
+      v = pack_value(mode, w, Cout, Cin, kh, kw, r2 / nt, cls * 4 + r2 % nt, k);
+    } else {
+      v = pack_value(mode, w, Cout, Cin, kh, kw, r / ntaps, r % ntaps, k);
+    }
     if (sizeof(T) == 4) ((float*)dst)[o] = v;
     else ((bf16_t*)dst)[o] = (bf16_t)f2bf(v);
   }
@@ -1822,7 +1896,7 @@
     if (f32) ((float*)J.dst)[di] = v;
     else ((bf16_t*)J.dst)[di] = (bf16_t)f2bf(v);
   };
-  if (J.mode == DMC_PACK_FWD) {
+  if (J.mode == DMC_PACK_FWD || J.mode == DMC_PACK_UPFOLD) {
     const int co0 = tl[1], k0 = tl[2];
     const int nco = min(kPackFwdCo, J.Cout - co0);
     const int KW = J.koff >= 0 ? J.Cin : J.Kc;
@@ -1845,6 +1919,15 @@
           if (r < nco && tid + u * 256 < run) sw[r * kPackFwdK * 9 + tid + u * 256] = v[r][u];
     }
     __syncthreads();
+    if (J.mode == DMC_PACK_UPFOLD) {
+      for (int r = 0; r < nco; ++r)
+        for (int ct = 0; ct < 16; ++ct)
+          for (int k = tid; k < kn; k += 256) {
+            const float v = k < kv ? fold_sum(sw + r * kPackFwdK * 9 + k * 9, ct >> 3, (ct >> 2) & 1, (ct >> 1) & 1, ct & 1) : 0.f;
+            store((((long)(ct >> 2) * J.Cout + co0 + r) * 4 + (ct & 3)) * J.Kc + koff + k0 + k, v);
+          }
+      return;
+    }
     if (!f32 && ((J.Kc | koff | k0 | kn) & 1) == 0) {
       for (int r = 0; r < nco; ++r)
         for (int t = 0; t < khkw; ++t)
@@ -1885,11 +1968,16 @@
   }
   __syncthreads();
   const int ntaps = J.mode == DMC_PACK_UPDGRAD ? 16 : khkw;
+  auto drow = [&](int c, int t) -> long {
+    if (J.mode != DMC_PACK_DOWNDGRAD) return (long)c * ntaps + t;
+    const int ky = t / 3, kx = t - ky * 3, a = ky != 1, b = kx != 1, ntx = b ? 2 : 1, cls = a * 2 + b;
+    return (long)down_base(cls) * J.Cin + (long)c * down_ntaps(cls) + (ky >> 1) * ntx + (kx >> 1);
+  };
   auto value = [&](int co, int c, int t) {
     float v = 0.f;
     if (co < cov) {
       const float* wp = sw + co * kPackDgP + c * khkw;
-      if (J.mode == DMC_PACK_DGRAD) {
+      if (J.mode == DMC_PACK_DGRAD || J.mode == DMC_PACK_DOWNDGRAD) {
         v = wp[t];
       } else {
         const int u = t >> 2, vv = t & 3;
@@ -1911,7 +1999,7 @@
     for (int q = 2 * wv + (ln >> 5); q < cn * ntaps; q += 8) {
       const int c = q / ntaps, t = q - c * ntaps;
       if (cp >= con) continue;
-      *(uint32_t*)((bf16_t*)J.dst + ((long)(c0 + c) * ntaps + t) * J.Kc + koff + co0 + cp) =
+      *(uint32_t*)((bf16_t*)J.dst + drow(c0 + c, t) * J.Kc + koff + co0 + cp) =
           f2bf2(value(cp, c, t), value(cp + 1, c, t));
     }
     return;
@@ -1920,7 +2008,7 @@
   for (int q = wv; q < cn * ntaps; q += 4) {
     const int c = q / ntaps, t = q - c * ntaps;
     if (co >= con) continue;
-    store(((long)(c0 + c) * ntaps + t) * J.Kc + koff + co0 + co, value(co, c, t));
+    store(drow(c0 + c, t) * J.Kc + koff + co0 + co, value(co, c, t));
   }
 }
 
@@ -1931,6 +2019,8 @@
   int per;
   size_t ws;
 };
+
+constexpr int kSplitCap = 8;
 
 FwdPlan plan_glds(const ConvK& k) {
   FwdPlan p{0, 1, 0, 0};
@@ -1944,7 +2034,7 @@
   int sp = (int)((target + blocks - 1) / blocks);
   const int maxs = nst / 4;
   if (sp > maxs) sp = maxs;
-  if (sp > dmc::opt(dmc::OPT_SK_MAX)) sp = (int)dmc::opt(dmc::OPT_SK_MAX);
+  if (sp > kSplitCap) sp = kSplitCap;
   if (sp >= 2) {
     p.splits = sp;
     p.per = (nst + sp - 1) / sp;
@@ -2025,6 +2115,7 @@
   int tpb = 0;
   int wm = 2, stages = 3;
   bool buf = false;
+  bool cls = false;
   int tile = 64;
   int splits = 1, per = 0;
   bool fused_pro = false;
@@ -2142,6 +2233,32 @@
   } else {
     p.grid = dim3(dmc::cdiv(k.M, 64), dmc::cdiv(k.Cout, 64));
   }
+  return p;
+}
+
+int plan_fold(const ConvK& k, size_t ws_avail) {
+  const long o = dmc::opt(dmc::OPT_RESAMPLE_FOLD);
+  const int kind = fold_kind(k);
+  if (!kind || o == 0 || (o == 2 && kind != DMC_FOLD_UP) || (o == 3 && kind != DMC_FOLD_DOWN_DGRAD)) return DMC_FOLD_NONE;
+  if (dmc::opt(dmc::OPT_NO_GLDS) || dmc::opt(dmc::OPT_NO_BUFLDS)) return DMC_FOLD_NONE;
+  const FwdPlan gp = plan_glds(k);
+  if (gp.splits > 1 && ws_avail >= gp.ws && !dmc::opt(dmc::OPT_NO_SPLITK)) return DMC_FOLD_NONE;
+  return kind;
+}
+
+ConvPlan plan_folded(const ConvK& k, bool want_gn_part) {
+  ConvPlan p;
+  if (k.M == 0 || k.Cout == 0) return p;
+  p.family = DMC_CONV_GLDS; p.buf = true; p.cls = true;
+  const int nb128 = dmc::cdiv(k.Cout, 128);
+  const long blocks = 4l * dmc::cdiv(k.M, 128) * nb128;
+  int bm = 128;
+  if (blocks < 120) { bm = 64; p.wm = 1; p.block = 128; }
+  else if (blocks > 256) p.stages = 2;
+  p.grid = dmc::opt(dmc::OPT_NO_XCD) ? dim3(dmc::cdiv(k.M, bm), nb128, 4) : dim3(dmc::cdiv(k.M, bm) * nb128, 1, 4);
+  const bool epi = want_gn_part && k.Cout % 128 == 0 && k.M % 128 == 0 && k.OHW % 64 == 0 &&
+                   !dmc::opt(dmc::OPT_NO_EPI_STATS);
+  p.gn = !want_gn_part ? DMC_GN_PART_NONE : epi ? DMC_GN_PART_KERNEL : DMC_GN_PART_PASS;
   return p;
 }
 
@@ -2194,7 +2311,11 @@
       }
       break;
     case DMC_CONV_GLDS:
-      if (p.wm == 1) {
+      if (p.cls) {
+        if (p.wm == 1) conv_fwd_glds_kernel<1, 2, true, 3, true><<<g, 128, 0, s>>>(k);
+        else if (p.stages == 2) conv_fwd_glds_kernel<2, 2, true, 2, true><<<g, 256, 0, s>>>(k);
+        else conv_fwd_glds_kernel<2, 2, true, 3, true><<<g, 256, 0, s>>>(k);
+      } else if (p.wm == 1) {
         if (p.buf) conv_fwd_glds_kernel<1, 2, true><<<g, 128, 0, s>>>(k);
         else conv_fwd_glds_kernel<1, 2, false><<<g, 128, 0, s>>>(k);
       } else if (p.stages == 2) {
@@ -2226,7 +2347,7 @@
   }
   const int rc = dmc::check_launch("dmc_conv2d");
   if (rc || p.gn != DMC_GN_PART_PASS) return rc;
-  const int nseg = k.M / 64, nch = k.Cout / 8;
+  const int nseg = (p.cls ? 4 : 1) * (k.M / 64), nch = k.Cout / 8;
   const int blocks = (int)(((long)nseg * nch + 3) / 4);
   if (k.out_f32 || k.dtype_bytes == 4) gn_part_kernel<float><<<blocks, 256, 0, s>>>(k.y1, k.ldy1, nseg, nch, part);
   else gn_part_kernel<bf16_t><<<blocks, 256, 0, s>>>(k.y1, k.ldy1, nseg, nch, part);
@@ -2237,6 +2358,12 @@
   if (k.M != 0 && k.Cout != 0 && d->gn_part)
     DMC_REQUIRE(k.OHW % 64 == 0 && k.Cout % 8 == 0 && k.Csplit == k.Cout && !k.out_nchw && k.ldy1 % 4 == 0,
                 "conv: GroupNorm partials need OH*OW %% 64 == 0, Cout %% 8 == 0 and one NHWC output");
+  if (d->fold != DMC_FOLD_NONE) {
+    DMC_REQUIRE(d->fold == fold_kind(k), "conv: fold %d does not apply (dmc_conv_resample_fold says which does)", d->fold);
+    set_fold(k, d->fold);
+    p = plan_folded(k, d->gn_part != nullptr);
+    return 0;
+  }
   p = plan_conv(k, d->gn_part != nullptr, ws_avail);
   DMC_REQUIRE(p.family == DMC_CONV_NONE || k.prologue != DMC_PRO_GN_SILU || p.fused_pro,
               "conv: DMC_PRO_GN_SILU is taken only by the small-map conv (dmc_conv_halo_prologue says when)");
@@ -2248,12 +2375,24 @@
 extern "C" size_t dmc_conv2d_workspace(const dmc_conv_desc* d) {
   ConvK k;
   if (fill_convk(d, nullptr, nullptr, nullptr, nullptr, nullptr, k)) return 0;
+  if (d->fold != DMC_FOLD_NONE) return 0;
   return plan_conv(k, false, 0).ws_report;
+}
+
+extern "C" int dmc_conv_resample_fold(const dmc_conv_desc* d, size_t ws_bytes) {
+  ConvK k;
+  if (d == nullptr || d->fold != DMC_FOLD_NONE || fill_convk(d, nullptr, nullptr, nullptr, nullptr, nullptr, k)) return 0;
+  return plan_fold(k, ws_bytes);
 }
 
 extern "C" int dmc_conv2d_fused_epilogue(const dmc_conv_desc* d, size_t ws_bytes) {
   ConvK k;
   if (fill_convk(d, nullptr, nullptr, nullptr, nullptr, nullptr, k)) return 0;
+  if (d->fold != DMC_FOLD_NONE) {
+    if (d->fold != fold_kind(k)) return 0;
+    set_fold(k, d->fold);
+    return plan_folded(k, true).gn == DMC_GN_PART_KERNEL ? DMC_FUSED_GN_STATS : 0;
+  }
   return plan_conv(k, true, ws_bytes).gn == DMC_GN_PART_KERNEL ? DMC_FUSED_GN_STATS : 0;
 }
 
@@ -2292,10 +2431,10 @@
 
 extern "C" int dmc_pack_weight(int pack_mode, int dtype, const float* w, int Cout, int Cin, int kh, int kw, int Kc,
                                void* dst, void* stream) {
-  DMC_REQUIRE(pack_mode >= 0 && pack_mode <= 2, "pack: mode");
-  DMC_REQUIRE(pack_mode != DMC_PACK_UPDGRAD || (kh == 3 && kw == 3), "pack: UPDGRAD needs 3x3");
-  const int ntaps = pack_mode == DMC_PACK_UPDGRAD ? 16 : kh * kw;
-  const long rows = pack_mode == DMC_PACK_FWD ? Cout : Cin;
+  DMC_REQUIRE(pack_mode >= 0 && pack_mode <= DMC_PACK_DOWNDGRAD, "pack: mode");
+  DMC_REQUIRE(pack_mode < DMC_PACK_UPDGRAD || (kh == 3 && kw == 3), "pack: the folded packs need 3x3");
+  const int ntaps = (pack_mode == DMC_PACK_UPDGRAD || pack_mode == DMC_PACK_UPFOLD) ? 16 : kh * kw;
+  const long rows = (pack_mode == DMC_PACK_FWD || pack_mode == DMC_PACK_UPFOLD) ? Cout : Cin;
   const long total = rows * ntaps * Kc;
   const int blocks = (int)((total + 255) / 256 < 8192 ? (total + 255) / 256 : 8192);
   hipStream_t s = dmc::as_stream(stream);
@@ -2312,7 +2451,7 @@
     if (tiles && n < cap) { tiles[3 * n] = job_index; tiles[3 * n + 1] = a; tiles[3 * n + 2] = b; }
     ++n;
   };
-  if (j->mode == DMC_PACK_FWD) {
+  if (j->mode == DMC_PACK_FWD || j->mode == DMC_PACK_UPFOLD) {
     const int KW = j->koff >= 0 ? j->Cin : j->Kc;
     for (int co = 0; co < j->Cout; co += kPackFwdCo)
       for (int k0 = 0; k0 < KW; k0 += kPackFwdK) put(co, k0);
diff --git a/diffusion_models_collection_amd/csrc/dmc_conv_impl.h b/diffusion_models_collection_amd/csrc/dmc_conv_impl.h
--- a/diffusion_models_collection_amd/csrc/dmc_conv_impl.h
+++ b/diffusion_models_collection_amd/csrc/dmc_conv_impl.h
@@ -3,6 +3,15 @@
 #include "dmc_internal.h"
 
 namespace {
+
+struct ConvCls {
+  int ntaps, tkw, tdy0, tdx0, tsy, tsx;
+  int woff;
+};
+inline unsigned cls_pack(const ConvCls& q, int tapbase) {
+  return (unsigned)q.ntaps | (unsigned)q.tkw << 4 | (unsigned)(q.tdy0 + 1) << 6 | (unsigned)(q.tdx0 + 1) << 8 |
+         (unsigned)(q.tsy + 1) << 10 | (unsigned)(q.tsx + 1) << 12 | (unsigned)tapbase << 14;
+}
 
 struct ConvK {
   const char* x1; const char* x2; const char* w; char* y1; char* y2;
@@ -25,7 +34,32 @@
   int dtype_bytes;
   int reg_epi;
   int gn_G; float gn_eps;
+  int ncls;
+  unsigned cls[4];
 };
+
+DMC_DEV ConvCls cls_select(const ConvK& a, int c) {
+  const unsigned u = c == 0 ? a.cls[0] : c == 1 ? a.cls[1] : c == 2 ? a.cls[2] : a.cls[3];
+  return ConvCls{(int)(u & 15), (int)(u >> 4 & 3), (int)(u >> 6 & 3) - 1, (int)(u >> 8 & 3) - 1, (int)(u >> 10 & 3) - 1,
+                 (int)(u >> 12 & 3) - 1, (int)(u >> 14 & 31) * a.Cout * a.Kc * 2};
+}
+
+DMC_DEV int cls_src_pixel(const ConvK& a, const ConvCls& q, int n, int oy, int ox, int tap) {
+  const int tr = tap / q.tkw;
+  const int iy = oy + q.tdy0 + q.tsy * tr, ix = ox + q.tdx0 + q.tsx * (tap - tr * q.tkw);
+  if (iy < 0 || iy >= a.H || ix < 0 || ix >= a.W) return -1;
+  return (n * a.H + iy) * a.W + ix;
+}
+
+DMC_DEV int cls_out_pixel(const ConvK& a, int par, int pix) {
+  const int n = pix / a.OHW, rem = pix - n * a.OHW;
+  const int i = rem / a.OW, j = rem - i * a.OW;
+  return (n * 2 * a.OH + 2 * i + (par >> 1)) * (2 * a.OW) + 2 * j + (par & 1);
+}
+DMC_DEV int cls_out_seg(const ConvK& a, int par, int seg) {
+  const int spi = a.OHW / 64, n = seg / spi;
+  return (n * 4 + par) * spi + (seg - n * spi);
+}
 
 DMC_DEV int src_pixel(const ConvK& a, int n, int oy, int ox, int tap) {
   const int tr = tap / a.tkw;
@@ -193,6 +227,8 @@
   k.reg_epi = (int)dmc::opt(dmc::OPT_REG_EPI);
   k.M = d->N * d->OH * d->OW; k.OHW = d->OH * d->OW;
   k.sk = nullptr; k.sk_per = 0;
+  k.ncls = 0;
+  for (unsigned& c : k.cls) c = 0;
   {
     const size_t esz = d->dtype == DMC_F32 ? 4 : 2;
     const size_t b1 = (size_t)d->N * d->H * d->W * d->ld1 * esz;
diff --git a/diffusion_models_collection_amd/csrc/dmc_elem.hip b/diffusion_models_collection_amd/csrc/dmc_elem.hip
--- a/diffusion_models_collection_amd/csrc/dmc_elem.hip
+++ b/diffusion_models_collection_amd/csrc/dmc_elem.hip
@@ -24,9 +24,10 @@
     {"DMC_HALO_PRO", 1}, {"DMC_GN_STATS_SPLIT", 0}, {"DMC_GN_BWD_SPLIT", 0}, {"DMC_ATTN_STAGED", 0},
     {"DMC_ATTN_HG", 0}, {"DMC_WG_BLOCKS", 512}, {"DMC_GN_STATS_ONE_MAX", 1l << 20}, {"DMC_GN_BWD_ONE_MAX", 65536},
     {"DMC_NO_XCD", 0}, {"DMC_NO_EPI_STATS", 0}, {"DMC_WG_MINPIX", 0}, {"DMC_GN_BWD_SLICES", 2}, {"DMC_NO_SKGN", 0},
-    {"DMC_WG_HALO_TARGET", 256}, {"DMC_SK_TARGET", 240}, {"DMC_SK_MAX", 8}, {"DMC_NO_NHALO", 0},
+    {"DMC_WG_HALO_TARGET", 256}, {"DMC_SK_TARGET", 240}, {"DMC_NO_NHALO", 0},
     {"DMC_GN_BWD_FUSED", 4}, {"DMC_GN_BWD_FUSED_MAXHW", 1l << 30}, {"DMC_GN_BWD_NT", 1024},
     {"DMC_REG_EPI", 3}, {"DMC_GEMM1X1", 1}, {"DMC_WG_PIPE", 1}, {"DMC_IMG_MASK", 15}, {"DMC_IMG_GN", 1}, {"DMC_WG_IMG4", 1},
+    {"DMC_RESAMPLE_FOLD", 1},
 };
 struct OptTable {
   long v[OPT_COUNT];
diff --git a/diffusion_models_collection_amd/csrc/dmc_internal.h b/diffusion_models_collection_amd/csrc/dmc_internal.h
--- a/diffusion_models_collection_amd/csrc/dmc_internal.h
+++ b/diffusion_models_collection_amd/csrc/dmc_internal.h
@@ -23,8 +23,8 @@
   OPT_NO_NARROW, OPT_NO_GLDS, OPT_NO_SPLITK, OPT_NO_BUFLDS, OPT_NO_HALO, OPT_HALO_PRO, OPT_GN_STATS_SPLIT,
   OPT_GN_BWD_SPLIT, OPT_ATTN_STAGED, OPT_ATTN_HG, OPT_WG_BLOCKS, OPT_GN_STATS_ONE_MAX, OPT_GN_BWD_ONE_MAX,
   OPT_NO_XCD, OPT_NO_EPI_STATS, OPT_WG_MINPIX, OPT_GN_BWD_SLICES, OPT_NO_SKGN, OPT_WG_HALO_TARGET, OPT_SK_TARGET,
-  OPT_SK_MAX, OPT_NO_NHALO, OPT_GN_BWD_FUSED, OPT_GN_BWD_FUSED_MAXHW, OPT_GN_BWD_NT,
-  OPT_REG_EPI, OPT_GEMM1X1, OPT_WG_PIPE, OPT_IMG_MASK, OPT_IMG_GN, OPT_WG_IMG4, OPT_COUNT
+  OPT_NO_NHALO, OPT_GN_BWD_FUSED, OPT_GN_BWD_FUSED_MAXHW, OPT_GN_BWD_NT,
+  OPT_REG_EPI, OPT_GEMM1X1, OPT_WG_PIPE, OPT_IMG_MASK, OPT_IMG_GN, OPT_WG_IMG4, OPT_RESAMPLE_FOLD, OPT_COUNT
 };
 long opt(Opt o);
 }
diff --git a/diffusion_models_collection_amd/kernels.py b/diffusion_models_collection_amd/kernels.py
--- a/diffusion_models_collection_amd/kernels.py
+++ b/diffusion_models_collection_amd/kernels.py
@@ -138,6 +138,10 @@
     p = L.ConvPlan()
     check(LIB.dmc_conv2d_plan(ctypes.byref(d), ws_bytes, ctypes.byref(p)), "dmc_conv2d_plan")
     return p
+
+
+def conv_fold(d):
+    return LIB.dmc_conv_resample_fold(ctypes.byref(d), LIB.dmc_conv2d_workspace(ctypes.byref(d)))
 
 
 def upsample2x(dtype, x, C):
@@ -312,8 +316,8 @@
         Cout, Cin, kh, kw = w.shape[0], w.shape[1], 1, 1
     else:
         Cout, Cin, kh, kw = w.shape
-    ntaps = 16 if mode == L.PACK_UPDGRAD else kh * kw
-    rows = Cout if mode == L.PACK_FWD else Cin
+    ntaps = 16 if mode in (L.PACK_UPDGRAD, L.PACK_UPFOLD) else kh * kw
+    rows = Cout if mode in (L.PACK_FWD, L.PACK_UPFOLD) else Cin
     if out is None:
         out = torch.empty(rows * ntaps * Kc, dtype=dtype, device=w.device)
     check(LIB.dmc_pack_weight(mode, L.dtype_code(dtype), ptr(w.contiguous()), Cout, Cin, kh, kw, Kc, ptr(out),
diff --git a/diffusion_models_collection_amd/models/_unet_exec.py b/diffusion_models_collection_amd/models/_unet_exec.py
--- a/diffusion_models_collection_amd/models/_unet_exec.py
+++ b/diffusion_models_collection_amd/models/_unet_exec.py
@@ -128,8 +128,8 @@
             Cout, Cin, kh, kw = w.shape[0], w.shape[1], 1, 1
         else:
             Cout, Cin, kh, kw = w.shape
-        ntaps = 16 if mode == L.PACK_UPDGRAD else kh * kw
-        rows = Cout if mode == L.PACK_FWD else Cin
+        ntaps = 16 if mode in (L.PACK_UPDGRAD, L.PACK_UPFOLD) else kh * kw
+        rows = Cout if mode in (L.PACK_FWD, L.PACK_UPFOLD) else Cin
 
         def make_buf():
             return torch.empty(rows * ntaps * Kc, dtype=dtype, device=w.device)
@@ -140,7 +140,7 @@
     def _conv(self, srcs, conv, taps, OH, OW, Cout, mode=L.MODE_NORMAL, stride=1, pro=None, drop=None,
               bias=None, addvec=None, ld_add=0, resid=None, out=None, out_f32=False, out_nchw=False,
               dtype=None, packmode=L.PACK_FWD, w=None, Kc=None, silu_pre=None, ld_silu=0, split=None,
-              act=L.ACT_NONE, y_pre=None, stats=None):
+              act=L.ACT_NONE, y_pre=None, stats=None, fold=False):
         dtype = dtype or self.dt
         gn_part = None
         if (stats is not None and _GN_PARTIALS and dtype == torch.bfloat16 and (OH * OW) % 64 == 0 and Cout % 8 == 0
@@ -156,8 +156,6 @@
         N = a.t.shape[0]
         if Kc is None:
             Kc = L.kc_for(C1 + C2, dtype)
-        if w is None:
-            w = self._wpack(conv, packmode, Kc, dtype)
         d = K.make_desc(dtype, N, a.H, a.W, C1, C2, ld1, ld2, Kc, OH, OW, Cout, taps, mode, stride)
         if pro is not None:
             K.set_prologue(d, pro[0], pro[1], pro[2], C1 + C2, drop, C1 + C2)
@@ -179,6 +177,11 @@
                        ld_res=(0 if resid is None or out_nchw else resid.shape[-1]), silu_pre=silu_pre,
                        ld_silu=ld_silu, ldy1=ldy1, ldy2=ldy2, Csplit=csplit, out_f32=out_f32, out_nchw=out_nchw,
                        act=act, y_pre=y_pre, ld_pre=0 if y_pre is None else y_pre.shape[-1], gn_part=gn_part)
+        if fold:
+            d.fold = K.conv_fold(d)
+            packmode = L.FOLD_PACK.get(d.fold, packmode)
+        if w is None:
+            w = self._wpack(conv, packmode, Kc, dtype)
         K.conv(d, a.t, srcs[1].t if len(srcs) > 1 else None, w, y1, y2)
         return d
 
@@ -468,7 +471,7 @@
             a = srcs[0]
             out = self._new(a.t.shape[0], 2 * a.H, 2 * a.W, a.C)
             self._conv([a], layer.conv, K.TAPS3, 2 * a.H, 2 * a.W, a.C, mode=L.MODE_UPSAMPLE, bias=layer.conv.bias,
-                       out=out.t, stats=out)
+                       out=out.t, stats=out, fold=True)
             if tape is not None:
                 tape.append(("up", layer, a, out))
             return out
@@ -668,7 +671,7 @@
                 buf, acc = self._grad_target(a)
                 dya = Act(dy, out.H, out.W, out.C)
                 self._conv([dya], layer.conv, K.TAPS3_DGRAD, a.H, a.W, a.C, mode=L.MODE_DILATE,
-                           out=buf, resid=buf if acc else None, packmode=L.PACK_DGRAD)
+                           out=buf, resid=buf if acc else None, packmode=L.PACK_DGRAD, fold=True)
             elif kind == "up":
                 _, layer, a, out = rec
                 N = a.t.shape[0]
diff --git a/include/dmc.h b/include/dmc.h
--- a/include/dmc.h
+++ b/include/dmc.h
@@ -12,7 +12,8 @@
 enum { DMC_LOSS_L1 = 0, DMC_LOSS_L2 = 1, DMC_LOSS_HUBER = 2 };
 enum { DMC_PRED_EPS = 0, DMC_PRED_V = 1 };
 #define DMC_OBJECTIVE_MAX_BLOCKS 64
-enum { DMC_PACK_FWD = 0, DMC_PACK_DGRAD = 1, DMC_PACK_UPDGRAD = 2 };
+enum { DMC_PACK_FWD = 0, DMC_PACK_DGRAD = 1, DMC_PACK_UPDGRAD = 2, DMC_PACK_UPFOLD = 3, DMC_PACK_DOWNDGRAD = 4 };
+enum { DMC_FOLD_NONE = 0, DMC_FOLD_UP = 1, DMC_FOLD_DOWN_DGRAD = 2 };
 
 int dmc_version(void);
 const char* dmc_last_error(void);
@@ -56,6 +57,7 @@
   float* wg_bias;
   int pro_groups;
   float pro_eps;
+  int fold;
 } dmc_conv_desc;
 enum { DMC_ACT_NONE = 0, DMC_ACT_GELU = 1, DMC_ACT_GELU_DROP = 2, DMC_ACT_DGELU = 3 };
 
@@ -87,6 +89,7 @@
   size_t ws_bytes;
 } dmc_conv_plan;
 int dmc_conv2d_plan(const dmc_conv_desc* d, size_t ws_bytes, dmc_conv_plan* out);
+int dmc_conv_resample_fold(const dmc_conv_desc* d, size_t ws_bytes);
 int dmc_conv2d(const dmc_conv_desc* d, const void* x1, const void* x2, const void* w,
                void* y1, void* y2, void* workspace, size_t ws_bytes, void* stream);
 
```

After: 12080 img/s, median of 6. 1.0% higher.
